# jaswon/osu-dreamer

Hardware: AMD Instinct MI355X
Metric: denoiser train-steps/sec + 50-step sample latents/sec, 1/2/4/8 MI355X (higher is better)
Workload: dtype bf16

## Files before the change

### include/osu_dreamer_hip.h

```cpp
#ifndef OSU_DREAMER_HIP_H
#define OSU_DREAMER_HIP_H

#ifdef __cplusplus
extern "C" {
#endif

enum { OD_F32 = 0, OD_BF16 = 1,
       OD_F32X3 = 2,
       OD_F32X3W = 3,
       OD_F16 = 4 };
enum { OD_EPI_NONE = 0, OD_EPI_SILU = 1 };
enum { OD_ACT_NONE = 0, OD_ACT_SILU = 1 };
enum { OD_ERR_ARG = -1, OD_ERR_ALIGN = -2, OD_ERR_UNSUPPORTED = -3, OD_ERR_COMM = -4 };

int od_version(void);
const char* od_build_source_sha(void);
const char* od_error_string(int code);

int od_gemm_nt(int dtype, const void* A, int lda, const void* W, int ldw, const float* bias, void* C, int ldc,
               int M, int N, int K, int epilogue, int accumulate, void* stream);
int od_gemm_nt_qkrope(int dtype, const void* A, int lda, const void* W, int ldw, const float* bias, void* C, int ldc, int M,
                      int N, int K, const float* wq, const float* wk, const float* table, int L, int H, int hd, float eps,
                      float q_scale, void* stream);
int od_gemm_nt_qkrope_split(int dtype, const void* A, int lda, const void* W, int ldw, const float* bias, void* C, int ldc,
                            void* qk_out, int ldqk, int qk_dtype, int M, int N, int K, const float* wq, const float* wk, const float* table,
                            int L, int H, int hd, float eps, float q_scale, void* stream);
int od_gemm_tn(int dtype, const void* G, int ldg, const void* A, int lda, float* dW, int lddw, float* dbias, int M, int N,
               int K, void* stream);
int od_gemm_tn_blocks(int dtype, const void* G, int ldg, const void* A, int lda, float* dW, int lddw, float* dbias, int M, int N,
                      int K, int n_block, int n_valid, void* stream);
int od_colsum(int dtype, const void* G, int ldg, float* out, int M, int N, void* stream);
int od_pack_weight(int dtype, const float* src, int N, int K, void* dst, int Np, int Kp, int transpose,
                   const int* row_map, void* stream);

int od_linear_small(const float* x, const float* W, const float* b, float* out, float* pre, int B, int N, int K, int act,
                    void* stream);
int od_linear_small_bwd(const float* x, const float* W, const float* pre, const float* dout, float* dpre, float* dW,
                        float* db, float* dx, int accumulate_dx, int B, int N, int K, int act, void* stream);

int od_cl_to_frames(int dtype, const float* src, void* dst, int ldd, int B, int C, int L, void* stream);
int od_proj_in(int dtype, const float* xt, const float* W, const float* bias, void* x, int ldx, int B, int E, int L,
               int D, void* stream);
int od_proj_in_bwd(int dtype, const float* xt, const void* dx, int ldx, float* dW, float* db, int B, int E, int L, int D,
                   void* stream);
int od_silu(int dtype, const void* x, void* y, long n, void* stream);
int od_silu_bwd(int dtype, const void* x, const void* dy, void* dx, long n, void* stream);

int od_rmsnorm_film(int dtype, const void* x, int ldx, const float* ssg, const void* cl, int ldcl, int cl_bcast,
                    void* h, int ldh, float* inv_rms, int B, int L, int C, float eps, void* stream);
int od_rmsnorm_film_bwd(int dtype, const void* x, int ldx, const float* inv_rms, const float* ssg, const void* dh,
                        int lddh, void* dres, int lddres, float* dssg, int B, int L, int C, void* stream);
int od_rmsnorm_gate_residual(int dtype, const void* x, int ldx, const void* h, int ldh, const float* ssg, void* xo,
                             int ldxo, float* inv_rms, int B, int L, int C, float eps, void* stream);
int od_rmsnorm_gate_residual_film(int dtype, const void* x, int ldx, const void* h, int ldh, const float* ssg_a, void* xo, int ldxo,
                                  float* inv_a, const float* ssg_b, const void* cl, int ldcl, int cl_bcast, void* h2, int ldh2,
                                  float* inv_b, int B, int L, int C, float eps, void* stream);
int od_rmsnorm_gate_residual_film_dwconv(int dtype, const void* x, int ldx, const void* h, int ldh, const float* ssg_a, void* xo, int ldxo,
                                         float* inv_a, const float* ssg_b, void* h2, int ldh2, float* inv_b, const float* conv_w,
                                         const float* conv_b, void* y, int ldy, int B, int L, int C, int ksize, float eps, void* stream);
int od_rmsnorm_gate_residual_bwd(int dtype, const void* h, int ldh, const float* inv_rms, const float* ssg,
                                 const void* dy, int lddy, void* dh, int lddh, float* dssg, int B, int L, int C,
                                 void* stream);

int od_rope_table(float* table, int L, int hd, void* stream);
int od_qk_norm_rope(int dtype, const void* qkv, int ldqkv, const float* wq, const float* wk, const float* table,
                    void* qk_out, int ldo, int B, int L, int H, int hd, float eps, float q_scale, void* stream);
int od_qk_norm_rope_bwd(int dtype, const void* qkv, int ldqkv, const float* wq, const float* wk, const float* table,
                        const void* dqk, int lddqk, void* dqkv, int lddqkv, float* dwq, float* dwk, int B, int L,
                        int H, int hd, float eps, float q_scale, void* stream);
int od_flash_attn_fwd(int dtype, const void* q, int ldq, const void* k, int ldk, const void* v, int ldv, void* o, int ldo,
                      float* lse, int B, int H, int L, int hd, float scale, int q_prescaled, void* stream);
int od_flash_attn_fwd_varlen(int dtype, const void* q, int ldq, const void* k, int ldk, const void* v, int ldv, void* o, int ldo,
                             float* lse, const int* lens, int B, int H, int L, int hd, float scale, int q_prescaled, void* stream);
int od_flash_attn_bwd(int dtype, const void* q, int ldq, const void* k, int ldk, const void* v, int ldv, const void* o,
                      int ldo, const void* dout, int lddo, const float* lse, float* delta, void* dq, int lddq, void* dk,
                      int lddk, void* dv, int lddv, int B, int H, int L, int hd, float scale, int q_prescaled, void* stream);
int od_attn_aux_create(void** aux_out);
int od_attn_aux_destroy(void* aux);
int od_flash_attn_bwd_aux(int dtype, const void* q, int ldq, const void* k, int ldk, const void* v, int ldv, const void* o,
                          int ldo, const void* dout, int lddo, const float* lse, float* delta, void* dq, int lddq, void* dk,
                          int lddk, void* dv, int lddv, int B, int H, int L, int hd, float scale, int q_prescaled, void* aux, void* stream);
int od_flash_attn_bwd_varlen(int dtype, const void* q, int ldq, const void* k, int ldk, const void* v, int ldv, const void* o,
                             int ldo, const void* dout, int lddo, const float* lse, float* delta, void* dq, int lddq, void* dk,
                             int lddk, void* dv, int lddv, const int* lens, int B, int H, int L, int hd, float scale, int q_prescaled,
                             void* aux, void* stream);
int od_flash_attn_bwd_fused_ws_bytes(int dtype, int B, int H, int L, long* total_out, long* zero_out);
int od_flash_attn_bwd_fused(int dtype, const void* q, int ldq, const void* k, int ldk, const void* v, int ldv, const void* o, int ldo,
                            const void* dout, int lddo, const float* lse, void* dq, int lddq, void* dk, int lddk, void* dv, int lddv,
                            int B, int H, int L, int hd, float scale, int q_prescaled, void* ws, long ws_bytes, void* stream);
int od_flash_attn_bwd_fused_status(const void* ws, int* err_out, void* stream);
int od_flash_attn_bwd_fused_err_offset(void);
int od_flash_attn_bwd_fused_passes(void);
int od_flash_attn_bwd_fused_prof(void* ws, long* out16);
int od_flash_attn_bwd_passes(void);

int od_dwconv(int dtype, const void* x, int ldx, const float* w, const float* bias, void* y, int ldy, int B, int L,
              int C, int ksize, void* stream);
int od_dwconv_varlen(int dtype, const void* x, int ldx, const float* w, const float* bias, void* y, int ldy, const int* lens,
                     int B, int L, int C, int ksize, void* stream);
int od_dwconv_bwd(int dtype, const void* x, int ldx, const float* w, const void* dy, int lddy, void* dx, int lddx,
                  float* dw, float* db, int B, int L, int C, int ksize, void* stream);
int od_dwconv_bwd_varlen(int dtype, const void* x, int ldx, const float* w, const void* dy, int lddy, void* dx, int lddx,
                         float* dw, float* db, const int* lens, int B, int L, int C, int ksize, void* stream);
int od_scale_channels(int dtype, void* x, int ldx, const float* scale, int B, int L, int C, void* stream);
int od_swiglu_rmsnorm(int dtype, const void* vg, int ldvg, void* hh, int ldhh, float* inv_rms, int M, int Hf, int Hp,
                      float eps, void* stream);
int od_swiglu_rmsnorm_bwd(int dtype, const void* vg, int ldvg, const float* inv_rms, const void* dhh, int lddhh,
                          void* dvg, int lddvg, int M, int Hf, int Hp, void* stream);

int od_final_norm_proj_out(int dtype, const void* x, int ldx, const float* W, const float* bias, float* v,
                           float* inv_rms, int B, int L, int C, int E, float eps, void* stream);
int od_final_norm_proj_out_bwd(int dtype, const void* x, int ldx, const float* inv_rms, const float* W, const float* dv,
                               void* dx, int lddx, float* dW, float* db, int B, int L, int C, int E, void* stream);
int od_uhead_fwd(const float* xt, const float* w0, const float* b0, const float* w1, const float* b1, const float* w3,
                 const float* b3, const float* w4, const float* b4, float* fsum, int B, int E, int L, int U,
                 void* stream);
int od_uhead_fwd_varlen(const float* xt, const float* w0, const float* b0, const float* w1, const float* b1, const float* w3,
                        const float* b3, const float* w4, const float* b4, float* fsum, const int* lens, int B, int E, int L,
                        int U, void* stream);
int od_uhead_bwd(const float* xt, const float* w0, const float* b0, const float* w1, const float* b1, const float* w3,
                 const float* b3, const float* w4, const float* b4, const float* dfm, float* dw0, float* db0, float* dw1,
                 float* db1, float* dw3, float* db3, float* dw4, float* db4, int B, int E, int L, int U, void* stream);
int od_uhead_bwd_varlen(const float* xt, const float* w0, const float* b0, const float* w1, const float* b1, const float* w3,
                        const float* b3, const float* w4, const float* b4, const float* dfm, float* dw0, float* db0, float* dw1,
                        float* db1, float* dw3, float* db3, float* dw4, float* db4, const int* lens, int B, int E, int L, int U,
                        void* stream);
int od_uhead_tail(const float* fsum, const float* mod, const float* w_out, const float* b_out, float* u, int B, int U,
                  int L, float u_scale, void* stream);
int od_uhead_tail_varlen(const float* fsum, const float* mod, const float* w_out, const float* b_out, float* u, const int* lens,
                         int B, int U, int L, float u_scale, void* stream);
int od_uhead_tail_bwd(const float* fsum, const float* mod, const float* w_out, const float* b_out, const float* du,
                      float* dfm, float* dmod, float* dw_out, float* db_out, int B, int U, int L, float u_scale,
                      void* stream);
int od_uhead_tail_bwd_varlen(const float* fsum, const float* mod, const float* w_out, const float* b_out, const float* du,
                             float* dfm, float* dmod, float* dw_out, float* db_out, const int* lens, int B, int U, int L,
                             float u_scale, void* stream);

int od_make_xt(const float* x0, const float* x1, const float* t, float* xt, float* dsq, int B, int E, int L, void* stream);
int od_make_xt_varlen(const float* x0, const float* x1, const float* t, float* xt, float* dsq, const int* lens, int B, int E, int L,
                      void* stream);
int od_loss_grad(const float* xt, const float* x1, const float* u, const float* v, const float* dsq, float* dv,
                 float* sums, int B, int E, int L, float c0, float osl_w, float del_w, void* stream);
int od_loss_grad_varlen(const float* xt, const float* x1, const float* u, const float* v, const float* dsq, float* dv,
                        float* sums, const int* lens, int B, int E, int L, float c0, float osl_w, float del_w, void* stream);
int od_loss_finalize(const float* sums, const float* dsq, const float* u, float* out, float* du, int B, float c0,
                     float osl_w, float del_w, void* stream);
int od_sampler_step(float* x, const float* u, const float* v, const float* eta, int B, int E, int L, void* stream);
int od_sampler_eta(const float* u, float* eta, int B, float c0, int num_steps, void* stream);
int od_sampler_eta_groups(const float* u, const int* offs, float* eta, int G, float c0, int num_steps, void* stream);
int od_sampler_step_varlen(float* x, const float* u, const float* v, const float* eta, const int* lens, const int* offs, int G,
                           int B, int E, int L, void* stream);

int od_det_clear(void);
int od_det_register(const float* base, long count, void* shadow_i64);
int od_det_enable(void* table_dev, void* stream);
int od_det_table_bytes(void);
int od_det_flush(float* dst, long count, void* stream);

int od_sqnorm(const float* g, long n, float* out, const int* status, void* stream);
int od_adamw_ema(float* p, const float* g, float* m, float* v, float* ema, long n, float lr, float beta1, float beta2,
                 float eps, float weight_decay, int step, float ema_decay, int ema_mode, const float* gnorm_sq,
                 float max_norm, const int* status, void* stream);

int od_ema_update(float* ema, const float* p, long n, float ema_decay, int ema_mode, void* stream);

int od_style_conditioning(const float* labels, const float* rff_w, const float* rff_b, const float* cond_w,
                          const float* cond_b, const float* null_labels, float* c, int B, int NL, int F, int H,
                          void* stream);
int od_rmsnorm_rows(const float* x, const float* gamma, float* y, int M, int C, float eps, void* stream);

int od_style_conditioning_bwd(const float* labels, const float* rff_w, const float* rff_b, const float* dc, float* dcond_w,
                              float* dcond_b, float* dnull_labels, int B, int NL, int F, int H, void* stream);
int od_rmsnorm_rows_bwd(const float* x, const float* gamma, const float* dy, float* dx, float* dgamma, int M, int C, float eps,
                        int accumulate_dx, void* stream);
int od_cast_rows(int src_dtype, const void* src, int dst_dtype, void* dst, long n, void* stream);

int od_spec_features_conv(int dtype, const float* audio, const float* w1, const float* b1, const float* g1, const float* w2,
                          const float* b2, const float* g2, void* out, int ldo, int B, int F, int L, float eps, void* stream);
int od_rmsnorm_affine_film(int dtype, const void* x, int ldx, const float* gamma, const float* ssg, void* y, int ldy, int B,
                           int L, int C, float eps, int act, void* stream);
int od_rmsnorm_affine_gate_residual(int dtype, const void* x, int ldx, const void* h, int ldh, const float* gamma,
                                    const float* ssg, void* xo, int ldxo, int B, int L, int C, float eps, void* stream);
int od_unet_mixer(int dtype, const void* x, int ldx, const void* p, int ldp, int p_bcast, const void* gx, int ldg,
                  const float* gamma, void* xo, int ldxo, int B, int L, int C, float eps, void* stream);
int od_unet_down(int dtype, const void* x, int ldx, const float* w, const float* bias, void* y, int ldy, int B, int Lo, int C,
                 int stride, void* stream);
int od_unet_up(int dtype, const void* x, int ldx, const float* w, const float* bias, void* y, int ldy, int B, int Li, int C,
               int stride, void* stream);
int od_chart_head(int dtype, const void* x, int ldx, const float* W, const float* bias, float* out, int B, int L, int C, int N,
// ... 83 lines not shown
```

### osu_dreamer_amd/csrc/heads.hip

```cpp
#include "od_common.h"
#include "od_api_internal.h"

namespace {

constexpr int UW = 32;
constexpr int UOWN = 30;
constexpr int UWPB = 4;
constexpr int MAXU = 64, MAXE = 8;

__device__ __forceinline__ float red32(float v) {
#pragma unroll
    for (int m = 16; m >= 1; m >>= 1) v += __shfl_xor(v, m);
    return v;
}

struct UHeadW {
    const float *w0, *b0, *w1, *b1, *w3, *b3, *w4, *b4;
};

struct UHeadSmem {
    float xts[MAXE][UW + 4];
    float z0s[MAXE][UW + 2];
    float z1s[MAXU][UW + 2];
    float a1s[MAXU][UW + 2];
    float z3s[MAXU][UW + 1];
    float g4s[MAXU][UW + 1];
    float w4s[MAXU][MAXU + 1];
};

__device__ __forceinline__ void uhead_window_fwd(UHeadSmem& S, const float* __restrict__ xt, const UHeadW& P, int b, int l0,
                                                 int E, int L, int U, int Lv) {
    const int t = threadIdx.x;
    for (int idx = t; idx < E * (UW + 4); idx += 256) {
        const int e = idx / (UW + 4), ix = idx % (UW + 4);
        const int f = l0 - 3 + ix;
        S.xts[e][ix] = (f >= 0 && f < Lv) ? xt[((size_t)b * E + e) * L + f] : 0.f;
    }
    __syncthreads();
    for (int idx = t; idx < E * (UW + 2); idx += 256) {
        const int e = idx / (UW + 2), i2 = idx % (UW + 2);
        S.z0s[e][i2] = P.b0[e] + P.w0[e * 3 + 0] * S.xts[e][i2] + P.w0[e * 3 + 1] * S.xts[e][i2 + 1] + P.w0[e * 3 + 2] * S.xts[e][i2 + 2];
    }
    __syncthreads();
    for (int idx = t; idx < U * (UW + 2); idx += 256) {
        const int c = idx / (UW + 2), i2 = idx % (UW + 2);
        const int f = l0 - 2 + i2;
        float z = P.b1[c];
        for (int e = 0; e < E; e++) z += P.w1[c * E + e] * S.z0s[e][i2];
        S.z1s[c][i2] = z;
        S.a1s[c][i2] = (f >= 0 && f < Lv) ? od_silu(z) : 0.f;
    }
    __syncthreads();
    for (int idx = t; idx < U * UW; idx += 256) {
        const int c = idx / UW, i = idx % UW;
        S.z3s[c][i] = P.b3[c] + P.w3[c * 3 + 0] * S.a1s[c][i] + P.w3[c * 3 + 1] * S.a1s[c][i + 1] + P.w3[c * 3 + 2] * S.a1s[c][i + 2];
    }
    __syncthreads();
}

__device__ __forceinline__ void uhead_load_w4(UHeadSmem& S, const UHeadW& P, int U) {
    for (int idx = threadIdx.x; idx < U * U; idx += 256) S.w4s[idx / U][idx % U] = P.w4[idx];
    __syncthreads();
}

template <bool VL = false>
__global__ __launch_bounds__(256) void uhead_fwd_kernel(const float* __restrict__ xt, UHeadW P, float* __restrict__ fsum,
                                                        int E, int L, int U, int nwin, int wpb, const OdDetTable* __restrict__ det,
                                                        const int* __restrict__ lens = nullptr) {
    __shared__ UHeadSmem S;
    const int b = blockIdx.y, t = threadIdx.x;
    const int Lb = VL ? od_uniform(lens[b]) : L;
    const int i = t & 31, grp = t >> 5, cpg = U / 8;
    uhead_load_w4(S, P, U);
    float acc[MAXU / 8];
#pragma unroll
    for (int q = 0; q < MAXU / 8; q++) acc[q] = 0.f;
    for (int wi = 0; wi < wpb; wi++) {
        const int win = blockIdx.x * wpb + wi;
        if (win >= nwin) break;
        const int l0 = win * UOWN;
        if (VL && l0 >= Lb) break;
        uhead_window_fwd(S, xt, P, b, l0, E, L, U, Lb);
        const int f = l0 - 1 + i;
        const bool own = (i >= 1 && i < UW - 1 && f < Lb);
#pragma unroll
        for (int q = 0; q < MAXU / 8; q++) {
            if (q < cpg) {
                const int c = grp * cpg + q;
                float z = P.b4[c];
                for (int cc = 0; cc < U; cc++) z += S.w4s[c][cc] * S.z3s[cc][i];
                if (own) acc[q] += od_silu(z);
            }
        }
        __syncthreads();
    }
#pragma unroll
    for (int q = 0; q < MAXU / 8; q++) {
        const float s = red32(acc[q]);
        if (q < cpg && i == 0) od_red_add(det, fsum + (size_t)b * U + grp * cpg + q, s);
    }
}

struct UHeadG {
    float *dw0, *db0, *dw1, *db1, *dw3, *db3, *dw4, *db4;
};

template <bool VL>
__device__ __forceinline__ void uhead_bwd_body(const float* __restrict__ xt, const UHeadW& P, const float* __restrict__ dfm,
                                               const UHeadG& G, int E, int L, int U, int nwin, const OdDetTable* __restrict__ det,
                                               const int* __restrict__ lens) {
    __shared__ UHeadSmem S;
    __shared__ float sdw3[MAXU][3], sdb3[MAXU], sdb4[MAXU], sdw1[MAXU][MAXE], sdb1[MAXU], sdw0[MAXE][3], sdb0[MAXE];
    const int b = blockIdx.y, t = threadIdx.x;
    const int i = t & 31, grp = t >> 5, cpg = U / 8;
    const int Lb = VL ? od_uniform(lens[b]) : L;
    for (int idx = t; idx < MAXU; idx += 256) {
        sdb3[idx] = 0.f; sdb4[idx] = 0.f; sdb1[idx] = 0.f;
        for (int j = 0; j < 3; j++) sdw3[idx][j] = 0.f;
        for (int e = 0; e < MAXE; e++) sdw1[idx][e] = 0.f;
    }
    if (t < MAXE) { sdb0[t] = 0.f; for (int j = 0; j < 3; j++) sdw0[t][j] = 0.f; }
    uhead_load_w4(S, P, U);
    float adw4[16];
#pragma unroll
    for (int q = 0; q < 16; q++) adw4[q] = 0.f;
    const float invL = 1.0f / (float)Lb;

    for (int wi = 0; wi < UWPB; wi++) {
        const int win = blockIdx.x * UWPB + wi;
        if (win >= nwin) break;
        const int l0 = win * UOWN;
        if (VL && l0 >= Lb) break;
        uhead_window_fwd(S, xt, P, b, l0, E, L, U, Lb);
        const int f = l0 - 1 + i;
        const bool inr = (f >= 0 && f < Lb);
        const bool own = (i >= 1 && i < UW - 1 && f < Lb);
#pragma unroll
        for (int q = 0; q < MAXU / 8; q++) {
            if (q < cpg) {
                const int c = grp * cpg + q;
                float z = P.b4[c];
                for (int cc = 0; cc < U; cc++) z += S.w4s[c][cc] * S.z3s[cc][i];
                const float g = inr ? dfm[(size_t)b * U + c] * invL * od_silu_grad(z) : 0.f;
                S.g4s[c][i] = g;
                const float s = red32(own ? g : 0.f);
                if (i == 0) atomicAdd(&sdb4[c], s);
            }
        }
        __syncthreads();
        {
            const int iend = (Lb - (l0 - 1)) < (UW - 1) ? (Lb - (l0 - 1)) : (UW - 1);
#pragma unroll
            for (int q = 0; q < 16; q++) {
                const int o = t + 256 * q;
                if (o < U * U) {
                    const int c = o / U, cc = o % U;
                    float s = 0.f;
                    for (int ii = 1; ii < iend; ii++) s += S.g4s[c][ii] * S.z3s[cc][ii];
                    adw4[q] += s;
                }
            }
        }
        __syncthreads();
        float dz3v[MAXU / 8];
#pragma unroll
        for (int q = 0; q < MAXU / 8; q++) {
            dz3v[q] = 0.f;
            if (q < cpg) {
                const int cc = grp * cpg + q;
                float s = 0.f;
                for (int c = 0; c < U; c++) s += S.w4s[c][cc] * S.g4s[c][i];
                dz3v[q] = s;
            }
        }
        __syncthreads();
#pragma unroll
        for (int q = 0; q < MAXU / 8; q++)
            if (q < cpg) S.z3s[grp * cpg + q][i] = dz3v[q];
        __syncthreads();
#pragma unroll
        for (int q = 0; q < MAXU / 8; q++) {
            if (q < cpg) {
                const int c = grp * cpg + q;
                const float g = own ? S.z3s[c][i] : 0.f;
                float s = red32(g);
                if (i == 0) atomicAdd(&sdb3[c], s);
                for (int j = 0; j < 3; j++) {
                    s = red32(g * S.a1s[c][i + j]);
                    if (i == 0) atomicAdd(&sdw3[c][j], s);
                }
                float dz1 = 0.f;
                if (own) {
                    float da1 = 0.f;
                    for (int j = 0; j < 3; j++) da1 += P.w3[c * 3 + j] * S.z3s[c][i - j + 1];
                    dz1 = da1 * od_silu_grad(S.z1s[c][i + 1]);
                }
                S.g4s[c][i] = dz1;
                s = red32(dz1);
                if (i == 0) atomicAdd(&sdb1[c], s);
                for (int e = 0; e < E; e++) {
                    s = red32(dz1 * S.z0s[e][i + 1]);
                    if (i == 0) atomicAdd(&sdw1[c][e], s);
                }
            }
        }
        __syncthreads();
        {
            const bool ev = grp < E;
            const int e = ev ? grp : 0;
            float dz0 = 0.f;
            if (ev)
                for (int c = 0; c < U; c++) dz0 += P.w1[c * E + e] * S.g4s[c][i];
            float s = red32(dz0);
            if (ev && i == 0) atomicAdd(&sdb0[e], s);
            for (int j = 0; j < 3; j++) {
                s = red32(dz0 * S.xts[e][i + 1 + j]);
                if (ev && i == 0) atomicAdd(&sdw0[e][j], s);
            }
        }
        __syncthreads();
    }
#pragma unroll
    for (int q = 0; q < 16; q++) {
        const int o = t + 256 * q;
        if (o < U * U) od_red_add(det, G.dw4 + o, adw4[q]);
    }
    __syncthreads();
    for (int c = t; c < U; c += 256) {
        od_red_add(det, G.db4 + c, sdb4[c]);
        od_red_add(det, G.db3 + c, sdb3[c]);
        od_red_add(det, G.db1 + c, sdb1[c]);
        for (int j = 0; j < 3; j++) od_red_add(det, G.dw3 + c * 3 + j, sdw3[c][j]);
        for (int e = 0; e < E; e++) od_red_add(det, G.dw1 + c * E + e, sdw1[c][e]);
    }
    if (t < E) {
        od_red_add(det, G.db0 + t, sdb0[t]);
        for (int j = 0; j < 3; j++) od_red_add(det, G.dw0 + t * 3 + j, sdw0[t][j]);
    }
}

__global__ __launch_bounds__(256) void uhead_bwd_kernel(const float* __restrict__ xt, UHeadW P, const float* __restrict__ dfm,
                                                        UHeadG G, int E, int L, int U, int nwin, const OdDetTable* __restrict__ det) {
    uhead_bwd_body<false>(xt, P, dfm, G, E, L, U, nwin, det, nullptr);
}
__global__ __launch_bounds__(256) void uhead_bwd_varlen_kernel(const float* __restrict__ xt, UHeadW P, const float* __restrict__ dfm,
                                                               UHeadG G, int E, int L, int U, int nwin, const OdDetTable* __restrict__ det,
                                                               const int* __restrict__ lens) {
    uhead_bwd_body<true>(xt, P, dfm, G, E, L, U, nwin, det, lens);
}

template <bool VL = false>
__global__ void uhead_tail_kernel(const float* __restrict__ fsum, const float* __restrict__ mod, const float* __restrict__ w,
                                  const float* __restrict__ bo, float* __restrict__ u, int B, int U, int L, float u_scale,
                                  const int* __restrict__ lens = nullptr) {
    const int b = blockIdx.x, lane = threadIdx.x;
    const float Lf = (float)(VL ? od_uniform(lens[b]) : L);
    float s = 0.f;
    for (int c = lane; c < U; c += 64) {
        const float f = fsum[(size_t)b * U + c] / Lf;
        s += w[c] * (f * (1.f + mod[(size_t)b * 2 * U + c]) + mod[(size_t)b * 2 * U + U + c]);
    }
    s = od_wave_sum(s);
    if (lane == 0) {
        const float y = s + bo[0];
        const float sp = y > 20.f ? y : log1pf(__expf(y));
        u[b] = u_scale * sp;
    }
}
template <bool VL = false>
__global__ void uhead_tail_bwd_kernel(const float* __restrict__ fsum, const float* __restrict__ mod, const float* __restrict__ w,
                                      const float* __restrict__ bo, const float* __restrict__ du, float* __restrict__ dfm,
                                      float* __restrict__ dmod, float* __restrict__ dw, float* __restrict__ dbo,
                                      int B, int U, int L, float u_scale, const OdDetTable* __restrict__ det,
                                      const int* __restrict__ lens = nullptr) {
    const int b = blockIdx.x, lane = threadIdx.x;
    const float Lf = (float)(VL ? od_uniform(lens[b]) : L);
    float s = 0.f;
    for (int c = lane; c < U; c += 64) {
        const float f = fsum[(size_t)b * U + c] / Lf;
        s += w[c] * (f * (1.f + mod[(size_t)b * 2 * U + c]) + mod[(size_t)b * 2 * U + U + c]);
    }
    s = od_wave_sum(s);
    const float y = s + bo[0];
    const float dy = du[b] * u_scale * od_sigmoid(y);
    for (int c = lane; c < U; c += 64) {
        const float f = fsum[(size_t)b * U + c] / Lf;
        const float sc = mod[(size_t)b * 2 * U + c], sh = mod[(size_t)b * 2 * U + U + c];
        const float fm = f * (1.f + sc) + sh;
        od_red_add(det, dw + c, dy * fm);
        const float dfmv = dy * w[c];
        dfm[(size_t)b * U + c] = dfmv * (1.f + sc);
        dmod[(size_t)b * 2 * U + c] = dfmv * f;
        dmod[(size_t)b * 2 * U + U + c] = dfmv;
    }
    if (lane == 0) od_red_add(det, dbo, dy);
}

__device__ __forceinline__ float block_sum_256(float v, float* sh) {
    v = od_wave_sum(v);
    __syncthreads();
    if ((threadIdx.x & 63) == 0) sh[threadIdx.x >> 6] = v;
    __syncthreads();
    return sh[0] + sh[1] + sh[2] + sh[3];
}

template <bool VL = false>
__global__ __launch_bounds__(256) void make_xt_kernel(const float* __restrict__ x0, const float* __restrict__ x1,
                                                      const float* __restrict__ t, float* __restrict__ xt,
                                                      float* __restrict__ dsq, int EL, int L, const OdDetTable* __restrict__ det,
                                                      const int* __restrict__ lens = nullptr) {
    __shared__ float sh[4];
    const int b = blockIdx.y;
    const int Lb = VL ? od_uniform(lens[b]) : L;
    const float w = t[b];
    float acc = 0.f;
    for (int i = blockIdx.x * 256 + threadIdx.x; i < EL; i += gridDim.x * 256) {
        const size_t o = (size_t)b * EL + i;
        if (VL && (i % L) >= Lb) { xt[o] = 0.f; continue; }
        const float a = x0[o], e = x1[o];
        const float v = w < 0.5f ? a + w * (e - a) : e - (e - a) * (1.f - w);
        xt[o] = v;
        const float d = v - e;
        acc += d * d;
    }
    acc = block_sum_256(acc, sh);
    if (threadIdx.x == 0) od_red_add(det, dsq + b, acc / (float)Lb);
}

template <bool VL = false>
__global__ __launch_bounds__(256) void loss_grad_kernel(const float* __restrict__ xt, const float* __restrict__ x1,
                                                        const float* __restrict__ u, const float* __restrict__ v,
                                                        const float* __restrict__ dsq, float* __restrict__ dv,
                                                        float* __restrict__ sums, int B, int EL, int L, float c0,
                                                        float osl_w, float del_w, const OdDetTable* __restrict__ det,
                                                        const int* __restrict__ lens = nullptr) {
    __shared__ float sh[4];
    const int b = blockIdx.y;
    const int Lb = VL ? od_uniform(lens[b]) : L;
    const float ub = u[b], den = dsq[b] + c0, ut = sqrtf(den);
    const float k1 = osl_w / ((float)B * den), k2 = del_w / (float)B, invL2 = 2.f / (float)Lb;
    float s1 = 0.f, s2 = 0.f, s3 = 0.f;
    for (int i = blockIdx.x * 256 + threadIdx.x; i < EL; i += gridDim.x * 256) {
        const size_t o = (size_t)b * EL + i;
        if (VL && (i % L) >= Lb) { dv[o] = 0.f; continue; }
        const float xv = xt[o], e = x1[o], vv = v[o];
        const float r1 = xv - ub * vv - e;
        const float r2 = vv - (xv - e) / ut;
        s1 += r1 * r1; s2 += r2 * r2; s3 += r1 * (-vv);
        dv[o] = k1 * invL2 * r1 * (-ub) + k2 * invL2 * r2;
    }
    s1 = block_sum_256(s1, sh); s2 = block_sum_256(s2, sh); s3 = block_sum_256(s3, sh);
    if (threadIdx.x == 0) {
        od_red_add(det, sums + b * 3 + 0, s1 / (float)Lb);
        od_red_add(det, sums + b * 3 + 1, s2 / (float)Lb);
        od_red_add(det, sums + b * 3 + 2, s3 * invL2);
    }
}

__global__ void loss_finalize_kernel(const float* __restrict__ sums, const float* __restrict__ dsq, const float* __restrict__ u,
                                     float* __restrict__ out, float* __restrict__ du, int B, float c0, float osl_w, float del_w) {
    const int lane = threadIdx.x;
    float osl = 0.f, del = 0.f, mape = 0.f;
    for (int b = lane; b < B; b += 64) {
        const float den = dsq[b] + c0, ut = sqrtf(den);
        osl += sums[b * 3 + 0] / den;
        del += sums[b * 3 + 1];
        mape += fabsf((u[b] - ut) / ut);
        du[b] = osl_w / ((float)B * den) * sums[b * 3 + 2];
    }
    osl = od_wave_sum(osl) / (float)B; del = od_wave_sum(del) / (float)B; mape = od_wave_sum(mape) / (float)B;
    if (lane == 0) { out[0] = osl_w * osl + del_w * del; out[1] = osl; out[2] = del; out[3] = mape; }
}

__global__ __launch_bounds__(256) void sampler_step_kernel(float* __restrict__ x, const float* __restrict__ u,
                                                           const float* __restrict__ v, const float* __restrict__ eta, int EL) {
    const int b = blockIdx.y;
    const float k = eta[0] * u[b];
    for (int i = blockIdx.x * 256 + threadIdx.x; i < EL; i += gridDim.x * 256) {
// ... 215 lines not shown
```

### osu_dreamer_amd/csrc/misc.hip

```cpp
#include "od_common.h"
#include "od_api_internal.h"
#include <type_traits>

namespace {

template <class T>
__global__ __launch_bounds__(256) void cl_to_frames_kernel(const float* __restrict__ src, T* __restrict__ dst, int ldd, int C, int L) {
    __shared__ float tile[64][65];
    const int b = blockIdx.z, l0 = blockIdx.x * 64, c0 = blockIdx.y * 64;
    const int tx = threadIdx.x & 63, ty = threadIdx.x >> 6;
    for (int i = ty; i < 64; i += 4) {
        const int c = c0 + i, l = l0 + tx;
        tile[i][tx] = (c < C && l < L) ? src[((size_t)b * C + c) * L + l] : 0.f;
    }
    __syncthreads();
    for (int i = ty; i < 64; i += 4) {
        const int l = l0 + i, c = c0 + tx;
        if (l < L && c < C) od_t<T>::st(dst + ((size_t)b * L + l) * ldd + c, tile[tx][i]);
    }
}

template <class T>
__global__ __launch_bounds__(256) void proj_in_kernel(const float* __restrict__ xt, const float* __restrict__ W,
                                                      const float* __restrict__ bias, T* __restrict__ x, int ldx,
                                                      int B, int E, int L, int D) {
    const int lane = threadIdx.x & 63;
    const long M = (long)B * L;
    const long nw = (long)gridDim.x * 4, w0 = (long)blockIdx.x * 4 + (threadIdx.x >> 6);
    for (int c = lane * 8; c < D; c += 512) {
        float wv[8][8], bv[8];
        od_ld8(bias + c, bv);
        if (E == 6) {
            float flat[48];
#pragma unroll
            for (int q = 0; q < 6; q++) od_ld8(W + (size_t)c * 6 + q * 8, *(float(*)[8])&flat[q * 8]);
#pragma unroll
            for (int k = 0; k < 8; k++)
#pragma unroll
                for (int e = 0; e < 8; e++) wv[k][e] = e < 6 ? flat[k * 6 + e] : 0.f;
        } else {
#pragma unroll
            for (int k = 0; k < 8; k++)
#pragma unroll
                for (int e = 0; e < 8; e++) wv[k][e] = e < E ? W[(size_t)(c + k) * E + e] : 0.f;
        }
        for (long m = w0; m < M; m += nw) {
            const int b = (int)(m / L), l = (int)(m % L);
            float xe[8];
#pragma unroll
            for (int e = 0; e < 8; e++) xe[e] = e < E ? xt[((size_t)b * E + e) * L + l] : 0.f;
            float o[8];
#pragma unroll
            for (int k = 0; k < 8; k++) {
                float s = bv[k];
#pragma unroll
                for (int e = 0; e < 8; e++) s += wv[k][e] * xe[e];
                o[k] = s;
            }
            od_st8(x + m * ldx + c, o);
        }
    }
}

template <class T>
__global__ __launch_bounds__(256) void proj_in_bwd_kernel(const float* __restrict__ xt, const T* __restrict__ dx, int ldx,
                                                          float* __restrict__ dW, float* __restrict__ db, int B, int E, int L, int D,
                                                          const OdDetTable* __restrict__ det) {
    __shared__ float red[64][73];
    const int lane = threadIdx.x & 63, wave = threadIdx.x >> 6;
    const int M = B * L;
    const int nw = gridDim.x * 4, w0 = blockIdx.x * 4 + wave;
    for (int c0 = 0; c0 < D; c0 += 512) {
        const int c = c0 + lane * 8;
        float aw[8][8], ab[8];
#pragma unroll
        for (int k = 0; k < 8; k++) {
            ab[k] = 0.f;
#pragma unroll
            for (int e = 0; e < 8; e++) aw[k][e] = 0.f;
        }
        if (c < D)
            for (int m = w0; m < M; m += nw) {
                const int b = m / L, l = m - b * L;
                float xe[8], g[8];
#pragma unroll
                for (int e = 0; e < 8; e++) xe[e] = e < E ? xt[((size_t)b * E + e) * L + l] : 0.f;
                od_ld8(dx + (size_t)m * ldx + c, g);
#pragma unroll
                for (int k = 0; k < 8; k++) {
                    ab[k] += g[k];
#pragma unroll
                    for (int e = 0; e < 8; e++) aw[k][e] += g[k] * xe[e];
                }
            }
        for (int w = 0; w < 4; w++) {
            if (wave == w) {
#pragma unroll
                for (int k = 0; k < 8; k++) {
                    red[lane][k * 9 + 8] = (w ? red[lane][k * 9 + 8] : 0.f) + ab[k];
#pragma unroll
                    for (int e = 0; e < 8; e++) red[lane][k * 9 + e] = (w ? red[lane][k * 9 + e] : 0.f) + aw[k][e];
                }
            }
            __syncthreads();
        }
        if (wave == 0 && c < D) {
#pragma unroll
            for (int k = 0; k < 8; k++) {
                od_red_add(det, db + c + k, red[lane][k * 9 + 8]);
#pragma unroll
                for (int e = 0; e < 8; e++)
                    if (e < E) od_red_add(det, dW + (size_t)(c + k) * E + e, red[lane][k * 9 + e]);
            }
        }
        __syncthreads();
    }
}

template <class T>
__global__ __launch_bounds__(256) void silu_kernel(const T* __restrict__ x, T* __restrict__ y, long n8) {
    for (long i = (long)blockIdx.x * 256 + threadIdx.x; i < n8; i += (long)gridDim.x * 256) {
        float v[8]; od_ld8(x + i * 8, v);
#pragma unroll
        for (int e = 0; e < 8; e++) v[e] = od_silu(v[e]);
        od_st8(y + i * 8, v);
    }
}
template <class T>
__global__ __launch_bounds__(256) void silu_bwd_kernel(const T* __restrict__ x, const T* __restrict__ dy, T* __restrict__ dx, long n8) {
    for (long i = (long)blockIdx.x * 256 + threadIdx.x; i < n8; i += (long)gridDim.x * 256) {
        float v[8], g[8]; od_ld8(x + i * 8, v); od_ld8(dy + i * 8, g);
#pragma unroll
        for (int e = 0; e < 8; e++) g[e] *= od_silu_grad(v[e]);
        od_st8(dx + i * 8, g);
    }
}

template <class T, int KS, int DW_RUN, bool VL = false>
__global__ __launch_bounds__(256) void dwconv_kernel(const T* __restrict__ x, int ldx, const float* __restrict__ w,
                                                     const float* __restrict__ bias, T* __restrict__ y, int ldy,
                                                     int L, int C, const int* __restrict__ lens = nullptr) {
    constexpr int R = KS / 2;
    const int cg = C / 8;
    const int b = blockIdx.y;
    const int Lb = VL ? od_uniform(lens[b]) : L;
    const long t = (long)blockIdx.x * 256 + threadIdx.x;
    const int cgi = (int)(t % cg);
    const long run = t / cg;
    const int l0 = (int)(run * DW_RUN);
    if (l0 >= L) return;
    const int c = cgi * 8;
    float wv[8][KS], bv[8];
#pragma unroll
    for (int k = 0; k < 8; k++) {
        bv[k] = bias[c + k];
#pragma unroll
        for (int j = 0; j < KS; j++) wv[k][j] = w[(size_t)(c + k) * KS + j];
    }
    float win[KS][8];
    const T* xb = x + (size_t)b * L * ldx + c;
#pragma unroll
    for (int j = 0; j < KS - 1; j++) {
        const int l = l0 - R + j;
        if (l >= 0 && l < Lb) od_ld8(xb + (size_t)l * ldx, win[j]);
        else {
#pragma unroll
            for (int k = 0; k < 8; k++) win[j][k] = 0.f;
        }
    }
    for (int i = 0; i < DW_RUN; i++) {
        const int l = l0 + i;
        if (l >= L) break;
        const int ln = l + R;
        if (ln < Lb) od_ld8(xb + (size_t)ln * ldx, win[KS - 1]);
        else {
#pragma unroll
            for (int k = 0; k < 8; k++) win[KS - 1][k] = 0.f;
        }
        float o[8];
#pragma unroll
        for (int k = 0; k < 8; k++) {
            float s = bv[k];
#pragma unroll
            for (int j = 0; j < KS; j++) s += wv[k][j] * win[j][k];
            o[k] = (VL && l >= Lb) ? 0.f : s;
        }
        od_st8(y + ((size_t)b * L + l) * ldy + c, o);
#pragma unroll
        for (int j = 0; j < KS - 1; j++)
#pragma unroll
            for (int k = 0; k < 8; k++) win[j][k] = win[j + 1][k];
    }
}

constexpr int DW_RUN_BWD = 64;
template <class T, int KS, bool VL = false>
__global__ __launch_bounds__(256) void dwconv_bwd_kernel(const T* __restrict__ x, int ldx, const float* __restrict__ w,
                                                         const T* __restrict__ dy, int lddy, T* __restrict__ dx, int lddx,
                                                         float* __restrict__ dw, float* __restrict__ db, int L, int C,
                                                         const OdDetTable* __restrict__ det, const int* __restrict__ lens = nullptr) {
    constexpr int R = KS / 2;
    __shared__ long long red[(KS <= 5 ? 1024 : 512) * (KS + 1)];
    __shared__ int s_bad;
    const int cg = C / 8;
    const int b = blockIdx.y;
    const int Lb = VL ? od_uniform(lens[b]) : L;
    const long t = (long)blockIdx.x * 256 + threadIdx.x;
    const int cgi = (int)(t % cg);
    const long run = t / cg;
    const int l0 = (int)(run * DW_RUN_BWD);
    const bool active = l0 < L;
    const int c = cgi * 8;
    for (int i = threadIdx.x; i < C * (KS + 1); i += 256) red[i] = 0;
    if (threadIdx.x == 0) s_bad = 0;
    __syncthreads();
    float wv[8][KS], adw[8][KS], adb[8];
#pragma unroll
    for (int k = 0; k < 8; k++) {
        adb[k] = 0.f;
#pragma unroll
        for (int j = 0; j < KS; j++) { wv[k][j] = w[(size_t)(c + k) * KS + j]; adw[k][j] = 0.f; }
    }
    if (active) {
        float wy[KS][8], wx[KS][8];
        const T* xb = x + (size_t)b * L * ldx + c;
        const T* yb = dy + (size_t)b * L * lddy + c;
#pragma unroll
        for (int j = 0; j < KS - 1; j++) {
            const int l = l0 - R + j;
            if (l >= 0 && l < Lb) { od_ld8(xb + (size_t)l * ldx, wx[j]); od_ld8(yb + (size_t)l * lddy, wy[j]); }
            else {
#pragma unroll
                for (int k = 0; k < 8; k++) { wx[j][k] = 0.f; wy[j][k] = 0.f; }
            }
        }
        constexpr int DW_PF = 2;
        typedef typename std::conditional<sizeof(T) == 2, u32x4, f32x4>::type row_t;
        row_t px[DW_PF][sizeof(T) == 2 ? 1 : 2], py[DW_PF][sizeof(T) == 2 ? 1 : 2];
        auto fetch = [&](int ln, int slot) {
            if (ln < Lb) {
#pragma unroll
                for (int h2 = 0; h2 < (sizeof(T) == 2 ? 1 : 2); h2++) {
                    px[slot][h2] = *(const row_t*)(xb + (size_t)ln * ldx + h2 * 4);
                    py[slot][h2] = *(const row_t*)(yb + (size_t)ln * lddy + h2 * 4);
                }
            } else {
#pragma unroll
                for (int h2 = 0; h2 < (sizeof(T) == 2 ? 1 : 2); h2++) { px[slot][h2] = (row_t)(0); py[slot][h2] = (row_t)(0); }
            }
        };
        auto unpack = [&](const row_t (&r)[sizeof(T) == 2 ? 1 : 2], float (&o8)[8]) {
            if constexpr (sizeof(T) == 2) {
#pragma unroll
                for (int i2 = 0; i2 < 4; i2++) {
                    union { uint32_t u; float f; } lo, hi;
                    lo.u = r[0][i2] << 16; hi.u = r[0][i2] & 0xffff0000u;
                    o8[2 * i2] = lo.f; o8[2 * i2 + 1] = hi.f;
                }
            } else {
#pragma unroll
                for (int i2 = 0; i2 < 4; i2++) { o8[i2] = r[0][i2]; o8[4 + i2] = r[1][i2]; }
            }
        };
#pragma unroll
        for (int pf = 0; pf < DW_PF; pf++) fetch(l0 + R + pf, pf);
        for (int i0 = 0; i0 < DW_RUN_BWD; i0 += DW_PF) {
          if (l0 + i0 >= L) break;
#pragma unroll
          for (int pf = 0; pf < DW_PF; pf++) {
            const int i = i0 + pf;
            const int l = l0 + i;
            if (l >= L) break;
            unpack(px[pf], wx[KS - 1]);
            unpack(py[pf], wy[KS - 1]);
            fetch(l + R + DW_PF, pf);
            float o[8];
#pragma unroll
            for (int k = 0; k < 8; k++) {
                float sacc = 0.f;
#pragma unroll
                for (int jj = 0; jj < KS; jj++) sacc += wv[k][jj] * wy[KS - 1 - jj][k];
                o[k] = (VL && l >= Lb) ? 0.f : sacc;
                const float gy = wy[R][k];
                adb[k] += gy;
#pragma unroll
                for (int jj = 0; jj < KS; jj++) adw[k][jj] += gy * wx[jj][k];
            }
            od_st8(dx + ((size_t)b * L + l) * lddx + c, o);
#pragma unroll
            for (int j = 0; j < KS - 1; j++)
#pragma unroll
                for (int k = 0; k < 8; k++) { wx[j][k] = wx[j + 1][k]; wy[j][k] = wy[j + 1][k]; }
          }
        }
#pragma unroll
        for (int k = 0; k < 8; k++) {
            od_lds_fix_add(&red[(c + k) * (KS + 1) + KS], adb[k], &s_bad);
#pragma unroll
            for (int j = 0; j < KS; j++) od_lds_fix_add(&red[(c + k) * (KS + 1) + j], adw[k][j], &s_bad);
        }
    }
    __syncthreads();
    for (int i = threadIdx.x; i < C * (KS + 1); i += 256) {
        const int ch = i / (KS + 1), j = i % (KS + 1);
        const float v = od_lds_unfix(red[i], s_bad);
        if (v != 0.f) {
            if (j == KS) od_red_add(det, db + ch, v); else od_red_add(det, dw + (size_t)ch * KS + j, v);
        }
    }
}

constexpr int LS_KC = 256, LS_NB = 8;
__global__ __launch_bounds__(256) void linear_small_kernel(const float* __restrict__ x, const float* __restrict__ W,
                                                           const float* __restrict__ bias, float* __restrict__ out,
                                                           float* __restrict__ pre, int B, int N, int K, int act) {
    __shared__ __attribute__((aligned(16))) float xs[32][LS_KC + 4];
    __shared__ __attribute__((aligned(16))) float ws[LS_NB][LS_KC + 4];
    const int b0 = blockIdx.y * 32, n0 = blockIdx.x * LS_NB;
    const int bl = threadIdx.x & 31, nl = threadIdx.x >> 5;
    float acc = 0.f;
    for (int k0 = 0; k0 < K; k0 += LS_KC) {
        const int kc = K - k0 < LS_KC ? K - k0 : LS_KC;
        for (int i = threadIdx.x; i < 32 * LS_KC; i += 256) {
            const int r = i / LS_KC, c = i % LS_KC;
            xs[r][c] = (b0 + r < B && c < kc) ? x[(size_t)(b0 + r) * K + k0 + c] : 0.f;
        }
        for (int i = threadIdx.x; i < LS_NB * LS_KC; i += 256) {
            const int r = i / LS_KC, c = i % LS_KC;
            ws[r][c] = (n0 + r < N && c < kc) ? W[(size_t)(n0 + r) * K + k0 + c] : 0.f;
        }
        __syncthreads();
#pragma unroll 8
        for (int c = 0; c < LS_KC; c += 4) {
            const f32x4 a = *(const f32x4*)&xs[bl][c], w = *(const f32x4*)&ws[nl][c];
            acc += a[0] * w[0]; acc += a[1] * w[1]; acc += a[2] * w[2]; acc += a[3] * w[3];
        }
        __syncthreads();
    }
    const int b = b0 + bl, n = n0 + nl;
    if (b < B && n < N) {
        const float s = acc + (bias ? bias[n] : 0.f);
        if (pre) pre[(size_t)b * N + n] = s;
        out[(size_t)b * N + n] = act == OD_ACT_SILU ? od_silu(s) : s;
    }
}
__global__ __launch_bounds__(256) void linear_small_dpre_kernel(const float* __restrict__ pre, const float* __restrict__ dout,
                                                                float* __restrict__ dpre, long n, int act) {
    const long i = (long)blockIdx.x * 256 + threadIdx.x;
    if (i >= n) return;
    dpre[i] = act == OD_ACT_SILU ? dout[i] * od_silu_grad(pre[i]) : dout[i];
}
__global__ __launch_bounds__(256) void linear_small_dw_kernel(const float* __restrict__ x, const float* __restrict__ dpre,
                                                              float* __restrict__ dW, float* __restrict__ db, int B, int N, int K) {
    const int n = blockIdx.y, k = blockIdx.x * 256 + threadIdx.x;
    if (dW && k < K) {
        float s0 = 0.f, s1 = 0.f, s2 = 0.f, s3 = 0.f;
        int b = 0;
        for (; b + 3 < B; b += 4) {
            s0 += dpre[(size_t)b * N + n] * x[(size_t)b * K + k];
            s1 += dpre[(size_t)(b + 1) * N + n] * x[(size_t)(b + 1) * K + k];
            s2 += dpre[(size_t)(b + 2) * N + n] * x[(size_t)(b + 2) * K + k];
            s3 += dpre[(size_t)(b + 3) * N + n] * x[(size_t)(b + 3) * K + k];
        }
        for (; b < B; b++) s0 += dpre[(size_t)b * N + n] * x[(size_t)b * K + k];
        dW[(size_t)n * K + k] += (s0 + s1) + (s2 + s3);
    }
    if (db && blockIdx.x == 0 && threadIdx.x == 0) {
        float s = 0.f;
        for (int b = 0; b < B; b++) s += dpre[(size_t)b * N + n];
        db[n] += s;
    }
}
constexpr int LS_NR = 32;
__global__ __launch_bounds__(256) void linear_small_dx_kernel(const float* __restrict__ W, const float* __restrict__ dpre,
                                                              float* __restrict__ dx, int B, int N, int K, const OdDetTable* __restrict__ det) {
    __shared__ __attribute__((aligned(16))) float ds[LS_NR][32];
    const int n0 = blockIdx.x * LS_NR, b0 = blockIdx.y * 32, k = blockIdx.z * 256 + threadIdx.x;
    for (int i = threadIdx.x; i < LS_NR * 32; i += 256) {
        const int bl = i / LS_NR, nl = i % LS_NR;
        ds[nl][bl] = (b0 + bl < B && n0 + nl < N) ? dpre[(size_t)(b0 + bl) * N + n0 + nl] : 0.f;
    }
    __syncthreads();
    if (k >= K) return;
    float acc[32];
#pragma unroll
    for (int i = 0; i < 32; i++) acc[i] = 0.f;
    const int nr = N - n0 < LS_NR ? N - n0 : LS_NR;
    for (int nl = 0; nl < nr; nl++) {
        const float w = W[(size_t)(n0 + nl) * K + k];
#pragma unroll
        for (int q4 = 0; q4 < 8; q4++) {
            const f32x4 d = *(const f32x4*)&ds[nl][4 * q4];
            acc[4 * q4] += d[0] * w; acc[4 * q4 + 1] += d[1] * w; acc[4 * q4 + 2] += d[2] * w; acc[4 * q4 + 3] += d[3] * w;
        }
    }
#pragma unroll
    for (int i = 0; i < 32; i++)
        if (b0 + i < B) od_red_add(det, dx + (size_t)(b0 + i) * K + k, acc[i]);
}

__global__ __launch_bounds__(256) void zero_f32_kernel(float* __restrict__ p, long n) {
    const long i = (long)blockIdx.x * 256 + threadIdx.x;
    if (i < n) p[i] = 0.f;
}

template <class T>
__global__ __launch_bounds__(256) void pack_weight_kernel(const float* __restrict__ src, int N, int K, T* __restrict__ dst,
                                                          int Np, int Kp, int transpose, const int* __restrict__ row_map) {
    const long i = (long)blockIdx.x * 256 + threadIdx.x;
    if (i >= (long)Np * Kp) return;
    int n, k;
    if (!transpose) { n = (int)(i / Kp); k = (int)(i % Kp); }
    else { k = (int)(i / Np); n = (int)(i % Np); }
    const int sn = row_map ? row_map[n] : (n < N ? n : -1);
    const float v = (sn >= 0 && k < K) ? src[(size_t)sn * K + k] : 0.f;
    od_t<T>::st(dst + i, v);
}

__global__ __launch_bounds__(256) void pack_weight_split_kernel(const float* __restrict__ src, int N, int K, bf16_t* __restrict__ dst,
                                                                int Np, int Kp, const int* __restrict__ row_map) {
    const long i = (long)blockIdx.x * 256 + threadIdx.x;
    if (i >= (long)Np * Kp) return;
    const int n = (int)(i / Kp), k = (int)(i % Kp);
    const int sn = row_map ? row_map[n] : (n < N ? n : -1);
    const float v = (sn >= 0 && k < K) ? src[(size_t)sn * K + k] : 0.f;
    const bf16_t hi = od_f2bf(v);
    const bf16_t lo = od_f2bf(v - od_bf2f(hi));
    bf16_t* slab = dst + ((size_t)n * Kp + (k & ~31)) * 2;
    slab[k & 31] = hi;
    slab[32 + (k & 31)] = lo;
}

}

#define DISPATCH_T(DT, CALL)                                       \
    do {                                                           \
        if ((DT) == OD_BF16) { typedef bf16_t T_; CALL; }          \
        else if ((DT) == OD_F32) { typedef float T_; CALL; }       \
        else return OD_ERR_ARG;                                    \
    } while (0)

extern "C" int od_cl_to_frames(int dtype, const float* src, void* dst, int ldd, int B, int C, int L, void* stream) {
    dim3 grid((L + 63) / 64, (C + 63) / 64, B);
    DISPATCH_T(dtype, OD_LAUNCH((cl_to_frames_kernel<T_>), grid, dim3(256), 0, (hipStream_t)stream, src, (T_*)dst, ldd, C, L));
    OD_CHECK_LAUNCH();
    return 0;
}

extern "C" int od_proj_in(int dtype, const float* xt, const float* W, const float* bias, void* x, int ldx, int B, int E, int L,
                          int D, void* stream) {
    if (E > 8) return OD_ERR_UNSUPPORTED;
    if (D % 8 || ldx % 8) return OD_ERR_ALIGN;
    const long M = (long)B * L;
    int blocks = (int)((M + 15) / 16); if (blocks > 4096) blocks = 4096;
    DISPATCH_T(dtype, OD_LAUNCH((proj_in_kernel<T_>), dim3(blocks), dim3(256), 0, (hipStream_t)stream, xt, W, bias, (T_*)x, ldx, B, E, L, D));
    OD_CHECK_LAUNCH();
    return 0;
}

extern "C" int od_proj_in_bwd(int dtype, const float* xt, const void* dx, int ldx, float* dW, float* db, int B, int E, int L, int D,
                              void* stream) {
    if (E > 8) return OD_ERR_UNSUPPORTED;
    if (D % 8 || ldx % 8) return OD_ERR_ALIGN;
    const long M = (long)B * L;
    if (M > 0x7fffffffL) return OD_ERR_UNSUPPORTED;
    int blocks = (int)((M + 63) / 64); if (blocks > 512) blocks = 512; if (blocks < 1) blocks = 1;
    DISPATCH_T(dtype, OD_LAUNCH((proj_in_bwd_kernel<T_>), dim3(blocks), dim3(256), 0, (hipStream_t)stream, xt, (const T_*)dx, ldx, dW, db, B, E, L, D, od_det_active()));
    OD_CHECK_LAUNCH();
    return 0;
}

extern "C" int od_silu(int dtype, const void* x, void* y, long n, void* stream) {
    if (n % 8) return OD_ERR_ALIGN;
    long n8 = n / 8; int blocks = (int)((n8 + 255) / 256); if (blocks > 4096) blocks = 4096; if (blocks < 1) blocks = 1;
    DISPATCH_T(dtype, OD_LAUNCH((silu_kernel<T_>), dim3(blocks), dim3(256), 0, (hipStream_t)stream, (const T_*)x, (T_*)y, n8));
    OD_CHECK_LAUNCH();
    return 0;
}
extern "C" int od_silu_bwd(int dtype, const void* x, const void* dy, void* dx, long n, void* stream) {
    if (n % 8) return OD_ERR_ALIGN;
    long n8 = n / 8; int blocks = (int)((n8 + 255) / 256); if (blocks > 4096) blocks = 4096; if (blocks < 1) blocks = 1;
    DISPATCH_T(dtype, OD_LAUNCH((silu_bwd_kernel<T_>), dim3(blocks), dim3(256), 0, (hipStream_t)stream, (const T_*)x, (const T_*)dy, (T_*)dx, n8));
    OD_CHECK_LAUNCH();
    return 0;
}

template <class T>
__global__ __launch_bounds__(256) void scale_channels_kernel(T* __restrict__ x, int ldx, const float* __restrict__ scale, long M, int L, int C) {
    const int cg = C / 8;
    const long i = (long)blockIdx.x * 256 + threadIdx.x;
    if (i >= M * cg) return;
    const long m = i / cg;
    const int c = (int)(i % cg) * 8;
    float v[8], f[8];
    od_ld8(x + m * ldx + c, v);
    od_ld8(scale + (m / L) * C + c, f);
#pragma unroll
    for (int e = 0; e < 8; e++) v[e] *= f[e];
    od_st8(x + m * ldx + c, v);
}

extern "C" int od_scale_channels(int dtype, void* x, int ldx, const float* scale, int B, int L, int C, void* stream) {
    if (C % 8 || ldx % 8) return OD_ERR_ALIGN;
    const long M = (long)B * L, n = M * (C / 8);
    if (n == 0) return 0;
    DISPATCH_T(dtype, OD_LAUNCH((scale_channels_kernel<T_>), dim3((unsigned)((n + 255) / 256)), dim3(256), 0, (hipStream_t)stream, (T_*)x, ldx, scale, M, L, C));
    OD_CHECK_LAUNCH();
    return 0;
}

extern "C" int od_dwconv(int dtype, const void* x, int ldx, const float* w, const float* bias, void* y, int ldy, int B, int L,
                         int C, int ksize, void* stream) {
    if (C % 8 || ldx % 8 || ldy % 8) return OD_ERR_ALIGN;
    if (ksize != 3 && ksize != 5 && ksize != 7 && ksize != 9) return OD_ERR_UNSUPPORTED;
#ifndef OD_DW_SMALL_THREADS
#define OD_DW_SMALL_THREADS 131072
#endif
    const bool small = (long)B * (C / 8) * ((L + 31) / 32) < OD_DW_SMALL_THREADS;
    const int run = small ? 4 : 32;
    const long threads = (long)(C / 8) * ((L + run - 1) / run);
    dim3 grid((unsigned)((threads + 255) / 256), B);
#define DW_GO(KS_, RUN_) DISPATCH_T(dtype, OD_LAUNCH((dwconv_kernel<T_, KS_, RUN_>), grid, dim3(256), 0, (hipStream_t)stream, (const T_*)x, ldx, w, bias, (T_*)y, ldy, L, C))
    if (ksize == 5) { if (small) DW_GO(5, 4); else DW_GO(5, 32); }
    else if (ksize == 3) { if (small) DW_GO(3, 4); else DW_GO(3, 32); }
    else if (ksize == 7) { if (small) DW_GO(7, 4); else DW_GO(7, 32); }
    else { if (small) DW_GO(9, 4); else DW_GO(9, 32); }
#undef DW_GO
    OD_CHECK_LAUNCH();
    return 0;
}

extern "C" int od_dwconv_varlen(int dtype, const void* x, int ldx, const float* w, const float* bias, void* y, int ldy, const int* lens,
                                int B, int L, int C, int ksize, void* stream) {
    if (C % 8 || ldx % 8 || ldy % 8) return OD_ERR_ALIGN;
    if (ksize != 3 && ksize != 5 && ksize != 7 && ksize != 9) return OD_ERR_UNSUPPORTED;
    if (!lens) return OD_ERR_ARG;
    const bool small = (long)B * (C / 8) * ((L + 31) / 32) < OD_DW_SMALL_THREADS;
    const int run = small ? 4 : 32;
    const long threads = (long)(C / 8) * ((L + run - 1) / run);
    dim3 grid((unsigned)((threads + 255) / 256), B);
#define DW_GO(KS_, RUN_) DISPATCH_T(dtype, OD_LAUNCH((dwconv_kernel<T_, KS_, RUN_, true>), grid, dim3(256), 0, (hipStream_t)stream, (const T_*)x, ldx, w, bias, (T_*)y, ldy, L, C, lens))
    if (ksize == 5) { if (small) DW_GO(5, 4); else DW_GO(5, 32); }
    else if (ksize == 3) { if (small) DW_GO(3, 4); else DW_GO(3, 32); }
    else if (ksize == 7) { if (small) DW_GO(7, 4); else DW_GO(7, 32); }
    else { if (small) DW_GO(9, 4); else DW_GO(9, 32); }
#undef DW_GO
    OD_CHECK_LAUNCH();
    return 0;
}

extern "C" int od_dwconv_bwd(int dtype, const void* x, int ldx, const float* w, const void* dy, int lddy, void* dx, int lddx,
                             float* dw, float* db, int B, int L, int C, int ksize, void* stream) {
    if (C % 8 || ldx % 8 || lddy % 8 || lddx % 8) return OD_ERR_ALIGN;
    if (C > 1024 || (ksize > 5 && C > 512)) return OD_ERR_UNSUPPORTED;
    const long threads = (long)(C / 8) * ((L + DW_RUN_BWD - 1) / DW_RUN_BWD);
    dim3 grid((unsigned)((threads + 255) / 256), B);
    if (ksize == 5) DISPATCH_T(dtype, OD_LAUNCH((dwconv_bwd_kernel<T_, 5>), grid, dim3(256), 0, (hipStream_t)stream, (const T_*)x, ldx, w, (const T_*)dy, lddy, (T_*)dx, lddx, dw, db, L, C, od_det_active()));
    else if (ksize == 3) DISPATCH_T(dtype, OD_LAUNCH((dwconv_bwd_kernel<T_, 3>), grid, dim3(256), 0, (hipStream_t)stream, (const T_*)x, ldx, w, (const T_*)dy, lddy, (T_*)dx, lddx, dw, db, L, C, od_det_active()));
    else if (ksize == 7 && C <= 512) DISPATCH_T(dtype, OD_LAUNCH((dwconv_bwd_kernel<T_, 7>), grid, dim3(256), 0, (hipStream_t)stream, (const T_*)x, ldx, w, (const T_*)dy, lddy, (T_*)dx, lddx, dw, db, L, C, od_det_active()));
    else if (ksize == 9 && C <= 512) DISPATCH_T(dtype, OD_LAUNCH((dwconv_bwd_kernel<T_, 9>), grid, dim3(256), 0, (hipStream_t)stream, (const T_*)x, ldx, w, (const T_*)dy, lddy, (T_*)dx, lddx, dw, db, L, C, od_det_active()));
    else return OD_ERR_UNSUPPORTED;
    OD_CHECK_LAUNCH();
    return 0;
}

extern "C" int od_dwconv_bwd_varlen(int dtype, const void* x, int ldx, const float* w, const void* dy, int lddy, void* dx, int lddx,
                                    float* dw, float* db, const int* lens, int B, int L, int C, int ksize, void* stream) {
    if (C % 8 || ldx % 8 || lddy % 8 || lddx % 8) return OD_ERR_ALIGN;
    if (C > 1024 || (ksize > 5 && C > 512)) return OD_ERR_UNSUPPORTED;
    if (!lens) return OD_ERR_ARG;
    const long threads = (long)(C / 8) * ((L + DW_RUN_BWD - 1) / DW_RUN_BWD);
    dim3 grid((unsigned)((threads + 255) / 256), B);
#define DWB_GO(KS_) DISPATCH_T(dtype, OD_LAUNCH((dwconv_bwd_kernel<T_, KS_, true>), grid, dim3(256), 0, (hipStream_t)stream, (const T_*)x, ldx, w, (const T_*)dy, lddy, (T_*)dx, lddx, dw, db, L, C, od_det_active(), lens))
    if (ksize == 5) DWB_GO(5);
    else if (ksize == 3) DWB_GO(3);
    else if (ksize == 7) DWB_GO(7);
    else if (ksize == 9) DWB_GO(9);
    else return OD_ERR_UNSUPPORTED;
#undef DWB_GO
    OD_CHECK_LAUNCH();
    return 0;
}

extern "C" int od_linear_small(const float* x, const float* W, const float* b, float* out, float* pre, int B, int N, int K, int act,
                               void* stream) {
    OD_LAUNCH(linear_small_kernel, dim3((N + LS_NB - 1) / LS_NB, (B + 31) / 32), dim3(256), 0, (hipStream_t)stream, x, W, b, out, pre, B, N, K, act);
    OD_CHECK_LAUNCH();
    return 0;
}

extern "C" int od_linear_small_bwd(const float* x, const float* W, const float* pre, const float* dout, float* dpre, float* dW,
                                   float* db, float* dx, int accumulate_dx, int B, int N, int K, int act, void* stream) {
    if (act != OD_ACT_NONE && !pre) return OD_ERR_ARG;
    const long n = (long)B * N;
    OD_LAUNCH(linear_small_dpre_kernel, dim3((unsigned)((n + 255) / 256)), dim3(256), 0, (hipStream_t)stream, pre, dout, dpre, n, act);
    if (dW || db)
        OD_LAUNCH(linear_small_dw_kernel, dim3((K + 255) / 256, N), dim3(256), 0, (hipStream_t)stream, x, (const float*)dpre, dW, db, B, N, K);
    if (dx) {
        if (!accumulate_dx)
            OD_LAUNCH(zero_f32_kernel, dim3((unsigned)(((long)B * K + 255) / 256)), dim3(256), 0, (hipStream_t)stream, dx, (long)B * K);
        OD_LAUNCH(linear_small_dx_kernel, dim3((N + LS_NR - 1) / LS_NR, (B + 31) / 32, (K + 255) / 256), dim3(256), 0, (hipStream_t)stream, W,
                  (const float*)dpre, dx, B, N, K, od_det_active());
    }
    OD_CHECK_LAUNCH();
    return 0;
}

extern "C" int od_pack_weight(int dtype, const float* src, int N, int K, void* dst, int Np, int Kp, int transpose,
                              const int* row_map, void* stream) {
    const long n = (long)Np * Kp;
    if (dtype == OD_F32X3W) {
        if (transpose || Kp % 32) return OD_ERR_UNSUPPORTED;
        OD_LAUNCH(pack_weight_split_kernel, dim3((unsigned)((n + 255) / 256)), dim3(256), 0, (hipStream_t)stream, src, N, K, (bf16_t*)dst, Np, Kp, row_map);
        OD_CHECK_LAUNCH();
        return 0;
    }
    DISPATCH_T(dtype, OD_LAUNCH((pack_weight_kernel<T_>), dim3((unsigned)((n + 255) / 256)), dim3(256), 0, (hipStream_t)stream, src, N, K, (T_*)dst, Np, Kp, transpose, row_map));
    OD_CHECK_LAUNCH();
    return 0;
}
```

### osu_dreamer_amd/csrc/od_common.h

```cpp
#pragma once
#if defined(OD_EMU)
#include "emu_hip.h"
#else
#include <hip/hip_runtime.h>
#define OD_LAUNCH(kern, grid, block, smem, stream, ...) \
    hipLaunchKernelGGL(kern, (grid), (block), (smem), (stream), __VA_ARGS__)
#define OD_LAUNCH_DYN(kern, grid, block, smem, stream, ...)                                                    \
    do {                                                                                                       \
         \
        static const hipError_t attr_rc__ =                                                                    \
            hipFuncSetAttribute((const void*)(kern), hipFuncAttributeMaxDynamicSharedMemorySize, 160 * 1024);  \
        if (attr_rc__ != hipSuccess) return -(int)attr_rc__ - 1000;                                            \
        hipLaunchKernelGGL(kern, (grid), (block), (smem), (stream), __VA_ARGS__);                              \
    } while (0)
#define OD_DYN_SMEM(name) extern __shared__ __attribute__((aligned(16))) unsigned char name[]
#endif
#include <stdint.h>

typedef unsigned short bf16_t;
typedef float f32x4 __attribute__((ext_vector_type(4)));
typedef float f32x16 __attribute__((ext_vector_type(16)));
typedef short s16x8 __attribute__((ext_vector_type(8)));
typedef short s16x4 __attribute__((ext_vector_type(4)));
typedef unsigned int u32x4 __attribute__((ext_vector_type(4)));
typedef unsigned int u32x2 __attribute__((ext_vector_type(2)));

#define OD_WAVE 64

__device__ __forceinline__ float od_bf2f(bf16_t h) {
    union { uint32_t u; float f; } c; c.u = ((uint32_t)h) << 16; return c.f;
}
#if defined(OD_EMU)
__device__ __forceinline__ bf16_t od_f2bf(float f) {
    union { uint32_t u; float f; } c; c.f = f;
    uint32_t u = c.u;
    if ((u & 0x7fffffffu) > 0x7f800000u) return (bf16_t)((u >> 16) | 0x40);
    u += 0x7fffu + ((u >> 16) & 1u);
    return (bf16_t)(u >> 16);
}
__device__ __forceinline__ uint32_t od_pack_bf2(float lo, float hi) { return (uint32_t)od_f2bf(lo) | ((uint32_t)od_f2bf(hi) << 16); }
__device__ __forceinline__ float od_exp2(float x) { return exp2f(x); }
#else
typedef __bf16 od_bf2_t __attribute__((ext_vector_type(2)));
typedef float od_f2_t __attribute__((ext_vector_type(2)));
__device__ __forceinline__ bf16_t od_f2bf(float f) { return __builtin_bit_cast(unsigned short, (__bf16)f); }
__device__ __forceinline__ uint32_t od_pack_bf2(float lo, float hi) {
    od_f2_t v; v[0] = lo; v[1] = hi;
    return __builtin_bit_cast(uint32_t, __builtin_convertvector(v, od_bf2_t));
}
__device__ __forceinline__ float od_exp2(float x) { return __builtin_amdgcn_exp2f(x); }
#endif

struct f16_t { unsigned short bits; };
#if defined(OD_EMU)
__device__ __forceinline__ float od_h2f(f16_t h) { return emu::f16_to_f32(h.bits); }
__device__ __forceinline__ f16_t od_f2h(float f) { return f16_t{emu::f32_to_f16(f)}; }
#else
__device__ __forceinline__ float od_h2f(f16_t h) { return (float)__builtin_bit_cast(_Float16, h.bits); }
__device__ __forceinline__ f16_t od_f2h(float f) { return f16_t{__builtin_bit_cast(unsigned short, (_Float16)f)}; }
#endif
#if defined(OD_EMU)
__device__ __forceinline__ uint32_t od_pack_h2(float lo, float hi) { return (uint32_t)od_f2h(lo).bits | ((uint32_t)od_f2h(hi).bits << 16); }
#else
typedef _Float16 od_h2_t __attribute__((ext_vector_type(2)));
__device__ __forceinline__ uint32_t od_pack_h2(float lo, float hi) {
    float __attribute__((ext_vector_type(2))) v; v[0] = lo; v[1] = hi;
    return __builtin_bit_cast(uint32_t, __builtin_convertvector(v, od_h2_t));
}
#endif
template <class T> __device__ __forceinline__ uint32_t od_pack2(float lo, float hi);
template <> __device__ __forceinline__ uint32_t od_pack2<bf16_t>(float lo, float hi) { return od_pack_bf2(lo, hi); }
template <> __device__ __forceinline__ uint32_t od_pack2<f16_t>(float lo, float hi) { return od_pack_h2(lo, hi); }

struct f32x3_t { float x; };
struct f32x3w_t : f32x3_t {};

template <class T> struct od_t;
template <> struct od_t<f32x3_t> {
    static __device__ __forceinline__ float ld(const f32x3_t* p) { return p->x; }
    static __device__ __forceinline__ void st(f32x3_t* p, float v) { p->x = v; }
};
template <> struct od_t<f32x3w_t> : od_t<f32x3_t> {};
template <> struct od_t<float> {
    static __device__ __forceinline__ float ld(const float* p) { return *p; }
    static __device__ __forceinline__ void st(float* p, float v) { *p = v; }
};
template <> struct od_t<bf16_t> {
    static __device__ __forceinline__ float ld(const bf16_t* p) { return od_bf2f(*p); }
    static __device__ __forceinline__ void st(bf16_t* p, float v) { *p = od_f2bf(v); }
};
template <> struct od_t<f16_t> {
    static __device__ __forceinline__ float ld(const f16_t* p) { return od_h2f(*p); }
    static __device__ __forceinline__ void st(f16_t* p, float v) { *p = od_f2h(v); }
};

template <class T> __device__ __forceinline__ float od_round_to(float x);
template <> __device__ __forceinline__ float od_round_to<float>(float x) { return x; }
template <> __device__ __forceinline__ float od_round_to<bf16_t>(float x) { return od_bf2f(od_f2bf(x)); }
template <> __device__ __forceinline__ float od_round_to<f16_t>(float x) { return od_h2f(od_f2h(x)); }
template <> __device__ __forceinline__ float od_round_to<f32x3_t>(float x) { return x; }
template <> __device__ __forceinline__ float od_round_to<f32x3w_t>(float x) { return x; }

__device__ __forceinline__ void od_ld8(const float* p, float (&v)[8]) {
    f32x4 a = *(const f32x4*)p, b = *(const f32x4*)(p + 4);
    v[0] = a[0]; v[1] = a[1]; v[2] = a[2]; v[3] = a[3];
    v[4] = b[0]; v[5] = b[1]; v[6] = b[2]; v[7] = b[3];
}
__device__ __forceinline__ void od_ld8(const bf16_t* p, float (&v)[8]) {
    u32x4 r = *(const u32x4*)p;
#pragma unroll
    for (int i = 0; i < 4; i++) {
        union { uint32_t u; float f; } lo, hi;
        lo.u = r[i] << 16; hi.u = r[i] & 0xffff0000u;
        v[2 * i] = lo.f; v[2 * i + 1] = hi.f;
    }
}
__device__ __forceinline__ void od_st8(float* p, const float (&v)[8]) {
    f32x4 a, b;
    a[0] = v[0]; a[1] = v[1]; a[2] = v[2]; a[3] = v[3];
    b[0] = v[4]; b[1] = v[5]; b[2] = v[6]; b[3] = v[7];
    *(f32x4*)p = a; *(f32x4*)(p + 4) = b;
}
__device__ __forceinline__ void od_ld8(const f32x3_t* p, float (&v)[8]) { od_ld8((const float*)p, v); }
__device__ __forceinline__ void od_st8(f32x3_t* p, const float (&v)[8]) { od_st8((float*)p, v); }
__device__ __forceinline__ void od_st8(bf16_t* p, const float (&v)[8]) {
    u32x4 r;
#pragma unroll
    for (int i = 0; i < 4; i++) r[i] = od_pack_bf2(v[2 * i], v[2 * i + 1]);
    *(u32x4*)p = r;
}

__device__ __forceinline__ void od_ld8(const f16_t* p, float (&v)[8]) {
    u32x4 r = *(const u32x4*)p;
#pragma unroll
    for (int i = 0; i < 4; i++) {
        v[2 * i] = od_h2f(f16_t{(unsigned short)(r[i] & 0xffffu)});
        v[2 * i + 1] = od_h2f(f16_t{(unsigned short)(r[i] >> 16)});
    }
}
__device__ __forceinline__ void od_st8(f16_t* p, const float (&v)[8]) {
    u32x4 r;
#pragma unroll
    for (int i = 0; i < 4; i++) r[i] = od_pack_h2(v[2 * i], v[2 * i + 1]);
    *(u32x4*)p = r;
}

template <class T> __device__ __forceinline__ void od_st8_nt(T* p, const float (&v)[8]) { od_st8(p, v); }
#if !defined(OD_EMU)
template <> __device__ __forceinline__ void od_st8_nt<bf16_t>(bf16_t* p, const float (&v)[8]) {
    u32x4 r;
#pragma unroll
    for (int i = 0; i < 4; i++) r[i] = od_pack_bf2(v[2 * i], v[2 * i + 1]);
    asm volatile("global_store_dwordx4 %0, %1, off nt\n\ts_nop 0" ::"v"(p), "v"(r) : "memory");
}
#endif

#if defined(OD_EMU)
__device__ __forceinline__ void od_st16_nt(void* p, u32x4 r) { *(u32x4*)p = r; }
#else
__device__ __forceinline__ void od_st16_nt(void* p, u32x4 r) {
    asm volatile("global_store_dwordx4 %0, %1, off nt\n\ts_nop 0" ::"v"(p), "v"(r) : "memory");
}
#endif

__device__ __forceinline__ float od_wave_sum(float v) {
#pragma unroll
    for (int m = 32; m >= 1; m >>= 1) v += __shfl_xor(v, m);
    return v;
}
__device__ __forceinline__ float od_silu(float x) { return x / (1.0f + __expf(-x)); }
__device__ __forceinline__ float od_sigmoid(float x) { return 1.0f / (1.0f + __expf(-x)); }
__device__ __forceinline__ float od_silu_grad(float x) {
    float s = od_sigmoid(x);
    return s * (1.0f + x * (1.0f - s));
}

#if defined(OD_EMU)
__device__ __forceinline__ f32x4 od_mul4(f32x4 a, f32x4 b) { return a * b; }
__device__ __forceinline__ f32x4 od_mul4s(f32x4 a, float b) { return a * b; }
#else
__device__ __forceinline__ float od_mul1(float a, float b) {
    float d = a * b;
    asm("" : "+v"(d));
    return d;
}
__device__ __forceinline__ f32x4 od_mul4(f32x4 a, f32x4 b) {
    f32x4 d;
#pragma unroll
    for (int r = 0; r < 4; r++) d[r] = od_mul1(a[r], b[r]);
    return d;
}
__device__ __forceinline__ f32x4 od_mul4s(f32x4 a, float b) {
    f32x4 d;
#pragma unroll
    for (int r = 0; r < 4; r++) d[r] = od_mul1(a[r], b);
    return d;
}
#endif

template <class T> struct od_frag;
template <> struct od_frag<bf16_t> { s16x8 v; };
template <> struct od_frag<f16_t> { s16x8 v; };
template <> struct od_frag<float> { float v[8]; };
template <> struct od_frag<f32x3_t> { s16x8 hi, lo; };
template <> struct od_frag<f32x3w_t> : od_frag<f32x3_t> {};
__device__ __forceinline__ void od_frag_pack(od_frag<float>& f, const float (&x)[8]) {
#pragma unroll
    for (int j = 0; j < 8; j++) f.v[j] = x[j];
}
__device__ __forceinline__ void od_split2(float a, float b, uint32_t& hi, uint32_t& lo) {
    hi = od_pack_bf2(a, b);
    union { uint32_t u; float f; } x, y;
    x.u = hi << 16; y.u = hi & 0xffff0000u;
    lo = od_pack_bf2(a - x.f, b - y.f);
}
__device__ __forceinline__ void od_frag_pack(od_frag<f32x3_t>& f, const float (&x)[8]) {
    u32x4 h, l;
#pragma unroll
    for (int i = 0; i < 4; i++) {
        uint32_t a, b;
        od_split2(x[2 * i], x[2 * i + 1], a, b);
        h[i] = a; l[i] = b;
    }
    f.hi = __builtin_bit_cast(s16x8, h); f.lo = __builtin_bit_cast(s16x8, l);
}

__device__ __forceinline__ void od_frag_load(od_frag<bf16_t>& f, const bf16_t* p) { f.v = *(const s16x8*)p; }
__device__ __forceinline__ void od_frag_load(od_frag<f16_t>& f, const f16_t* p) { f.v = *(const s16x8*)p; }
__device__ __forceinline__ void od_frag_load(od_frag<float>& f, const float* p) { od_ld8(p, f.v); }
__device__ __forceinline__ void od_frag_load(od_frag<f32x3_t>& f, const f32x3_t* p) { float x[8]; od_ld8(p, x); od_frag_pack(f, x); }
__device__ __forceinline__ void od_frag_zero(od_frag<bf16_t>& f) { f.v = (s16x8)(0); }
__device__ __forceinline__ void od_frag_zero(od_frag<float>& f) {
#pragma unroll
    for (int j = 0; j < 8; j++) f.v[j] = 0.f;
}
__device__ __forceinline__ void od_frag_zero(od_frag<f32x3_t>& f) { f.hi = (s16x8)(0); f.lo = (s16x8)(0); }
__device__ __forceinline__ void od_frag_set4(od_frag<bf16_t>& f, int half, float a, float b, float c, float d) {
    u32x4 w = __builtin_bit_cast(u32x4, f.v);
    w[2 * half] = od_pack_bf2(a, b);
    w[2 * half + 1] = od_pack_bf2(c, d);
    f.v = __builtin_bit_cast(s16x8, w);
}
__device__ __forceinline__ void od_frag_set4(od_frag<f16_t>& f, int half, float a, float b, float c, float d) {
    u32x4 w = __builtin_bit_cast(u32x4, f.v);
    w[2 * half] = od_pack_h2(a, b);
    w[2 * half + 1] = od_pack_h2(c, d);
    f.v = __builtin_bit_cast(s16x8, w);
}
__device__ __forceinline__ void od_frag_set4(od_frag<float>& f, int half, float a, float b, float c, float d) {
    f.v[4 * half] = a; f.v[4 * half + 1] = b; f.v[4 * half + 2] = c; f.v[4 * half + 3] = d;
}
__device__ __forceinline__ void od_frag_set4(od_frag<f32x3_t>& f, int half, float a, float b, float c, float d) {
    u32x4 h = __builtin_bit_cast(u32x4, f.hi), l = __builtin_bit_cast(u32x4, f.lo);
    uint32_t h0, l0, h1, l1;
    od_split2(a, b, h0, l0);
    od_split2(c, d, h1, l1);
    h[2 * half] = h0; l[2 * half] = l0; h[2 * half + 1] = h1; l[2 * half + 1] = l1;
    f.hi = __builtin_bit_cast(s16x8, h); f.lo = __builtin_bit_cast(s16x8, l);
}

#if defined(OD_EMU)
__device__ __forceinline__ s16x4 od_lds_tr_read(const bf16_t* p) { return emu::ds_read_tr16_b64(p); }
#else
__device__ __forceinline__ s16x4 od_lds_tr_read(const bf16_t* p) {
    return __builtin_amdgcn_ds_read_tr16_b64_v4i16((__attribute__((address_space(3))) s16x4*)p);
}
#endif
__device__ __forceinline__ s16x4 od_lds_tr_read_at(unsigned addr);

__device__ __forceinline__ f32x4 od_mma(const od_frag<bf16_t>& a, const od_frag<bf16_t>& b, f32x4 c) {
    return __builtin_amdgcn_mfma_f32_16x16x32_bf16(a.v, b.v, c, 0, 0, 0);
}
#if defined(OD_EMU)
__device__ __forceinline__ f32x4 od_mma(const od_frag<f16_t>& a, const od_frag<f16_t>& b, f32x4 c) { return emu::mfma_16x16x32_f16(a.v, b.v, c); }
#else
typedef _Float16 od_h8_t __attribute__((ext_vector_type(8)));
__device__ __forceinline__ f32x4 od_mma(const od_frag<f16_t>& a, const od_frag<f16_t>& b, f32x4 c) {
    return __builtin_amdgcn_mfma_f32_16x16x32_f16(__builtin_bit_cast(od_h8_t, a.v), __builtin_bit_cast(od_h8_t, b.v), c, 0, 0, 0);
}
#endif
__device__ __forceinline__ f32x4 od_mma(const od_frag<float>& a, const od_frag<float>& b, f32x4 c) {
#pragma unroll
    for (int j = 0; j < 8; j++) c = __builtin_amdgcn_mfma_f32_16x16x4f32(a.v[j], b.v[j], c, 0, 0, 0);
    return c;
}
__device__ __forceinline__ f32x4 od_mma(const od_frag<f32x3_t>& a, const od_frag<f32x3_t>& b, f32x4 c) {
    c = __builtin_amdgcn_mfma_f32_16x16x32_bf16(a.lo, b.hi, c, 0, 0, 0);
    c = __builtin_amdgcn_mfma_f32_16x16x32_bf16(a.hi, b.lo, c, 0, 0, 0);
    return __builtin_amdgcn_mfma_f32_16x16x32_bf16(a.hi, b.hi, c, 0, 0, 0);
}

static __device__ __attribute__((aligned(16))) unsigned char od_zero16[16];

#if defined(OD_EMU)
__device__ __forceinline__ void od_glds16(const void* g, void* lds) { emu::global_load_lds16(g, lds); }
#else
__device__ __forceinline__ void od_glds16(const void* g, void* lds) {
    __builtin_amdgcn_global_load_lds((const __attribute__((address_space(1))) void*)g,
                                     (__attribute__((address_space(3))) void*)lds, 16, 0, 0);
}
#endif
#if defined(OD_EMU)
__device__ __forceinline__ void od_glds16_async(const void* g, void* lds_base) { emu::global_load_lds16(g, (unsigned char*)lds_base + 16 * emu::lane_id()); }
#else
__device__ __forceinline__ void od_glds16_async(const void* g, void* lds_base) {
    const unsigned a = (unsigned)__builtin_amdgcn_readfirstlane((int)(unsigned)(size_t)(__attribute__((address_space(3))) unsigned char*)lds_base);
    asm volatile("s_mov_b32 m0, %1\n\ts_nop 0\n\tglobal_load_lds_dwordx4 %0, off" ::"v"(g), "s"(a) : "memory", "m0");
}
#endif

#if defined(OD_EMU)
struct od_srd_t { const unsigned char* base; unsigned bytes; };
__device__ __forceinline__ od_srd_t od_make_srd(const void* base, unsigned bytes) { return od_srd_t{(const unsigned char*)base, bytes}; }
__device__ __forceinline__ void od_srd_set_bytes(od_srd_t& r, unsigned bytes) { r.bytes = bytes; }
__device__ __forceinline__ void od_buffer_lds16(od_srd_t r, unsigned voff, unsigned soff, void* lds) {
    alignas(16) unsigned char tmp[16] = {0};
    const unsigned off = voff + soff;
    if (off < r.bytes) { const unsigned n = (r.bytes - off) & ~3u; memcpy(tmp, r.base + off, n < 16 ? n : 16); }
    emu::global_load_lds16(tmp, (unsigned char*)lds + 16 * emu::lane_id());
}
// ... 137 lines not shown
```

### osu_dreamer_amd/csrc/rowops.hip

```cpp
#include "od_common.h"
#include "od_api_internal.h"

namespace {

#ifndef OD_QK_BPW
#define OD_QK_BPW 8
#endif
constexpr int ROWS_PER_WAVE_BWD = 16;

template <class T, int NCH>
__device__ __forceinline__ void load_row(const T* row, int C, int lane, float (&v)[NCH][8]) {
#pragma unroll
    for (int i = 0; i < NCH; i++) {
        const int c = (lane + 64 * i) * 8;
        if (c < C) od_ld8(row + c, v[i]);
        else {
#pragma unroll
            for (int e = 0; e < 8; e++) v[i][e] = 0.f;
        }
    }
}
template <int NCH>
__device__ __forceinline__ float row_sumsq(const float (&v)[NCH][8]) {
    float s = 0.f;
// ... 250 lines not shown
                for (int e = 0; e < 8; e++) hv[e] = v[0][e] * inv2 * (1.f + sc[e]) + sh[e];
                if (own && h2) od_st8(h2 + m * ldh2 + c, hv);
#pragma unroll
                for (int e = 0; e < 8; e++) win[KS - 1][e] = od_round_to<T>(hv[e]);
            }
        }
        const int lc = l - R;
        if (lc >= l0 && lc < lend && act) {
            float o[8];
#pragma unroll
            for (int k = 0; k < 8; k++) {
                float s = bv[k];
#pragma unroll
                for (int j = 0; j < KS; j++) s += wv[k][j] * win[j][k];
                o[k] = s;
            }
            od_st8(y + ((size_t)b * L + lc) * ldy + c, o);
        }
#pragma unroll
        for (int j = 0; j < KS - 1; j++)
#pragma unroll
            for (int e = 0; e < 8; e++) win[j][e] = win[j + 1][e];
    }
}

template <class T, int NCH>
__global__ __launch_bounds__(256) void rmsnorm_gate_res_bwd_kernel(const T* __restrict__ h, int ldh, const float* __restrict__ inv_rms,
                                                                   const float* __restrict__ ssg, const T* __restrict__ dy, int lddy,
                                                                   T* __restrict__ dh, int lddh, float* __restrict__ dssg,
                                                                   int B, int L, int C, const OdDetTable* __restrict__ det) {
    __shared__ float red[NCH * 512];
    const int lane = threadIdx.x & 63, wave = threadIdx.x >> 6;
    const int b = blockIdx.y;
    const int l0 = (blockIdx.x * 4 + wave) * ROWS_PER_WAVE_BWD;
    float dg[NCH][8], gate[NCH][8];
#pragma unroll
    for (int i = 0; i < NCH; i++) {
        const int c = (lane + 64 * i) * 8;
#pragma unroll
        for (int e = 0; e < 8; e++) { dg[i][e] = 0.f; gate[i][e] = 0.f; }
        if (c < C) od_ld8(ssg + (size_t)b * 3 * C + 2 * C + c, gate[i]);
    }
    for (int r = 0; r < ROWS_PER_WAVE_BWD; r++) {
        const int l = l0 + r;
        if (l >= L) break;
        const long m = (long)b * L + l;
        float hv[NCH][8], gv[NCH][8];
        load_row<T, NCH>(h + m * ldh, C, lane, hv);
        load_row<T, NCH>(dy + m * lddy, C, lane, gv);
        const float inv = inv_rms[m];
        float dot = 0.f;
#pragma unroll
        for (int i = 0; i < NCH; i++)
#pragma unroll
            for (int e = 0; e < 8; e++) {
                const float hh = hv[i][e] * inv;
                dg[i][e] += gv[i][e] * hh;
                gv[i][e] *= gate[i][e];
                dot += gv[i][e] * hh;
                hv[i][e] = hh;
            }
        dot = od_wave_sum(dot) / (float)C;
#pragma unroll
        for (int i = 0; i < NCH; i++) {
            const int c = (lane + 64 * i) * 8;
            if (c >= C) continue;
            float o[8];
#pragma unroll
            for (int e = 0; e < 8; e++) o[e] = inv * (gv[i][e] - hv[i][e] * dot);
            od_st8(dh + m * lddh + c, o);
        }
    }
    for (int w = 0; w < 4; w++) {
        if (wave == w) {
#pragma unroll
            for (int i = 0; i < NCH; i++)
#pragma unroll
                for (int e = 0; e < 8; e++) {
                    const int idx = (lane + 64 * i) * 8 + e;
                    if (w == 0) red[idx] = dg[i][e]; else red[idx] += dg[i][e];
                }
        }
        __syncthreads();
    }
    for (int c = threadIdx.x; c < C; c += 256) od_red_add(det, dssg + (size_t)b * 3 * C + 2 * C + c, red[c]);
}

template <class T, int NCH>
__global__ __launch_bounds__(256) void swiglu_rmsnorm_kernel(const T* __restrict__ vg, int ldvg, T* __restrict__ hh, int ldhh,
                                                             float* __restrict__ inv_rms, long M, int Hf, int Hp, float eps) {
    const int lane = threadIdx.x & 63;
    const long m = (long)blockIdx.x * 4 + (threadIdx.x >> 6);
    if (m >= M) return;
    float v[NCH][8], g[NCH][8];
    load_row<T, NCH>(vg + m * ldvg, Hp, lane, v);
    load_row<T, NCH>(vg + m * ldvg + Hp, Hp, lane, g);
#pragma unroll
    for (int i = 0; i < NCH; i++)
#pragma unroll
        for (int e = 0; e < 8; e++) v[i][e] *= od_silu(g[i][e]);
    const float inv = rsqrtf(row_sumsq<NCH>(v) / (float)Hf + eps);
    if (lane == 0 && inv_rms) inv_rms[m] = inv;
#pragma unroll
    for (int i = 0; i < NCH; i++) {
        const int c = (lane + 64 * i) * 8;
        if (c >= Hp) continue;
        float o[8];
#pragma unroll
        for (int e = 0; e < 8; e++) o[e] = v[i][e] * inv;
        od_st8(hh + m * ldhh + c, o);
    }
}

template <class T, int NCH>
__global__ __launch_bounds__(256) void swiglu_rmsnorm_bwd_kernel(const T* __restrict__ vg, int ldvg, const float* __restrict__ inv_rms,
                                                                 const T* __restrict__ dhh, int lddhh, T* __restrict__ dvg, int lddvg,
                                                                 long M, int Hf, int Hp) {
    const int lane = threadIdx.x & 63;
    const long m = (long)blockIdx.x * 4 + (threadIdx.x >> 6);
    if (m >= M) return;
    float v[NCH][8], g[NCH][8], d[NCH][8];
    load_row<T, NCH>(vg + m * ldvg, Hp, lane, v);
    load_row<T, NCH>(vg + m * ldvg + Hp, Hp, lane, g);
    load_row<T, NCH>(dhh + m * lddhh, Hp, lane, d);
    const float inv = inv_rms[m];
    float dot = 0.f;
    float sg[NCH][8], gs[NCH][8];
#pragma unroll
    for (int i = 0; i < NCH; i++)
#pragma unroll
        for (int e = 0; e < 8; e++) {
            gs[i][e] = od_sigmoid(g[i][e]);
            sg[i][e] = g[i][e] * gs[i][e];
            dot += d[i][e] * (v[i][e] * sg[i][e] * inv);
        }
    dot = od_wave_sum(dot) / (float)Hf;
#pragma unroll
    for (int i = 0; i < NCH; i++) {
        const int c = (lane + 64 * i) * 8;
        if (c >= Hp) continue;
        float ov[8], og[8];
#pragma unroll
        for (int e = 0; e < 8; e++) {
            const float sh = v[i][e] * sg[i][e] * inv;
            const float ds = inv * (d[i][e] - sh * dot);
            ov[e] = ds * sg[i][e];
            og[e] = ds * v[i][e] * (gs[i][e] * (1.0f + g[i][e] * (1.0f - gs[i][e])));
        }
        od_st8(dvg + m * lddvg + c, ov);
        od_st8(dvg + m * lddvg + Hp + c, og);
    }
}

template <class T, int NCH>
__global__ __launch_bounds__(256) void final_proj_kernel(const T* __restrict__ x, int ldx, const float* __restrict__ W,
                                                         const float* __restrict__ bias, float* __restrict__ vout,
                                                         float* __restrict__ inv_rms, int B, int L, int C, int E, float eps) {
    const int lane = threadIdx.x & 63;
    const long m = (long)blockIdx.x * 4 + (threadIdx.x >> 6);
    if (m >= (long)B * L) return;
    const int b = (int)(m / L), l = (int)(m % L);
    float v[NCH][8];
    load_row<T, NCH>(x + m * ldx, C, lane, v);
    const float inv = rsqrtf(row_sumsq<NCH>(v) / (float)C + eps);
    if (lane == 0 && inv_rms) inv_rms[m] = inv;
    for (int e = 0; e < E; e++) {
        float s = 0.f;
#pragma unroll
        for (int i = 0; i < NCH; i++) {
            const int c = (lane + 64 * i) * 8;
            if (c >= C) continue;
            float w[8]; od_ld8(W + (size_t)e * C + c, w);
#pragma unroll
            for (int k = 0; k < 8; k++) s += w[k] * v[i][k];
        }
        s = od_wave_sum(s) * inv;
        if (lane == 0) vout[((size_t)b * E + e) * L + l] = s + bias[e];
    }
}

template <class T, int NCH>
__global__ __launch_bounds__(256) void final_proj_bwd_kernel(const T* __restrict__ x, int ldx, const float* __restrict__ inv_rms,
                                                             const float* __restrict__ W, const float* __restrict__ dv,
                                                             T* __restrict__ dx, int lddx, float* __restrict__ dW,
                                                             float* __restrict__ db, int B, int L, int C, int E,
                                                             const OdDetTable* __restrict__ det) {
    constexpr int MAXE = 8;
    __shared__ float red[MAXE * NCH * 512];
    __shared__ float redb[4][MAXE];
    const int lane = threadIdx.x & 63, wave = threadIdx.x >> 6;
    const int b = blockIdx.y;
    const int l0 = (blockIdx.x * 4 + wave) * ROWS_PER_WAVE_BWD;
    float wv[MAXE][NCH][8], dw[MAXE][NCH][8], dbv[MAXE];
#pragma unroll
    for (int e = 0; e < MAXE; e++) {
        dbv[e] = 0.f;
#pragma unroll
        for (int i = 0; i < NCH; i++) {
            const int c = (lane + 64 * i) * 8;
#pragma unroll
            for (int k = 0; k < 8; k++) { wv[e][i][k] = 0.f; dw[e][i][k] = 0.f; }
            if (e < E && c < C) od_ld8(W + (size_t)e * C + c, wv[e][i]);
        }
    }
    for (int r = 0; r < ROWS_PER_WAVE_BWD; r++) {
        const int l = l0 + r;
        if (l >= L) break;
        const long m = (long)b * L + l;
        float xv[NCH][8], dn[NCH][8], dve[MAXE];
        load_row<T, NCH>(x + m * ldx, C, lane, xv);
        const float inv = inv_rms[m];
#pragma unroll
        for (int e = 0; e < MAXE; e++) { dve[e] = e < E ? dv[((size_t)b * E + e) * L + l] : 0.f; dbv[e] += dve[e]; }
        float dot = 0.f;
#pragma unroll
        for (int i = 0; i < NCH; i++)
#pragma unroll
            for (int k = 0; k < 8; k++) {
                const float xh = xv[i][k] * inv;
                float s = 0.f;
#pragma unroll
                for (int e = 0; e < MAXE; e++) { s += dve[e] * wv[e][i][k]; dw[e][i][k] += dve[e] * xh; }
                dn[i][k] = s;
                dot += s * xh;
                xv[i][k] = xh;
            }
        dot = od_wave_sum(dot) / (float)C;
#pragma unroll
        for (int i = 0; i < NCH; i++) {
            const int c = (lane + 64 * i) * 8;
            if (c >= C) continue;
            float o[8];
#pragma unroll
            for (int k = 0; k < 8; k++) o[k] = inv * (dn[i][k] - xv[i][k] * dot);
            od_st8(dx + m * lddx + c, o);
        }
    }
    if (lane == 0)
        for (int e = 0; e < MAXE; e++) redb[wave][e] = dbv[e];
    for (int w = 0; w < 4; w++) {
        if (wave == w) {
#pragma unroll
            for (int e = 0; e < MAXE; e++)
#pragma unroll
                for (int i = 0; i < NCH; i++)
#pragma unroll
                    for (int k = 0; k < 8; k++) {
                        const int idx = e * NCH * 512 + (lane + 64 * i) * 8 + k;
                        if (w == 0) red[idx] = dw[e][i][k]; else red[idx] += dw[e][i][k];
                    }
        }
        __syncthreads();
    }
    for (int e = 0; e < E; e++)
        for (int c = threadIdx.x; c < C; c += 256) od_red_add(det, dW + (size_t)e * C + c, red[e * NCH * 512 + c]);
    if (threadIdx.x < E) od_red_add(det, db + threadIdx.x, redb[0][threadIdx.x] + redb[1][threadIdx.x] + redb[2][threadIdx.x] + redb[3][threadIdx.x]);
}

template <class T, class TO = T>
__global__ __launch_bounds__(256) void qk_norm_rope_kernel(const T* __restrict__ qkv, int ldqkv, const float* __restrict__ wq,
                                                           const float* __restrict__ wk, const float* __restrict__ table,
                                                           TO* __restrict__ out, int ldo, int B, int L, int H, int hd, float eps,
                                                           float q_scale) {
    const int lane = threadIdx.x & 63;
    const long m = (long)blockIdx.x * 4 + (threadIdx.x >> 6);
    if (m >= (long)B * L) return;
    const int l = (int)(m % L);
    const int lph = hd / 8, half = lph / 2;
    const int nchunks = 2 * H * lph;
    const int niter = (nchunks + 63) / 64;
    for (int it = 0; it < niter; it++) {
        const int q = it * 64 + lane;
        const bool act = q < nchunks;
        const int slot = q / lph, c8 = q % lph;
        float v[8];
        if (act) od_ld8(qkv + m * ldqkv + (size_t)slot * hd + c8 * 8, v);
        else {
#pragma unroll
            for (int e = 0; e < 8; e++) v[e] = 0.f;
        }
        float ss = 0.f;
#pragma unroll
        for (int e = 0; e < 8; e++) ss += v[e] * v[e];
        for (int msk = 1; msk < lph; msk <<= 1) ss += __shfl_xor(ss, msk);
        const float inv = rsqrtf(ss / (float)hd + eps);
        const float* w = (slot < H ? wq : wk) + c8 * 8;
        float y[8], p[8];
#pragma unroll
        for (int e = 0; e < 8; e++) y[e] = act ? v[e] * inv * w[e] : 0.f;
#pragma unroll
        for (int e = 0; e < 8; e++) p[e] = __shfl_xor(y[e], half);
        if (act) {
            const bool first = c8 < half;
            const int j0 = (c8 % half) * 8;
            const float* tb = table + ((size_t)l * (hd / 2) + j0) * 2;
            float o[8];
#pragma unroll
            for (int e = 0; e < 8; e++) {
                const float cs = tb[2 * e], sn = tb[2 * e + 1];
                o[e] = (first ? (y[e] * cs - p[e] * sn) : (p[e] * sn + y[e] * cs)) * (slot < H ? q_scale : 1.f);
            }
            od_st8(out + m * ldo + (size_t)slot * hd + c8 * 8, o);
        }
    }
}

template <class T>
__global__ __launch_bounds__(256) void qk_norm_rope_bwd_kernel(const T* __restrict__ qkv, int ldqkv, const float* __restrict__ wq,
                                                               const float* __restrict__ wk, const float* __restrict__ table,
                                                               const T* __restrict__ dqk, int lddqk, T* __restrict__ dqkv, int lddqkv,
                                                               float* __restrict__ dwq, float* __restrict__ dwk,
                                                               int B, int L, int H, int hd, float eps, float q_scale,
                                                               const OdDetTable* __restrict__ det) {
    __shared__ long long sdw[2][256];
    __shared__ int s_bad;
    const int lane = threadIdx.x & 63, wave = threadIdx.x >> 6;
    for (int i = threadIdx.x; i < 512; i += 256) sdw[i >> 8][i & 255] = 0;
    if (threadIdx.x == 0) s_bad = 0;
    __syncthreads();
    const int lph = hd / 8, half = lph / 2;
    const int nchunks = 2 * H * lph;
    const int niter = (nchunks + 63) / 64;
    float aq[8], ak[8];
#pragma unroll
    for (int e = 0; e < 8; e++) { aq[e] = 0.f; ak[e] = 0.f; }
    const long M = (long)B * L;
    const long mbase = ((long)blockIdx.x * 4 + wave) * ROWS_PER_WAVE_BWD;
    for (int r = 0; r < ROWS_PER_WAVE_BWD; r++) {
        const long m = mbase + r;
        if (m >= M) break;
        const int l = (int)(m % L);
        for (int it = 0; it < niter; it++) {
            const int q = it * 64 + lane;
            const bool act = q < nchunks;
            const int slot = q / lph, c8 = q % lph;
            float v[8], d[8];
            if (act) {
                od_ld8(qkv + m * ldqkv + (size_t)slot * hd + c8 * 8, v); od_ld8(dqk + m * lddqk + (size_t)slot * hd + c8 * 8, d);
                if (slot < H) {
#pragma unroll
                    for (int e = 0; e < 8; e++) d[e] *= q_scale;
                }
            } else {
#pragma unroll
                for (int e = 0; e < 8; e++) { v[e] = 0.f; d[e] = 0.f; }
            }
            float ss = 0.f;
#pragma unroll
            for (int e = 0; e < 8; e++) ss += v[e] * v[e];
            for (int msk = 1; msk < lph; msk <<= 1) ss += __shfl_xor(ss, msk);
            const float inv = rsqrtf(ss / (float)hd + eps);
            float p[8], dy[8];
#pragma unroll
            for (int e = 0; e < 8; e++) p[e] = __shfl_xor(d[e], half);
            const bool first = c8 < half;
            const int j0 = (c8 % (half > 0 ? half : 1)) * 8;
            const float* tb = table + ((size_t)l * (hd / 2) + j0) * 2;
            const float* w = (slot < H ? wq : wk) + c8 * 8;
            float dot = 0.f;
#pragma unroll
            for (int e = 0; e < 8; e++) {
                const float cs = act ? tb[2 * e] : 0.f, sn = act ? tb[2 * e + 1] : 0.f;
                dy[e] = first ? (d[e] * cs + p[e] * sn) : (-p[e] * sn + d[e] * cs);
                const float xh = v[e] * inv;
                const float wv = act ? w[e] : 0.f;
                if (act) { if (slot < H) aq[e] += dy[e] * xh; else ak[e] += dy[e] * xh; }
                dy[e] *= wv;
                dot += dy[e] * xh;
                v[e] = xh;
            }
            for (int msk = 1; msk < lph; msk <<= 1) dot += __shfl_xor(dot, msk);
            dot /= (float)hd;
            if (act) {
                float o[8];
#pragma unroll
                for (int e = 0; e < 8; e++) o[e] = inv * (dy[e] - v[e] * dot);
                od_st8(dqkv + m * lddqkv + (size_t)slot * hd + c8 * 8, o);
            }
        }
    }
    const int c8 = lane % lph;
#pragma unroll
    for (int e = 0; e < 8; e++) {
        od_lds_fix_add(&sdw[0][c8 * 8 + e], aq[e], &s_bad);
        od_lds_fix_add(&sdw[1][c8 * 8 + e], ak[e], &s_bad);
    }
    __syncthreads();
    if (threadIdx.x < hd) {
        od_red_add(det, dwq + threadIdx.x, od_lds_unfix(sdw[0][threadIdx.x], s_bad));
        od_red_add(det, dwk + threadIdx.x, od_lds_unfix(sdw[1][threadIdx.x], s_bad));
    }
}

template <class T, int LPH, int NIT>
__global__ __launch_bounds__(256) void qk_norm_rope_pos_kernel(const T* __restrict__ qkv, int ldqkv, const float* __restrict__ wq,
                                                               const float* __restrict__ wk, const float* __restrict__ table,
// ... 129 lines not shown

__global__ void rope_table_kernel(float* __restrict__ table, int L, int hd) {
    const long i = (long)blockIdx.x * blockDim.x + threadIdx.x;
    const int half = hd / 2;
    if (i >= (long)L * half) return;
    const int l = (int)(i / half), j = (int)(i % half);
    const float e = (float)(2 * j) / (float)(-hd);
    const float inv_freq = (float)pow(10000.0, (double)e);
    const float ang = (float)l * inv_freq;
    table[2 * i] = cosf(ang);
    table[2 * i + 1] = sinf(ang);
}

inline int nch_for(int C) { return (C + 511) / 512; }

inline void qk_pos_split(int B, int L, int& bpw, int& lpw) {
    bpw = B < OD_QK_BPW ? B : OD_QK_BPW;
    lpw = OD_QK_BPW / bpw;
    if (lpw < 1) lpw = 1;
    (void)L;
}

}

#define DISPATCH_T_NCH(DT, NCHV, CALL)                                          \
    do {                                                                        \
        if ((DT) == OD_BF16) {                                                  \
            typedef bf16_t T_;                                                  \
            if ((NCHV) == 1) { constexpr int N_ = 1; CALL; }                    \
            else if ((NCHV) == 2) { constexpr int N_ = 2; CALL; }               \
            else if ((NCHV) == 3) { constexpr int N_ = 3; CALL; }               \
            else return OD_ERR_UNSUPPORTED;                                     \
        } else if ((DT) == OD_F32) {                                            \
            typedef float T_;                                                   \
            if ((NCHV) == 1) { constexpr int N_ = 1; CALL; }                    \
            else if ((NCHV) == 2) { constexpr int N_ = 2; CALL; }               \
            else if ((NCHV) == 3) { constexpr int N_ = 3; CALL; }               \
            else return OD_ERR_UNSUPPORTED;                                     \
        } else return OD_ERR_ARG;                                               \
    } while (0)

extern "C" int od_rmsnorm_film(int dtype, const void* x, int ldx, const float* ssg, const void* cl, int ldcl, int cl_bcast,
                               void* h, int ldh, float* inv_rms, int B, int L, int C, float eps, void* stream) {
    if (C % 8 || ldx % 8 || ldh % 8 || (cl && ldcl % 8)) return OD_ERR_ALIGN;
    const long M = (long)B * L;
    dim3 grid((unsigned)((M + 3) / 4));
    DISPATCH_T_NCH(dtype, nch_for(C),
        OD_LAUNCH((rmsnorm_film_kernel<T_, N_>), grid, dim3(256), 0, (hipStream_t)stream, (const T_*)x, ldx, ssg, (const T_*)cl, ldcl,
                  cl_bcast, (T_*)h, ldh, inv_rms, B, L, C, eps));
    OD_CHECK_LAUNCH();
    return 0;
}

extern "C" int od_rmsnorm_film_bwd(int dtype, const void* x, int ldx, const float* inv_rms, const float* ssg, const void* dh,
                                   int lddh, void* dres, int lddres, float* dssg, int B, int L, int C, void* stream) {
    if (C % 8 || ldx % 8 || lddh % 8 || lddres % 8) return OD_ERR_ALIGN;
    dim3 grid((L + 4 * ROWS_PER_WAVE_BWD - 1) / (4 * ROWS_PER_WAVE_BWD), B);
    DISPATCH_T_NCH(dtype, nch_for(C),
        OD_LAUNCH((rmsnorm_film_bwd_kernel<T_, N_>), grid, dim3(256), 0, (hipStream_t)stream, (const T_*)x, ldx, inv_rms, ssg,
                  (const T_*)dh, lddh, (T_*)dres, lddres, dssg, B, L, C, od_det_active()));
    OD_CHECK_LAUNCH();
    return 0;
}

extern "C" int od_rmsnorm_gate_residual(int dtype, const void* x, int ldx, const void* h, int ldh, const float* ssg, void* xo,
                                        int ldxo, float* inv_rms, int B, int L, int C, float eps, void* stream) {
    if (C % 8 || ldx % 8 || ldh % 8 || ldxo % 8) return OD_ERR_ALIGN;
    const long M = (long)B * L;
    dim3 grid((unsigned)((M + 3) / 4));
    DISPATCH_T_NCH(dtype, nch_for(C),
        OD_LAUNCH((rmsnorm_gate_res_kernel<T_, N_>), grid, dim3(256), 0, (hipStream_t)stream, (const T_*)x, ldx, (const T_*)h, ldh, ssg,
                  (T_*)xo, ldxo, inv_rms, B, L, C, eps));
    OD_CHECK_LAUNCH();
    return 0;
}

extern "C" int od_rmsnorm_gate_residual_film(int dtype, const void* x, int ldx, const void* h, int ldh, const float* ssg_a, void* xo,
                                             int ldxo, float* inv_a, const float* ssg_b, const void* cl, int ldcl, int cl_bcast,
                                             void* h2, int ldh2, float* inv_b, int B, int L, int C, float eps, void* stream) {
    if (C % 8 || ldx % 8 || ldh % 8 || ldxo % 8 || ldh2 % 8 || (cl && ldcl % 8)) return OD_ERR_ALIGN;
    const long M = (long)B * L;
    dim3 grid((unsigned)((M + 3) / 4));
    DISPATCH_T_NCH(dtype, nch_for(C),
        OD_LAUNCH((rmsnorm_gate_res_film_kernel<T_, N_>), grid, dim3(256), 0, (hipStream_t)stream, (const T_*)x, ldx, (const T_*)h, ldh,
                  ssg_a, (T_*)xo, ldxo, inv_a, ssg_b, (const T_*)cl, ldcl, cl_bcast, (T_*)h2, ldh2, inv_b, B, L, C, eps));
    OD_CHECK_LAUNCH();
    return 0;
}

extern "C" int od_rmsnorm_gate_residual_film_dwconv(int dtype, const void* x, int ldx, const void* h, int ldh, const float* ssg_a, void* xo,
                                                    int ldxo, float* inv_a, const float* ssg_b, void* h2, int ldh2, float* inv_b,
                                                    const float* conv_w, const float* conv_b, void* y, int ldy, int B, int L, int C,
                                                    int ksize, float eps, void* stream) {
    if (C % 8 || ldx % 8 || ldh % 8 || ldxo % 8 || (h2 && ldh2 % 8) || ldy % 8) return OD_ERR_ALIGN;
    if (C > 512 || (ksize != 3 && ksize != 5 && ksize != 7 && ksize != 9)) return OD_ERR_UNSUPPORTED;
    if (!x || !h || !xo || !y || !conv_w || !conv_b || xo == x || xo == h) return OD_ERR_ARG;
#ifndef OD_FD_SMALL_RUNS
#define OD_FD_SMALL_RUNS 2048
#endif
    const bool small = (long)B * ((L + 31) / 32) < OD_FD_SMALL_RUNS;
    const int run = small ? 8 : 32;
    dim3 grid((unsigned)((L + 4 * run - 1) / (4 * run)), (unsigned)B);
#define FD_GO2(T_, KS_, RUN_) OD_LAUNCH((rmsnorm_gate_res_film_dwconv_kernel<T_, KS_, RUN_>), grid, dim3(256), 0, (hipStream_t)stream, (const T_*)x, ldx, \
                   (const T_*)h, ldh, ssg_a, (T_*)xo, ldxo, inv_a, ssg_b, (T_*)h2, ldh2, inv_b, conv_w, conv_b, (T_*)y, ldy, B, L, C, eps)
#define FD_GO1(T_, KS_) do { if (small) FD_GO2(T_, KS_, 8); else FD_GO2(T_, KS_, 32); } while (0)
#define FD_GO(KS_) do { if (dtype == OD_BF16) FD_GO1(bf16_t, KS_); else if (dtype == OD_F32) FD_GO1(float, KS_); else return OD_ERR_UNSUPPORTED; } while (0)
    if (ksize == 5) FD_GO(5); else if (ksize == 3) FD_GO(3); else if (ksize == 7) FD_GO(7); else FD_GO(9);
#undef FD_GO
#undef FD_GO1
#undef FD_GO2
    OD_CHECK_LAUNCH();
    return 0;
}

extern "C" int od_rmsnorm_gate_residual_bwd(int dtype, const void* h, int ldh, const float* inv_rms, const float* ssg,
                                            const void* dy, int lddy, void* dh, int lddh, float* dssg, int B, int L, int C,
                                            void* stream) {
    if (C % 8 || ldh % 8 || lddy % 8 || lddh % 8) return OD_ERR_ALIGN;
    dim3 grid((L + 4 * ROWS_PER_WAVE_BWD - 1) / (4 * ROWS_PER_WAVE_BWD), B);
    DISPATCH_T_NCH(dtype, nch_for(C),
        OD_LAUNCH((rmsnorm_gate_res_bwd_kernel<T_, N_>), grid, dim3(256), 0, (hipStream_t)stream, (const T_*)h, ldh, inv_rms, ssg,
                  (const T_*)dy, lddy, (T_*)dh, lddh, dssg, B, L, C, od_det_active()));
    OD_CHECK_LAUNCH();
    return 0;
}

extern "C" int od_swiglu_rmsnorm(int dtype, const void* vg, int ldvg, void* hh, int ldhh, float* inv_rms, int M, int Hf, int Hp,
                                 float eps, void* stream) {
    if (Hp % 8 || ldvg % 8 || ldhh % 8 || Hf > Hp) return OD_ERR_ALIGN;
    dim3 grid((unsigned)((M + 3) / 4));
    DISPATCH_T_NCH(dtype, nch_for(Hp),
        OD_LAUNCH((swiglu_rmsnorm_kernel<T_, N_>), grid, dim3(256), 0, (hipStream_t)stream, (const T_*)vg, ldvg, (T_*)hh, ldhh, inv_rms,
                  (long)M, Hf, Hp, eps));
    OD_CHECK_LAUNCH();
    return 0;
}

extern "C" int od_swiglu_rmsnorm_bwd(int dtype, const void* vg, int ldvg, const float* inv_rms, const void* dhh, int lddhh,
                                     void* dvg, int lddvg, int M, int Hf, int Hp, void* stream) {
    if (Hp % 8 || ldvg % 8 || lddhh % 8 || lddvg % 8 || Hf > Hp) return OD_ERR_ALIGN;
    dim3 grid((unsigned)((M + 3) / 4));
    DISPATCH_T_NCH(dtype, nch_for(Hp),
        OD_LAUNCH((swiglu_rmsnorm_bwd_kernel<T_, N_>), grid, dim3(256), 0, (hipStream_t)stream, (const T_*)vg, ldvg, inv_rms,
                  (const T_*)dhh, lddhh, (T_*)dvg, lddvg, (long)M, Hf, Hp));
    OD_CHECK_LAUNCH();
    return 0;
}

extern "C" int od_final_norm_proj_out(int dtype, const void* x, int ldx, const float* W, const float* bias, float* v,
                                      float* inv_rms, int B, int L, int C, int E, float eps, void* stream) {
    if (C % 8 || ldx % 8) return OD_ERR_ALIGN;
    if (E > 8 || C > 1024) return OD_ERR_UNSUPPORTED;
    const long M = (long)B * L;
    dim3 grid((unsigned)((M + 3) / 4));
    DISPATCH_T_NCH(dtype, nch_for(C),
        OD_LAUNCH((final_proj_kernel<T_, N_>), grid, dim3(256), 0, (hipStream_t)stream, (const T_*)x, ldx, W, bias, v, inv_rms, B, L, C, E, eps));
    OD_CHECK_LAUNCH();
    return 0;
}

extern "C" int od_final_norm_proj_out_bwd(int dtype, const void* x, int ldx, const float* inv_rms, const float* W,
                                          const float* dv, void* dx, int lddx, float* dW, float* db, int B, int L, int C, int E,
                                          void* stream) {
    if (C % 8 || ldx % 8 || lddx % 8) return OD_ERR_ALIGN;
    if (E > 8 || C > 512) return OD_ERR_UNSUPPORTED;
    dim3 grid((L + 4 * ROWS_PER_WAVE_BWD - 1) / (4 * ROWS_PER_WAVE_BWD), B);
    if (dtype == OD_BF16)
        OD_LAUNCH((final_proj_bwd_kernel<bf16_t, 1>), grid, dim3(256), 0, (hipStream_t)stream, (const bf16_t*)x, ldx, inv_rms, W, dv,
                  (bf16_t*)dx, lddx, dW, db, B, L, C, E, od_det_active());
    else
        OD_LAUNCH((final_proj_bwd_kernel<float, 1>), grid, dim3(256), 0, (hipStream_t)stream, (const float*)x, ldx, inv_rms, W, dv,
                  (float*)dx, lddx, dW, db, B, L, C, E, od_det_active());
    OD_CHECK_LAUNCH();
    return 0;
}

extern "C" int od_rope_table(float* table, int L, int hd, void* stream) {
    if (hd % 2 || L <= 0) return OD_ERR_ARG;
    const long n = (long)L * (hd / 2);
    OD_LAUNCH(rope_table_kernel, dim3((unsigned)((n + 255) / 256)), dim3(256), 0, (hipStream_t)stream, table, L, hd);
    OD_CHECK_LAUNCH();
    return 0;
}

extern "C" int od_qk_norm_rope(int dtype, const void* qkv, int ldqkv, const float* wq, const float* wk, const float* table,
                               void* qk_out, int ldo, int B, int L, int H, int hd, float eps, float q_scale, void* stream) {
    if (hd % 16 || hd > 256 || 64 % (hd / 8)) return OD_ERR_UNSUPPORTED;
    if (ldqkv % 8 || ldo % 8) return OD_ERR_ALIGN;
    const long M = (long)B * L;
    const int lph = hd / 8;
    if (dtype != OD_F16 && (lph == 4 || lph == 8) && (H * lph) % 64 == 0 && ldqkv >= 2 * H * hd) {
        const int nit = 2 * H * lph / 64;
        if (nit == 2 || nit == 4 || nit == 8) {
            int bpw, lpw; qk_pos_split(B, L, bpw, lpw);
            const long waves = (long)((L + lpw - 1) / lpw) * ((B + bpw - 1) / bpw);
            dim3 g2((unsigned)((waves + 3) / 4));
#define QKP(TT, LPHV, NITV) OD_LAUNCH((qk_norm_rope_pos_kernel<TT, LPHV, NITV>), g2, dim3(256), 0, (hipStream_t)stream, (const TT*)qkv, ldqkv, wq, wk, table, (TT*)qk_out, ldo, B, L, eps, q_scale, bpw, lpw)
#define QKP_T(TT) do { if (lph == 8) { if (nit == 2) QKP(TT, 8, 2); else if (nit == 4) QKP(TT, 8, 4); else QKP(TT, 8, 8); } \
                       else { if (nit == 2) QKP(TT, 4, 2); else if (nit == 4) QKP(TT, 4, 4); else QKP(TT, 4, 8); } } while (0)
            if (dtype == OD_BF16) QKP_T(bf16_t); else QKP_T(float);
#undef QKP_T
#undef QKP
            OD_CHECK_LAUNCH();
            return 0;
        }
    }
    dim3 grid((unsigned)((M + 3) / 4));
    if (dtype == OD_F16)
        OD_LAUNCH((qk_norm_rope_kernel<bf16_t, f16_t>), grid, dim3(256), 0, (hipStream_t)stream, (const bf16_t*)qkv, ldqkv, wq, wk, table,
                  (f16_t*)qk_out, ldo, B, L, H, hd, eps, q_scale);
    else if (dtype == OD_BF16)
        OD_LAUNCH((qk_norm_rope_kernel<bf16_t>), grid, dim3(256), 0, (hipStream_t)stream, (const bf16_t*)qkv, ldqkv, wq, wk, table,
                  (bf16_t*)qk_out, ldo, B, L, H, hd, eps, q_scale);
    else
        OD_LAUNCH((qk_norm_rope_kernel<float>), grid, dim3(256), 0, (hipStream_t)stream, (const float*)qkv, ldqkv, wq, wk, table,
                  (float*)qk_out, ldo, B, L, H, hd, eps, q_scale);
    OD_CHECK_LAUNCH();
    return 0;
}

extern "C" int od_qk_norm_rope_bwd(int dtype, const void* qkv, int ldqkv, const float* wq, const float* wk, const float* table,
                                   const void* dqk, int lddqk, void* dqkv, int lddqkv, float* dwq, float* dwk, int B, int L,
                                   int H, int hd, float eps, float q_scale, void* stream) {
    if (hd % 16 || hd > 256 || 64 % (hd / 8)) return OD_ERR_UNSUPPORTED;
    if (ldqkv % 8 || lddqk % 8 || lddqkv % 8) return OD_ERR_ALIGN;
    const long M = (long)B * L;
    const int lph = hd / 8;
    if ((lph == 4 || lph == 8) && (H * lph) % 64 == 0) {
        const int nit = 2 * H * lph / 64;
        if (nit == 2 || nit == 4 || nit == 8) {
            int bpw, lpw; qk_pos_split(B, L, bpw, lpw);
            lpw *= 4;
            const long waves = (long)((L + lpw - 1) / lpw) * ((B + bpw - 1) / bpw);
            dim3 g2((unsigned)((waves + 3) / 4));
#define QKPB(TT, LPHV, NITV) OD_LAUNCH((qk_norm_rope_pos_bwd_kernel<TT, LPHV, NITV>), g2, dim3(256), 0, (hipStream_t)stream, (const TT*)qkv, ldqkv, wq, wk, table, (const TT*)dqk, lddqk, (TT*)dqkv, lddqkv, dwq, dwk, B, L, eps, q_scale, bpw, lpw, od_det_active())
#define QKPB_T(TT) do { if (lph == 8) { if (nit == 2) QKPB(TT, 8, 2); else if (nit == 4) QKPB(TT, 8, 4); else QKPB(TT, 8, 8); } \
                        else { if (nit == 2) QKPB(TT, 4, 2); else if (nit == 4) QKPB(TT, 4, 4); else QKPB(TT, 4, 8); } } while (0)
            if (dtype == OD_BF16) QKPB_T(bf16_t); else QKPB_T(float);
#undef QKPB_T
#undef QKPB
            OD_CHECK_LAUNCH();
            return 0;
        }
    }
    dim3 grid((unsigned)((M + 4 * ROWS_PER_WAVE_BWD - 1) / (4 * ROWS_PER_WAVE_BWD)));
    if (dtype == OD_BF16)
        OD_LAUNCH((qk_norm_rope_bwd_kernel<bf16_t>), grid, dim3(256), 0, (hipStream_t)stream, (const bf16_t*)qkv, ldqkv, wq, wk, table,
                  (const bf16_t*)dqk, lddqk, (bf16_t*)dqkv, lddqkv, dwq, dwk, B, L, H, hd, eps, q_scale, od_det_active());
    else
        OD_LAUNCH((qk_norm_rope_bwd_kernel<float>), grid, dim3(256), 0, (hipStream_t)stream, (const float*)qkv, ldqkv, wq, wk, table,
                  (const float*)dqk, lddqk, (float*)dqkv, lddqkv, dwq, dwk, B, L, H, hd, eps, q_scale, od_det_active());
    OD_CHECK_LAUNCH();
    return 0;
}
```

### osu_dreamer_amd/engine.py

```python
from __future__ import annotations


import math
import os
from typing import Dict, List, Optional

import torch

from . import det, ops
from ._lib import OD_ACT_NONE, OD_ACT_SILU

OD_FUSE_FILM_DWCONV_DEFAULT = "0"

FP32_EPS = float(torch.finfo(torch.float32).eps)


def _ceil(x: int, m: int) -> int:
    return (x + m - 1) // m * m


class Workspace:

    def __init__(self, device):
        self.device = device
        self.t: Dict[str, torch.Tensor] = {}
        self.bytes = 0

    def get(self, name: str, shape, dtype) -> torch.Tensor:
        t = self.t.get(name)
        if t is None:
            t = torch.zeros(shape, dtype=dtype, device=self.device)
            self.t[name] = t
            self.bytes += t.numel() * t.element_size()
            if name in det.WS_NAMES:
                ctx = det.context(self.device)
                if ctx is not None:
                    ctx.register(t)
        return t


class DenoiserEngine:
    def __init__(self, model):
        self.model = model
        a = model.args
        ba = a.backbone_args
        self.E, self.A, self.S = model.emb_dim, model.a_dim, model.style_dim
        self.Cg, self.D, self.U = a.global_cond_dim, a.backbone_dim, a.u_head_dim
        self.H, self.hd, self.depth = ba.n_heads, ba.head_dim, ba.depth
        self.dh = self.H * self.hd
        self.q_scale = math.log2(math.e) / math.sqrt(self.hd)
        self.radius = ba.radius
        self.ksize = 1 + 2 * ba.radius
        self.Hf = int(self.D * ba.expand * 2 / 3)
        self.Hp = _ceil(self.Hf, 64)
        if ba.radius not in (0, 1, 2, 3, 4):
            raise NotImplementedError("depthwise kernel sizes 3, 5, 7, 9 (radius 1-4) are compiled; radius 0 is the identity")
        if not (0.0 <= ba.dropout < 1.0):
            raise ValueError(f"dropout probability has to be in [0, 1), got {ba.dropout}")
        self.dropout = float(ba.dropout)
        self._packed: Dict[str, torch.Tensor] = {}
        self._packed_key = None
        self._plan_key = None
        self.ws: Optional[Workspace] = None
        self._rowmap = None
        self.generation = 0
        self._attn_aux = None
        self._attn_ws_cache: Dict[tuple, "ops.FusedAttnBwdWorkspace"] = {}
        self._attn_ws = None
        self.varlen = False
        self.attn_f16 = False

    def _det_flush(self, *tensors):
        ctx = det.context(self.model.arena.data.device)
        if ctx is not None:
            for t in tensors:
                ctx.flush(t)

    def _det_flush_segment(self, name: str):
        ctx = det.context(self.model.arena.data.device)
        if ctx is not None:
            s, e = self.model.arena.segments(self.depth)[name]
            ctx.flush(self.model.arena.ensure_grad()[s:e])

    def P(self, name: str) -> torch.Tensor:
        return self.model.arena.view(name)

    def G(self, name: str) -> torch.Tensor:
        return self.model.arena.grad_view(name)

    def _gemm_weights(self) -> List[str]:
        names = ["proj_audio.0"]
        for i in range(self.depth):
            p = f"net.layers.{i}."
            names += [p + "proj_cl", p + "attn.qkv_proj", p + "attn.out_proj", p + "ffn.proj_vg.1", p + "ffn.proj_o"]
        return names

    def pack_weights(self, dtype: torch.dtype, train: bool, x3: bool = False):
        dev = self.model.arena.data.device
        x3 = bool(x3 and dtype == torch.float32 and not train)
        key = (dtype, train, dev, x3)
        if self._packed_key != key:
            self._packed = {}
            self._packed_key = key
            self.generation += 1
            Hf, Hp = self.Hf, self.Hp
            rm = [-1] * (2 * Hp)
            for j in range(Hf):
                rm[j] = j
                rm[Hp + j] = Hf + j
            self._rowmap = torch.tensor(rm, dtype=torch.int32, device=dev)
        pk = self._packed
        for n in self._gemm_weights():
            w = self.P(n + ".weight")
            N, K = w.shape[0], w.shape[1]
            Np, Kp, rmap = N, K, None
            if n.endswith("ffn.proj_vg.1"):
                Np, rmap = 2 * self.Hp, self._rowmap
            if n.endswith("ffn.proj_o"):
                Kp = self.Hp
            if n not in pk:
                pk[n] = torch.empty(Np, Kp, dtype=dtype, device=dev)
                if x3 and Kp % 32 == 0:
                    pk[n] = ops.SplitWeight(pk[n])
                if train:
                    pk[n + ".T"] = torch.empty(Kp, Np, dtype=dtype, device=dev)
                if rmap is not None:
                    pk[n + ".b"] = torch.empty(Np, dtype=torch.float32, device=dev)
            ops.pack_weight(w, pk[n], row_map=rmap)
            if train:
                ops.pack_weight(w, pk[n + ".T"], transpose=True, row_map=rmap)
            if rmap is not None:
                ops.pack_weight(self.P(n + ".bias"), pk[n + ".b"].view(Np, 1), row_map=rmap)

    def W(self, name: str, T: bool = False) -> torch.Tensor:
        return self._packed[name + (".T" if T else "")]

    def plain_gemm(self, A: torch.Tensor, W: torch.Tensor, bias, C: torch.Tensor):
        ops.gemm_nt(A, W, bias, C, x3=self.x3)

    def plan(self, B: int, L: int, Ba: int, dtype: torch.dtype, train: bool, x3: bool = False, lens=None, offs=None):
        dev = self.model.arena.data.device
        assert not (x3 and train), "the f32x3 product exists for the forward kernels only"
        varlen = lens is not None
        x3 = bool(x3 and dtype == torch.float32)
        ngroups = len(offs) - 1 if offs is not None else 0
        key = (B, L, Ba, dtype, train, dev, x3, getattr(self.model, "attn_dtype", None), varlen, ngroups)
        if key != self._plan_key:
            self.ws = Workspace(dev)
            self._plan_key = key
            self.generation += 1
            tab = self.ws.get("rope", (L, self.hd // 2, 2), torch.float32)
            ops.rope_table(tab, L, self.hd)
        self.varlen = varlen
        if varlen:
            lens_t = torch.as_tensor(lens).to("cpu", torch.int32)
            if lens_t.shape != (B,) or int(lens_t.min()) < 1 or int(lens_t.max()) > L:
                raise ValueError(f"lens must hold B = {B} lengths in [1, {L}]")
            self.ws.get("vl.lens", (B,), torch.int32).copy_(lens_t)
            if offs is not None:
                offs_t = torch.as_tensor(offs).to("cpu", torch.int32)
                if int(offs_t[0]) != 0 or int(offs_t[-1]) != B or bool((offs_t[1:] <= offs_t[:-1]).any()):
                    raise ValueError("offs must rise strictly from 0 to B")
                self.ws.get("vl.offs", (ngroups + 1,), torch.int32).copy_(offs_t)
        self.B, self.L, self.Ba, self.dtype, self.train, self.x3 = B, L, Ba, dtype, train, x3
        self.M, self.Ma = B * L, Ba * L
        self.attn_f16 = getattr(self.model, "attn_dtype", None) == torch.float16
        if self.attn_f16 and (dtype != torch.bfloat16 or self.hd != 64):
            if not getattr(self, "_warned_f16_fallback", False):
                import warnings
                warnings.warn(f"attn_dtype = float16 applies to compute_dtype bfloat16 with head_dim 64; this plan (dtype {dtype}, head_dim "
                              f"{self.hd}) runs its attention in {dtype}")
                self._warned_f16_fallback = True
            self.attn_f16 = False
        if varlen and train and self.attn_f16:
            raise NotImplementedError("ragged training has no half-operand attention (attn_dtype = float16 runs the fused backward, which has no "
                                      "varlen form): train ragged batches with attn_dtype = None")
        return self.ws

    def buf(self, name, shape, dtype=None):
        return self.ws.get(name, shape, self.dtype if dtype is None else dtype)

    def lbuf(self, name, i, shape, dtype=None):
        return self.buf(f"{name}.{i}" if self.train else name, shape, dtype)

    def conditioning(self, audio: torch.Tensor, style: torch.Tensor):
        B, Ba, L = self.B, self.Ba, self.L
        D, A, Cg, U = self.D, self.A, self.Cg, self.U
        f32 = torch.float32
        a_t = self.buf("a_t", (self.Ma, A))
        a_pre = self.buf("a_pre", (self.Ma, A))
        a = self.buf("a", (self.Ma, A))
        ops.cl_to_frames(audio, a_t)
        ops.gemm_nt(a_t, self.W("proj_audio.0"), self.P("proj_audio.0.bias"), a_pre, x3=self.x3)
        ops.silu(a_pre, a)
        cg, cg_pre = self.buf("cg", (B, Cg), f32), self.buf("cg_pre", (B, Cg), f32)
        ops.linear_small(style, self.P("proj_style.0.weight"), self.P("proj_style.0.bias"), cg, cg_pre, OD_ACT_SILU)
        for i in range(self.depth):
            p = f"net.layers.{i}."
            for s in ("ssg1", "ssg2"):
                ops.linear_small(cg, self.P(p + s + ".weight"), self.P(p + s + ".bias"),
                                 self.buf(f"{s}.{i}", (B, 3 * D), f32))
            if not self.train:
                ops.gemm_nt(a, self.W(p + "proj_cl"), self.P(p + "proj_cl.bias"), self.buf(f"cl.{i}", (self.Ma, D)), x3=self.x3)
        ops.linear_small(cg, self.P("u_mod.weight"), self.P("u_mod.bias"), self.buf("umod", (B, 2 * U), f32))

    def pred(self, xt: torch.Tensor, u: torch.Tensor, v: torch.Tensor):
        B, L, M, D, dh, Hp = self.B, self.L, self.M, self.D, self.dh, self.Hp
        f32 = torch.float32
        tab = self.ws.t["rope"]
        bcast = self.Ba == 1 and B > 1
        x = self.lbuf("x_in", 0, (M, D))
        ops.proj_in(xt, self.P("proj_in.weight"), self.P("proj_in.bias"), x)

        def cl_of(i):
            if not self.train:
                return self.ws.t[f"cl.{i}"]
            cl = self.buf("cl", (self.Ma, D))
            ops.gemm_nt(self.ws.t["a"], self.W(f"net.layers.{i}.proj_cl"), self.P(f"net.layers.{i}.proj_cl.bias"), cl)
            return cl

        h1 = self.lbuf("h1", 0, (M, D))
        ops.rmsnorm_film(x, self.ws.t["ssg1.0"], cl_of(0), bcast, h1, self.lbuf("inv1", 0, (M,), f32), B, L)
        for i in range(self.depth):
            p = f"net.layers.{i}."
            ssg1, ssg2 = self.ws.t[f"ssg1.{i}"], self.ws.t[f"ssg2.{i}"]
            qkv = self.lbuf("qkv", i, (M, 3 * dh))
            if self.train or self.attn_f16 or self.hd not in (32, 64) or (2 * dh) % 128:
                qk = self.lbuf("qk16" if self.attn_f16 else "qk", i, (M, 2 * dh), torch.float16 if self.attn_f16 else None)
                ops.gemm_nt_qkrope_split(h1, self.W(p + "attn.qkv_proj"), self.P(p + "attn.qkv_proj.bias"), qkv, qk,
                                         self.P(p + "attn.q_norm.weight"), self.P(p + "attn.k_norm.weight"), tab, L, self.H,
                                         self.hd, FP32_EPS, x3=self.x3, q_scale=self.q_scale)
            else:
                ops.gemm_nt_qkrope(h1, self.W(p + "attn.qkv_proj"), self.P(p + "attn.qkv_proj.bias"), qkv,
                                   self.P(p + "attn.q_norm.weight"), self.P(p + "attn.k_norm.weight"), tab, L,
                                   self.H, self.hd, FP32_EPS, x3=self.x3, q_scale=self.q_scale)
                qk = qkv
            y = self.lbuf("y", i, (M, dh))
            lse = self.lbuf("lse", i, (B, self.H, L), f32)
            if self.varlen:
                ops.flash_attn_fwd_varlen(qk[:, :dh], qk[:, dh:], self._v_of(qkv), y, lse, self.ws.t["vl.lens"], B, self.H, L, self.hd,
                                          1.0 / math.sqrt(self.hd), x3=self.x3, q_prescaled=True)
            else:
                ops.flash_attn_fwd(qk[:, :dh], qk[:, dh:], self._v_of(qkv), y, lse, B, self.H, L, self.hd,
                                   1.0 / math.sqrt(self.hd), x3=self.x3, q_prescaled=True)
            ao = self.lbuf("ao", i, (M, D))
            self.plain_gemm(y, self.W(p + "attn.out_proj"), self.P(p + "attn.out_proj.bias"), ao)
            x_mid = self.lbuf("x_mid", i, (M, D))
            h2 = self.lbuf("h2", i, (M, D))
            fuse_dw = (self.radius > 0 and not self.varlen and D <= 512 and x.data_ptr() != x_mid.data_ptr() and x.dtype in (torch.bfloat16, torch.float32)
                       and os.environ.get("OD_FUSE_FILM_DWCONV", OD_FUSE_FILM_DWCONV_DEFAULT) == "1")
            if fuse_dw:
                hdw = self.lbuf("hdw", i, (M, D))
                ops.rmsnorm_gate_residual_film_dwconv(x, ao, ssg1, x_mid, self.lbuf("inv2", i, (M,), f32), ssg2, h2 if self.train else None,
                                                      self.lbuf("inv3", i, (M,), f32),
                                                      self.P(p + "ffn.proj_vg.0.weight"), self.P(p + "ffn.proj_vg.0.bias"), hdw, B, L, self.ksize)
            else:
                ops.rmsnorm_gate_residual_film(x, ao, ssg1, x_mid, self.lbuf("inv2", i, (M,), f32), ssg2, None, False, h2,
                                               self.lbuf("inv3", i, (M,), f32), B, L)
            if fuse_dw:
                pass
            elif self.radius > 0:
                hdw = self.lbuf("hdw", i, (M, D))
                if self.varlen:
                    ops.dwconv_varlen(h2, self.P(p + "ffn.proj_vg.0.weight"), self.P(p + "ffn.proj_vg.0.bias"), hdw, self.ws.t["vl.lens"], B, L,
                                      self.ksize)
                else:
                    ops.dwconv(h2, self.P(p + "ffn.proj_vg.0.weight"), self.P(p + "ffn.proj_vg.0.bias"), hdw, B, L, self.ksize)
            else:
                hdw = h2
            vg = self.lbuf("vg", i, (M, 2 * Hp))
            ops.gemm_nt(hdw, self.W(p + "ffn.proj_vg.1"), self._packed[p + "ffn.proj_vg.1.b"], vg, x3=self.x3)
            hh = self.lbuf("hh", i, (M, Hp))
            ops.swiglu_rmsnorm(vg, hh, self.lbuf("inv4", i, (M,), f32), self.Hf, Hp)
            if self._drop_active():
                ops.scale_channels(hh, self.draw_dropout_mask(i), B, L)
            fo = self.lbuf("fo", i, (M, D))
            self.plain_gemm(hh, self.W(p + "ffn.proj_o"), self.P(p + "ffn.proj_o.bias"), fo)
            x = self.buf(f"x_in.{i + 1}", (M, D)) if self.train else self.buf(f"x_in.{(i + 1) & 1}", (M, D))
            if i + 1 < self.depth:
                h1 = self.lbuf("h1", i + 1, (M, D))
                ops.rmsnorm_gate_residual_film(x_mid, fo, ssg2, x, self.lbuf("inv5", i, (M,), f32),
                                               self.ws.t[f"ssg1.{i + 1}"], cl_of(i + 1), bcast, h1,
                                               self.lbuf("inv1", i + 1, (M,), f32), B, L)
            else:
                ops.rmsnorm_gate_residual(x_mid, fo, ssg2, x, self.lbuf("inv5", i, (M,), f32), B, L)
        self._x_last = x
        ops.final_norm_proj_out(x, self.P("proj_out.weight"), self.P("proj_out.bias"), v,
                                self.buf("invf", (M,), f32), B, L)
        fsum = self.buf("fsum", (B, self.U), f32)
        fsum.zero_()
        if self.varlen:
            ops.uhead_fwd_varlen(xt, self._uhead_w(), fsum, self.ws.t["vl.lens"], self.U)
            self._det_flush(fsum)
            ops.uhead_tail_varlen(fsum, self.ws.t["umod"], self.P("u_out.weight"), self.P("u_out.bias"), u, self.ws.t["vl.lens"], L,
                                  self.model.u_scale)
        else:
            ops.uhead_fwd(xt, self._uhead_w(), fsum, self.U)
            self._det_flush(fsum)
            ops.uhead_tail(fsum, self.ws.t["umod"], self.P("u_out.weight"), self.P("u_out.bias"), u, L, self.model.u_scale)

    def _v_of(self, qkv: torch.Tensor) -> torch.Tensor:
        v = qkv[:, 2 * self.dh:]
        return v.view(torch.float16) if self.attn_f16 else v

    def attn_bwd_passes(self) -> int:
        from . import _lib
        return int(_lib.lib().cdll.od_flash_attn_bwd_fused_passes() if self.fused_attn_bwd() else _lib.lib().cdll.od_flash_attn_bwd_passes())

    def fused_attn_bwd(self) -> bool:
        import os
        if self.dtype != torch.bfloat16 or self.hd != 64 or self.varlen:
            return False
        if self.attn_f16:
            return True
        env = os.environ.get("OD_ATTN_BWD_FUSED", "")
        if env in ("0", "1"):
            return env == "1"
        return self.L >= 2048

    def attn_bwd_launch(self, i: int, dy: torch.Tensor, delta: torch.Tensor, dqkv: torch.Tensor, core_only: bool = False):
        t, dh, p = self.ws.t, self.dh, f"net.layers.{i}."
        qk, qkv, y, lse = t[f"qk16.{i}" if self.attn_f16 else f"qk.{i}"], t[f"qkv.{i}"], t[f"y.{i}"], t[f"lse.{i}"]
        wq, wk = self.P(p + "attn.q_norm.weight"), self.P(p + "attn.k_norm.weight")
        gq, gk = self.G(p + "attn.q_norm.weight"), self.G(p + "attn.k_norm.weight")
        scale = 1.0 / math.sqrt(self.hd)
        dqk = self.buf("d.qk", (self.M, 2 * dh))
        if self.fused_attn_bwd():
            key = (self.B, self.H, self.L, qk.device, qk.dtype)
            ws = self._attn_ws_cache.get(key)
            if ws is None:
                if len(self._attn_ws_cache) >= 4:
                    self._attn_ws_cache.pop(next(iter(self._attn_ws_cache)))
                ws = self._attn_ws_cache[key] = ops.FusedAttnBwdWorkspace(self.B, self.H, self.L, qk.device, qk.dtype)
                ws.checked = False
            self._attn_ws = ws
            ops.flash_attn_bwd_fused(qk[:, :dh], qk[:, dh:], self._v_of(qkv), y, dy, lse, dqk[:, :dh], dqk[:, dh:], dqkv[:, 2 * dh:],
                                     self.B, self.H, self.L, self.hd, scale, self._attn_ws, q_prescaled=True)
        else:
            if (self._attn_aux is None or self._attn_aux.device != qk.device) and qk.is_cuda:
                if self._attn_aux is not None:
                    self._attn_aux.close()
                with torch.cuda.device(qk.device):
                    self._attn_aux = ops.AttnAux()
                self._attn_aux.device = qk.device
            if self.varlen:
                ops.flash_attn_bwd_varlen(qk[:, :dh], qk[:, dh:], qkv[:, 2 * dh:], y, dy, lse, delta, dqk[:, :dh], dqk[:, dh:],
                                          dqkv[:, 2 * dh:], self.ws.t["vl.lens"], self.B, self.H, self.L, self.hd, scale, q_prescaled=True,
                                          aux=self._attn_aux)
            else:
                ops.flash_attn_bwd(qk[:, :dh], qk[:, dh:], qkv[:, 2 * dh:], y, dy, lse, delta, dqk[:, :dh], dqk[:, dh:],
                                   dqkv[:, 2 * dh:], self.B, self.H, self.L, self.hd, scale, q_prescaled=True, aux=self._attn_aux)
        if not core_only:
            ops.qk_norm_rope_bwd(qkv, wq, wk, t["rope"], dqk, dqkv, gq, gk, self.B, self.L, self.H, self.hd, FP32_EPS, q_scale=self.q_scale)

    def _drop_active(self) -> bool:
        return self.dropout > 0.0 and self.model.training

# ... 134 lines not shown
```

### osu_dreamer_amd/ops.py

```python
from __future__ import annotations

import os
from typing import Optional

import torch

from . import _lib
from ._lib import OD_ACT_NONE, OD_ACT_SILU, OD_BF16, OD_EPI_NONE, OD_EPI_SILU, OD_F32, OD_F32X3, OD_F32X3W


def dt_code(dtype: torch.dtype) -> int:
    if dtype == torch.float32:
        return OD_F32
    if dtype == torch.bfloat16:
        return OD_BF16
    if dtype == torch.float16:
        return _lib.OD_F16
    raise TypeError(f"unsupported compute dtype {dtype}")


class SplitWeight:

    def __init__(self, storage: torch.Tensor):
        self.t = storage


def mm_code(dtype: torch.dtype, x3: bool, w=None) -> int:
    if isinstance(w, SplitWeight):
        if not (x3 and dtype == torch.float32):
            raise ValueError("a pre-split weight can only feed the fp32-as-3-x-bf16 product")
        return OD_F32X3W
    return OD_F32X3 if (x3 and dtype == torch.float32) else dt_code(dtype)


def _w(W):
    return W.t if isinstance(W, SplitWeight) else W


def _stream(t: torch.Tensor) -> int:
    return torch.cuda.current_stream(t.device).cuda_stream if t.is_cuda else 0


def _p(t: Optional[torch.Tensor]) -> Optional[int]:
    return None if t is None else t.data_ptr()


def _ld(t: torch.Tensor) -> int:
    assert t.dim() == 2 and t.stride(1) == 1, "need a row-major 2-D view"
    return t.stride(0)


def _f32(*ts):
    for t in ts:
        assert t is None or (t.dtype == torch.float32 and t.is_contiguous()), "expected contiguous fp32"


def _i32(*ts):
    for t in ts:
        assert t.dtype == torch.int32 and t.is_contiguous(), "expected contiguous int32"


def gemm_nt(A, W, bias, C, epilogue=OD_EPI_NONE, accumulate=False, x3=False):
    code, W = mm_code(A.dtype, x3, W), _w(W)
    M, K = A.shape
    N = W.shape[0]
    assert W.shape[1] == K and tuple(C.shape) == (M, N)
    assert A.dtype == W.dtype == C.dtype
    _f32(bias)
    _lib.lib().od_gemm_nt(code, _p(A), _ld(A), _p(W), _ld(W), _p(bias), _p(C), _ld(C), M, N, K,
                          epilogue, int(accumulate), _stream(A))


def gemm_nt_qkrope(A, W, bias, C, wq, wk, table, L, H, hd, eps, x3=False, q_scale=1.0):
    code, W = mm_code(A.dtype, x3, W), _w(W)
    M, K = A.shape
    N = W.shape[0]
    assert W.shape[1] == K and tuple(C.shape) == (M, N) and A.dtype == W.dtype == C.dtype
    _f32(bias, wq, wk, table)
    _lib.lib().od_gemm_nt_qkrope(code, _p(A), _ld(A), _p(W), _ld(W), _p(bias), _p(C), _ld(C), M, N, K,
                                 _p(wq), _p(wk), _p(table), L, H, hd, eps, q_scale, _stream(A))


def gemm_nt_qkrope_split(A, W, bias, C, qk_out, wq, wk, table, L, H, hd, eps, x3=False, q_scale=1.0):
    code, W = mm_code(A.dtype, x3, W), _w(W)
    M, K = A.shape
    N = W.shape[0]
    assert W.shape[1] == K and tuple(C.shape) == (M, N) and tuple(qk_out.shape) == (M, 2 * H * hd)
    assert A.dtype == W.dtype == C.dtype
    assert qk_out.dtype == A.dtype or (qk_out.dtype == torch.float16 and A.dtype == torch.bfloat16)
    _f32(bias, wq, wk, table)
    qk_code = _lib.OD_F16 if qk_out.dtype == torch.float16 else (OD_F32 if A.dtype == torch.float32 else code)
    _lib.lib().od_gemm_nt_qkrope_split(code, _p(A), _ld(A), _p(W), _ld(W), _p(bias), _p(C), _ld(C), _p(qk_out),
                                       _ld(qk_out), qk_code, M, N, K, _p(wq), _p(wk), _p(table), L, H, hd, eps, q_scale, _stream(A))


def gemm_tn(G, A, dW, n_cols=None, k_cols=None, dbias=None, n_block=0, n_valid=0):
    M = G.shape[0]
    N = n_cols if n_cols is not None else G.shape[1]
    K = k_cols if k_cols is not None else A.shape[1]
    rows = N if not n_block else (N // n_block) * n_valid
    assert not n_block or N % n_block == 0
    assert dW.dtype == torch.float32 and dW.is_contiguous() and dW.numel() == rows * K
    _f32(dbias)
    _lib.lib().od_gemm_tn_blocks(dt_code(G.dtype), _p(G), _ld(G), _p(A), _ld(A), _p(dW), K, _p(dbias), M, N, K, n_block, n_valid, _stream(G))


def colsum(G, out, n_cols=None):
    M = G.shape[0]
    N = n_cols if n_cols is not None else G.shape[1]
    _f32(out)
    _lib.lib().od_colsum(dt_code(G.dtype), _p(G), _ld(G), _p(out), M, N, _stream(G))


def pack_weight(src, dst, transpose=False, row_map=None):
    N = src.shape[0]
    K = src.numel() // N
    _f32(src)
    code = OD_F32X3W if isinstance(dst, SplitWeight) else dt_code(_w(dst).dtype)
    dst = _w(dst)
    if transpose:
        Kp, Np = dst.shape
    else:
        Np, Kp = dst.shape
    assert dst.is_contiguous()
    _lib.lib().od_pack_weight(code, _p(src), N, K, _p(dst), Np, Kp, int(transpose), _p(row_map), _stream(src))


def linear_small(x, W, b, out, pre=None, act=OD_ACT_NONE):
    B, K = x.shape
    N = W.shape[0]
    _f32(x, W, b, out, pre)
    _lib.lib().od_linear_small(_p(x), _p(W), _p(b), _p(out), _p(pre), B, N, K, act, _stream(x))


def linear_small_bwd(x, W, pre, dout, dpre, dW, db, dx, accumulate_dx, act=OD_ACT_NONE):
    B, K = x.shape
    N = W.shape[0]
    _f32(x, W, pre, dout, dpre, dW, db, dx)
    _lib.lib().od_linear_small_bwd(_p(x), _p(W), _p(pre), _p(dout), _p(dpre), _p(dW), _p(db), _p(dx),
                                   int(accumulate_dx), B, N, K, act, _stream(x))


def cl_to_frames(src, dst):
    B, C, L = src.shape
    _f32(src)
    _lib.lib().od_cl_to_frames(dt_code(dst.dtype), _p(src), _p(dst), _ld(dst), B, C, L, _stream(src))


def proj_in(xt, W, bias, x):
    B, E, L = xt.shape
    D = x.shape[1]
    _f32(xt, W, bias)
    _lib.lib().od_proj_in(dt_code(x.dtype), _p(xt), _p(W), _p(bias), _p(x), _ld(x), B, E, L, D, _stream(xt))


def proj_in_bwd(xt, dx, dW, db):
    B, E, L = xt.shape
    D = dx.shape[1]
    _f32(xt, dW, db)
    _lib.lib().od_proj_in_bwd(dt_code(dx.dtype), _p(xt), _p(dx), _ld(dx), _p(dW), _p(db), B, E, L, D, _stream(xt))


def silu(x, y):
    assert x.is_contiguous() and y.is_contiguous()
    _lib.lib().od_silu(dt_code(x.dtype), _p(x), _p(y), x.numel(), _stream(x))


def silu_bwd(x, dy, dx):
    assert x.is_contiguous() and dy.is_contiguous() and dx.is_contiguous()
    _lib.lib().od_silu_bwd(dt_code(x.dtype), _p(x), _p(dy), _p(dx), x.numel(), _stream(x))


def rmsnorm_film(x, ssg, cl, cl_bcast, h, inv_rms, B, L, eps=1e-6):
    C = x.shape[1]
    _f32(ssg, inv_rms)
    _lib.lib().od_rmsnorm_film(dt_code(x.dtype), _p(x), _ld(x), _p(ssg), _p(cl), _ld(cl) if cl is not None else 0,
                               int(cl_bcast), _p(h), _ld(h), _p(inv_rms), B, L, C, eps, _stream(x))


def rmsnorm_film_bwd(x, inv_rms, ssg, dh, dres, dssg, B, L):
    C = x.shape[1]
    _f32(ssg, inv_rms, dssg)
    _lib.lib().od_rmsnorm_film_bwd(dt_code(x.dtype), _p(x), _ld(x), _p(inv_rms), _p(ssg), _p(dh), _ld(dh), _p(dres),
                                   _ld(dres), _p(dssg), B, L, C, _stream(x))


def rmsnorm_gate_residual(x, h, ssg, xo, inv_rms, B, L, eps=1e-6):
    C = x.shape[1]
    _f32(ssg, inv_rms)
    _lib.lib().od_rmsnorm_gate_residual(dt_code(x.dtype), _p(x), _ld(x), _p(h), _ld(h), _p(ssg), _p(xo), _ld(xo),
                                        _p(inv_rms), B, L, C, eps, _stream(x))


def rmsnorm_gate_residual_film(x, h, ssg_a, xo, inv_a, ssg_b, cl, cl_bcast, h2, inv_b, B, L, eps=1e-6):
    _f32(ssg_a, ssg_b, inv_a, inv_b)
    _lib.lib().od_rmsnorm_gate_residual_film(dt_code(x.dtype), _p(x), _ld(x), _p(h), _ld(h), _p(ssg_a), _p(xo), _ld(xo),
                                             _p(inv_a), _p(ssg_b), _p(cl), _ld(cl) if cl is not None else 0, int(cl_bcast),
                                             _p(h2), _ld(h2), _p(inv_b), B, L, x.shape[1], eps, _stream(x))


def rmsnorm_gate_residual_film_dwconv(x, h, ssg_a, xo, inv_a, ssg_b, h2, inv_b, conv_w, conv_b, y, B, L, ksize, eps=1e-6):
    _f32(ssg_a, ssg_b, inv_a, inv_b, conv_w, conv_b)
    assert xo.data_ptr() != x.data_ptr() and xo.data_ptr() != h.data_ptr()
    _lib.lib().od_rmsnorm_gate_residual_film_dwconv(dt_code(x.dtype), _p(x), _ld(x), _p(h), _ld(h), _p(ssg_a), _p(xo), _ld(xo), _p(inv_a),
                                                    _p(ssg_b), _p(h2), _ld(h2) if h2 is not None else 0, _p(inv_b), _p(conv_w), _p(conv_b),
                                                    _p(y), _ld(y), B, L, x.shape[1], ksize, eps, _stream(x))


def rmsnorm_gate_residual_bwd(h, inv_rms, ssg, dy, dh, dssg, B, L):
    C = h.shape[1]
    _f32(ssg, inv_rms, dssg)
    _lib.lib().od_rmsnorm_gate_residual_bwd(dt_code(h.dtype), _p(h), _ld(h), _p(inv_rms), _p(ssg), _p(dy), _ld(dy),
                                            _p(dh), _ld(dh), _p(dssg), B, L, C, _stream(h))


def rope_table(table, L, hd):
    _f32(table)
    _lib.lib().od_rope_table(_p(table), L, hd, _stream(table))


def qk_norm_rope(qkv, wq, wk, table, qk_out, B, L, H, hd, eps, q_scale=1.0):
    _f32(wq, wk, table)
    _lib.lib().od_qk_norm_rope(dt_code(qkv.dtype), _p(qkv), _ld(qkv), _p(wq), _p(wk), _p(table), _p(qk_out),
                               _ld(qk_out), B, L, H, hd, eps, q_scale, _stream(qkv))


def qk_norm_rope_bwd(qkv, wq, wk, table, dqk, dqkv, dwq, dwk, B, L, H, hd, eps, q_scale=1.0):
    _f32(wq, wk, table, dwq, dwk)
    _lib.lib().od_qk_norm_rope_bwd(dt_code(qkv.dtype), _p(qkv), _ld(qkv), _p(wq), _p(wk), _p(table), _p(dqk), _ld(dqk),
                                   _p(dqkv), _ld(dqkv), _p(dwq), _p(dwk), B, L, H, hd, eps, q_scale, _stream(qkv))


def flash_attn_fwd(q, k, v, o, lse, B, H, L, hd, scale, x3=False, q_prescaled=False):
    _f32(lse)
    assert q.dtype == k.dtype == v.dtype and (o.dtype == q.dtype or (q.dtype == torch.float16 and o.dtype == torch.bfloat16))
    _lib.lib().od_flash_attn_fwd(mm_code(q.dtype, x3), _p(q), _ld(q), _p(k), _ld(k), _p(v), _ld(v), _p(o), _ld(o), _p(lse),
                                 B, H, L, hd, scale, int(q_prescaled), _stream(q))


class AttnAux:

    def __init__(self):
        import ctypes
        self.handle = ctypes.c_void_p()
        _lib.lib().od_attn_aux_create(ctypes.byref(self.handle))

    def close(self):
        if self.handle:
            _lib.lib().od_attn_aux_destroy(self.handle)
            self.handle = None

    def __del__(self):
        try:
            self.close()
        except Exception:
            pass


def flash_attn_fwd_varlen(q, k, v, o, lse, lens, B, H, L, hd, scale, x3=False, q_prescaled=False):
    _f32(lse)
    _i32(lens)
    assert q.dtype == k.dtype == v.dtype and (o.dtype == q.dtype or (q.dtype == torch.float16 and o.dtype == torch.bfloat16))
    _lib.lib().od_flash_attn_fwd_varlen(mm_code(q.dtype, x3), _p(q), _ld(q), _p(k), _ld(k), _p(v), _ld(v), _p(o), _ld(o), _p(lse),
                                        _p(lens), B, H, L, hd, scale, int(q_prescaled), _stream(q))


def flash_attn_bwd(q, k, v, o, do, lse, delta, dq, dk, dv, B, H, L, hd, scale, q_prescaled=False, aux=None):
    _f32(lse, delta)
    _lib.lib().od_flash_attn_bwd_aux(dt_code(q.dtype), _p(q), _ld(q), _p(k), _ld(k), _p(v), _ld(v), _p(o), _ld(o), _p(do),
                                     _ld(do), _p(lse), _p(delta), _p(dq), _ld(dq), _p(dk), _ld(dk), _p(dv), _ld(dv),
                                     B, H, L, hd, scale, int(q_prescaled), aux.handle if aux is not None else None, _stream(q))


def flash_attn_bwd_varlen(q, k, v, o, do, lse, delta, dq, dk, dv, lens, B, H, L, hd, scale, q_prescaled=False, aux=None):
    _f32(lse, delta)
    _i32(lens)
    _lib.lib().od_flash_attn_bwd_varlen(dt_code(q.dtype), _p(q), _ld(q), _p(k), _ld(k), _p(v), _ld(v), _p(o), _ld(o), _p(do),
                                        _ld(do), _p(lse), _p(delta), _p(dq), _ld(dq), _p(dk), _ld(dk), _p(dv), _ld(dv), _p(lens),
                                        B, H, L, hd, scale, int(q_prescaled), aux.handle if aux is not None else None, _stream(q))


class FusedAttnBwdWorkspace:

    def __init__(self, B, H, L, device, dtype=torch.bfloat16):
        import ctypes
# ... 525 lines not shown
```

Baseline: 3.238.

## Batch small linears and weight packing, restructure u-head and projection backward kernels

Several independent changes land together. The per-layer FiLM modulation linears are batched into one multi-job launch, and weight packing becomes a single multi-job kernel. The u-head forward and backward kernels now use transposed, padded w4 in shared memory with vectorized loads, register accumulation in place of shared atomics, and a 4x4 register tile for dw4. The proj_in and final_proj backward kernels are templated on the embedding count and software-pipelined over frame chunks. The goal is to cut launch overhead, shared-memory atomics and redundant loads, at the cost of more template instantiations and higher register pressure.

```diff
diff --git a/include/osu_dreamer_hip.h b/include/osu_dreamer_hip.h
--- a/include/osu_dreamer_hip.h
+++ b/include/osu_dreamer_hip.h
@@ -32,9 +32,13 @@
 int od_colsum(int dtype, const void* G, int ldg, float* out, int M, int N, void* stream);
 int od_pack_weight(int dtype, const float* src, int N, int K, void* dst, int Np, int Kp, int transpose,
                    const int* row_map, void* stream);
+int od_pack_weights_multi(int njobs, const void* src, const void* dst, const void* dst_T, const int* dims, const int* row_map,
+                          void* stream);
 
 int od_linear_small(const float* x, const float* W, const float* b, float* out, float* pre, int B, int N, int K, int act,
                     void* stream);
+int od_linear_small_multi(const float* x, int njobs, const void* W, const void* bias, const void* out, const int* N, int B, int K,
+                          void* stream);
 int od_linear_small_bwd(const float* x, const float* W, const float* pre, const float* dout, float* dpre, float* dW,
                         float* db, float* dx, int accumulate_dx, int B, int N, int K, int act, void* stream);
 
diff --git a/osu_dreamer_amd/csrc/heads.hip b/osu_dreamer_amd/csrc/heads.hip
--- a/osu_dreamer_amd/csrc/heads.hip
+++ b/osu_dreamer_amd/csrc/heads.hip
@@ -18,15 +18,18 @@
     const float *w0, *b0, *w1, *b1, *w3, *b3, *w4, *b4;
 };
 
+constexpr int UZS = UW + 4;
+constexpr int UWS = MAXU + 4;
 struct UHeadSmem {
     float xts[MAXE][UW + 4];
     float z0s[MAXE][UW + 2];
     float z1s[MAXU][UW + 2];
     float a1s[MAXU][UW + 2];
-    float z3s[MAXU][UW + 1];
-    float g4s[MAXU][UW + 1];
-    float w4s[MAXU][MAXU + 1];
+    __attribute__((aligned(16))) float z3s[MAXU][UZS];
+    __attribute__((aligned(16))) float g4s[MAXU][UZS];
+    __attribute__((aligned(16))) float w4t[MAXU][UWS];
 };
+__device__ __forceinline__ int uhead_pad(int c, int cpg) { return 8 * (c / cpg) + c % cpg; }
 
 __device__ __forceinline__ void uhead_window_fwd(UHeadSmem& S, const float* __restrict__ xt, const UHeadW& P, int b, int l0,
                                                  int E, int L, int U, int Lv) {
@@ -59,8 +62,21 @@
 }
 
 __device__ __forceinline__ void uhead_load_w4(UHeadSmem& S, const UHeadW& P, int U) {
-    for (int idx = threadIdx.x; idx < U * U; idx += 256) S.w4s[idx / U][idx % U] = P.w4[idx];
-    __syncthreads();
+    const int cpg = U / 8;
+    for (int idx = threadIdx.x; idx < MAXU * UWS; idx += 256) (&S.w4t[0][0])[idx] = 0.f;
+    __syncthreads();
+    for (int idx = threadIdx.x; idx < U * U; idx += 256) S.w4t[idx % U][uhead_pad(idx / U, cpg)] = P.w4[idx];
+    __syncthreads();
+}
+__device__ __forceinline__ void uhead_z4(const UHeadSmem& S, int U, int grp, int i, const float (&b4v)[8], float (&z)[8]) {
+#pragma unroll
+    for (int q = 0; q < 8; q++) z[q] = b4v[q];
+    for (int cc = 0; cc < U; cc++) {
+        const float zv = S.z3s[cc][i];
+        const f32x4 wa = *(const f32x4*)&S.w4t[cc][grp * 8], wb = *(const f32x4*)&S.w4t[cc][grp * 8 + 4];
+#pragma unroll
+        for (int q = 0; q < 4; q++) { z[q] += wa[q] * zv; z[4 + q] += wb[q] * zv; }
+    }
 }
 
 template <bool VL = false>
@@ -72,9 +88,9 @@
     const int Lb = VL ? od_uniform(lens[b]) : L;
     const int i = t & 31, grp = t >> 5, cpg = U / 8;
     uhead_load_w4(S, P, U);
-    float acc[MAXU / 8];
-#pragma unroll
-    for (int q = 0; q < MAXU / 8; q++) acc[q] = 0.f;
+    float acc[MAXU / 8], b4v[MAXU / 8];
+#pragma unroll
+    for (int q = 0; q < MAXU / 8; q++) { acc[q] = 0.f; b4v[q] = q < cpg ? P.b4[grp * cpg + q] : 0.f; }
     for (int wi = 0; wi < wpb; wi++) {
         const int win = blockIdx.x * wpb + wi;
         if (win >= nwin) break;
@@ -83,15 +99,11 @@
         uhead_window_fwd(S, xt, P, b, l0, E, L, U, Lb);
         const int f = l0 - 1 + i;
         const bool own = (i >= 1 && i < UW - 1 && f < Lb);
-#pragma unroll
-        for (int q = 0; q < MAXU / 8; q++) {
-            if (q < cpg) {
-                const int c = grp * cpg + q;
-                float z = P.b4[c];
-                for (int cc = 0; cc < U; cc++) z += S.w4s[c][cc] * S.z3s[cc][i];
-                if (own) acc[q] += od_silu(z);
-            }
-        }
+        float z[MAXU / 8];
+        uhead_z4(S, U, grp, i, b4v, z);
+#pragma unroll
+        for (int q = 0; q < MAXU / 8; q++)
+            if (q < cpg && own) acc[q] += od_silu(z[q]);
         __syncthreads();
     }
 #pragma unroll
@@ -114,17 +126,32 @@
     const int b = blockIdx.y, t = threadIdx.x;
     const int i = t & 31, grp = t >> 5, cpg = U / 8;
     const int Lb = VL ? od_uniform(lens[b]) : L;
-    for (int idx = t; idx < MAXU; idx += 256) {
-        sdb3[idx] = 0.f; sdb4[idx] = 0.f; sdb1[idx] = 0.f;
-        for (int j = 0; j < 3; j++) sdw3[idx][j] = 0.f;
-        for (int e = 0; e < MAXE; e++) sdw1[idx][e] = 0.f;
-    }
-    if (t < MAXE) { sdb0[t] = 0.f; for (int j = 0; j < 3; j++) sdw0[t][j] = 0.f; }
+    for (int idx = t; idx < MAXU * UZS; idx += 256) (&S.g4s[0][0])[idx] = 0.f;
     uhead_load_w4(S, P, U);
-    float adw4[16];
-#pragma unroll
-    for (int q = 0; q < 16; q++) adw4[q] = 0.f;
     const float invL = 1.0f / (float)Lb;
+    float rdb4[8], rdb3[8], rdw3[8][3], rdb1[8], rdw1[8][MAXE], rdb0 = 0.f, rdw0[3] = {0.f, 0.f, 0.f};
+    float b4v[8], dfv[8], w3v[8][3];
+#pragma unroll
+    for (int q = 0; q < 8; q++) {
+        const int c = grp * cpg + q;
+        rdb4[q] = 0.f; rdb3[q] = 0.f; rdb1[q] = 0.f;
+        b4v[q] = q < cpg ? P.b4[c] : 0.f;
+        dfv[q] = q < cpg ? dfm[(size_t)b * U + c] * invL : 0.f;
+#pragma unroll
+        for (int j = 0; j < 3; j++) { rdw3[q][j] = 0.f; w3v[q][j] = q < cpg ? P.w3[c * 3 + j] : 0.f; }
+#pragma unroll
+        for (int e = 0; e < MAXE; e++) rdw1[q][e] = 0.f;
+    }
+    const int tc = (t >> 4) * 4, tcc = (t & 15) * 4;
+    const bool tile = tc < U && tcc < U;
+    float adw4[4][4];
+#pragma unroll
+    for (int a = 0; a < 4; a++)
+#pragma unroll
+        for (int a2 = 0; a2 < 4; a2++) adw4[a][a2] = 0.f;
+    int prow[4];
+#pragma unroll
+    for (int a = 0; a < 4; a++) prow[a] = tile ? uhead_pad(tc + a, cpg) : 0;
 
     for (int wi = 0; wi < UWPB; wi++) {
         const int win = blockIdx.x * UWPB + wi;
@@ -135,95 +162,131 @@
         const int f = l0 - 1 + i;
         const bool inr = (f >= 0 && f < Lb);
         const bool own = (i >= 1 && i < UW - 1 && f < Lb);
-#pragma unroll
-        for (int q = 0; q < MAXU / 8; q++) {
-            if (q < cpg) {
-                const int c = grp * cpg + q;
-                float z = P.b4[c];
-                for (int cc = 0; cc < U; cc++) z += S.w4s[c][cc] * S.z3s[cc][i];
-                const float g = inr ? dfm[(size_t)b * U + c] * invL * od_silu_grad(z) : 0.f;
-                S.g4s[c][i] = g;
-                const float s = red32(own ? g : 0.f);
-                if (i == 0) atomicAdd(&sdb4[c], s);
-            }
-        }
-        __syncthreads();
         {
-            const int iend = (Lb - (l0 - 1)) < (UW - 1) ? (Lb - (l0 - 1)) : (UW - 1);
-#pragma unroll
-            for (int q = 0; q < 16; q++) {
-                const int o = t + 256 * q;
-                if (o < U * U) {
-                    const int c = o / U, cc = o % U;
-                    float s = 0.f;
-                    for (int ii = 1; ii < iend; ii++) s += S.g4s[c][ii] * S.z3s[cc][ii];
-                    adw4[q] += s;
+            float z[8];
+            uhead_z4(S, U, grp, i, b4v, z);
+#pragma unroll
+            for (int q = 0; q < 8; q++) {
+                if (q < cpg) {
+                    const float g = inr ? dfv[q] * od_silu_grad(z[q]) : 0.f;
+                    S.g4s[grp * 8 + q][i] = g;
+                    rdb4[q] += own ? g : 0.f;
                 }
             }
         }
         __syncthreads();
-        float dz3v[MAXU / 8];
-#pragma unroll
-        for (int q = 0; q < MAXU / 8; q++) {
-            dz3v[q] = 0.f;
-            if (q < cpg) {
-                const int cc = grp * cpg + q;
-                float s = 0.f;
-                for (int c = 0; c < U; c++) s += S.w4s[c][cc] * S.g4s[c][i];
-                dz3v[q] = s;
+        if (tile) {
+            const int iend = (Lb - (l0 - 1)) < (UW - 1) ? (Lb - (l0 - 1)) : (UW - 1);
+            for (int i4 = 0; i4 < UW; i4 += 4) {
+                if (i4 >= iend) break;
+                f32x4 gv[4], zv[4];
+#pragma unroll
+                for (int a = 0; a < 4; a++) {
+                    gv[a] = *(const f32x4*)&S.g4s[prow[a]][i4];
+                    zv[a] = *(const f32x4*)&S.z3s[tcc + a][i4];
+#pragma unroll
+                    for (int k = 0; k < 4; k++)
+                        if (i4 + k < 1 || i4 + k >= iend) zv[a][k] = 0.f;
+                }
+#pragma unroll
+                for (int a = 0; a < 4; a++)
+#pragma unroll
+                    for (int a2 = 0; a2 < 4; a2++)
+#pragma unroll
+                        for (int k = 0; k < 4; k++) adw4[a][a2] += gv[a][k] * zv[a2][k];
             }
         }
         __syncthreads();
-#pragma unroll
-        for (int q = 0; q < MAXU / 8; q++)
-            if (q < cpg) S.z3s[grp * cpg + q][i] = dz3v[q];
-        __syncthreads();
-#pragma unroll
-        for (int q = 0; q < MAXU / 8; q++) {
-            if (q < cpg) {
-                const int c = grp * cpg + q;
-                const float g = own ? S.z3s[c][i] : 0.f;
-                float s = red32(g);
-                if (i == 0) atomicAdd(&sdb3[c], s);
-                for (int j = 0; j < 3; j++) {
-                    s = red32(g * S.a1s[c][i + j]);
-                    if (i == 0) atomicAdd(&sdw3[c][j], s);
-                }
-                float dz1 = 0.f;
-                if (own) {
-                    float da1 = 0.f;
-                    for (int j = 0; j < 3; j++) da1 += P.w3[c * 3 + j] * S.z3s[c][i - j + 1];
-                    dz1 = da1 * od_silu_grad(S.z1s[c][i + 1]);
-                }
-                S.g4s[c][i] = dz1;
-                s = red32(dz1);
-                if (i == 0) atomicAdd(&sdb1[c], s);
-                for (int e = 0; e < E; e++) {
-                    s = red32(dz1 * S.z0s[e][i + 1]);
-                    if (i == 0) atomicAdd(&sdw1[c][e], s);
+        float dz3v[8];
+#pragma unroll
+        for (int q = 0; q < 8; q++) dz3v[q] = 0.f;
+        for (int p = 0; p < MAXU; p += 4) {
+            const float g0 = S.g4s[p][i], g1 = S.g4s[p + 1][i], g2 = S.g4s[p + 2][i], g3 = S.g4s[p + 3][i];
+#pragma unroll
+            for (int q = 0; q < 8; q++) {
+                if (q < cpg) {
+                    const f32x4 w = *(const f32x4*)&S.w4t[grp * cpg + q][p];
+                    dz3v[q] += w[0] * g0; dz3v[q] += w[1] * g1; dz3v[q] += w[2] * g2; dz3v[q] += w[3] * g3;
                 }
             }
         }
         __syncthreads();
-        {
-            const bool ev = grp < E;
-            const int e = ev ? grp : 0;
-            float dz0 = 0.f;
-            if (ev)
-                for (int c = 0; c < U; c++) dz0 += P.w1[c * E + e] * S.g4s[c][i];
-            float s = red32(dz0);
-            if (ev && i == 0) atomicAdd(&sdb0[e], s);
-            for (int j = 0; j < 3; j++) {
-                s = red32(dz0 * S.xts[e][i + 1 + j]);
-                if (ev && i == 0) atomicAdd(&sdw0[e][j], s);
+#pragma unroll
+        for (int q = 0; q < 8; q++)
+            if (q < cpg) S.z3s[grp * cpg + q][i] = dz3v[q];
+        __syncthreads();
+#pragma unroll
+        for (int q = 0; q < 8; q++) {
+            if (q < cpg) {
+                const int c = grp * cpg + q;
+                const float g = own ? S.z3s[c][i] : 0.f;
+                rdb3[q] += g;
+#pragma unroll
+                for (int j = 0; j < 3; j++) rdw3[q][j] += g * S.a1s[c][i + j];
+                float dz1 = 0.f;
+                if (own) {
+                    float da1 = 0.f;
+#pragma unroll
+                    for (int j = 0; j < 3; j++) da1 += w3v[q][j] * S.z3s[c][i - j + 1];
+                    dz1 = da1 * od_silu_grad(S.z1s[c][i + 1]);
+                }
+                S.g4s[grp * 8 + q][i] = dz1;
+                rdb1[q] += dz1;
+#pragma unroll
+                for (int e = 0; e < MAXE; e++)
+                    if (e < E) rdw1[q][e] += dz1 * S.z0s[e][i + 1];
             }
         }
         __syncthreads();
-    }
-#pragma unroll
-    for (int q = 0; q < 16; q++) {
-        const int o = t + 256 * q;
-        if (o < U * U) od_red_add(det, G.dw4 + o, adw4[q]);
+        if (grp < E) {
+            const int e = grp;
+            float dz0 = 0.f;
+            for (int c = 0; c < U; c++) dz0 += P.w1[c * E + e] * S.g4s[uhead_pad(c, cpg)][i];
+            rdb0 += dz0;
+#pragma unroll
+            for (int j = 0; j < 3; j++) rdw0[j] += dz0 * S.xts[e][i + 1 + j];
+        }
+        __syncthreads();
+    }
+#pragma unroll
+    for (int q = 0; q < 8; q++) {
+        if (q < cpg) {
+            const int c = grp * cpg + q;
+            float s = red32(rdb4[q]);
+            if (i == 0) sdb4[c] = s;
+            s = red32(rdb3[q]);
+            if (i == 0) sdb3[c] = s;
+            s = red32(rdb1[q]);
+            if (i == 0) sdb1[c] = s;
+#pragma unroll
+            for (int j = 0; j < 3; j++) {
+                s = red32(rdw3[q][j]);
+                if (i == 0) sdw3[c][j] = s;
+            }
+#pragma unroll
+            for (int e = 0; e < MAXE; e++) {
+                if (e < E) {
+                    s = red32(rdw1[q][e]);
+                    if (i == 0) sdw1[c][e] = s;
+                }
+            }
+        }
+    }
+    {
+        const bool ev = grp < E;
+        float s = red32(rdb0);
+        if (ev && i == 0) sdb0[grp] = s;
+#pragma unroll
+        for (int j = 0; j < 3; j++) {
+            s = red32(rdw0[j]);
+            if (ev && i == 0) sdw0[grp][j] = s;
+        }
+    }
+    if (tile) {
+#pragma unroll
+        for (int a = 0; a < 4; a++)
+#pragma unroll
+            for (int a2 = 0; a2 < 4; a2++) od_red_add(det, G.dw4 + (size_t)(tc + a) * U + tcc + a2, adw4[a][a2]);
     }
     __syncthreads();
     for (int c = t; c < U; c += 256) {
diff --git a/osu_dreamer_amd/csrc/misc.hip b/osu_dreamer_amd/csrc/misc.hip
--- a/osu_dreamer_amd/csrc/misc.hip
+++ b/osu_dreamer_amd/csrc/misc.hip
@@ -62,56 +62,88 @@
     }
 }
 
-template <class T>
+constexpr int PIB_CH = 8;
+template <class T, int NE>
 __global__ __launch_bounds__(256) void proj_in_bwd_kernel(const float* __restrict__ xt, const T* __restrict__ dx, int ldx,
                                                           float* __restrict__ dW, float* __restrict__ db, int B, int E, int L, int D,
                                                           const OdDetTable* __restrict__ det) {
+    static_assert(NE * PIB_CH <= 64, "one lane per (channel, frame) of a chunk");
     __shared__ float red[64][73];
     const int lane = threadIdx.x & 63, wave = threadIdx.x >> 6;
-    const int M = B * L;
-    const int nw = gridDim.x * 4, w0 = blockIdx.x * 4 + wave;
+    const long M = (long)B * L;
+    const long nw = (long)gridDim.x * 4, w0 = (long)blockIdx.x * 4 + wave;
+    const long per = (M + nw - 1) / nw;
+    const long mbeg = w0 * per < M ? w0 * per : M, mend = mbeg + per < M ? mbeg + per : M;
+    const int xe_e = lane / PIB_CH, xe_j = lane % PIB_CH;
     for (int c0 = 0; c0 < D; c0 += 512) {
         const int c = c0 + lane * 8;
-        float aw[8][8], ab[8];
+        const bool act = c < D;
+        float aw[8][NE], ab[8];
 #pragma unroll
         for (int k = 0; k < 8; k++) {
             ab[k] = 0.f;
 #pragma unroll
-            for (int e = 0; e < 8; e++) aw[k][e] = 0.f;
-        }
-        if (c < D)
-            for (int m = w0; m < M; m += nw) {
-                const int b = m / L, l = m - b * L;
-                float xe[8], g[8];
-#pragma unroll
-                for (int e = 0; e < 8; e++) xe[e] = e < E ? xt[((size_t)b * E + e) * L + l] : 0.f;
-                od_ld8(dx + (size_t)m * ldx + c, g);
+            for (int e = 0; e < NE; e++) aw[k][e] = 0.f;
+        }
+        auto chunk = [&](long m) {
+            if (m >= mend) return 0;
+            long n = mend - m;
+            const long left = L - m % L;
+            if (n > left) n = left;
+            return (int)(n < PIB_CH ? n : PIB_CH);
+        };
+        auto fetch = [&](long m, int n, od_raw8<T> (&g)[PIB_CH], float& xv) {
+            const long b = m / L, l = m - b * L;
+            xv = (xe_e < E && xe_j < n) ? xt[((size_t)b * E + xe_e) * L + l + xe_j] : 0.f;
+#pragma unroll
+            for (int j = 0; j < PIB_CH; j++) {
+                if (act && j < n) g[j].ld(dx + (size_t)(m + j) * ldx + c);
+                else g[j].zero();
+            }
+        };
+        od_raw8<T> g[PIB_CH], gn[PIB_CH];
+        float xv = 0.f, xvn = 0.f;
+        long m = mbeg;
+        int n = chunk(m);
+        if (n) fetch(m, n, g, xv);
+        while (n) {
+            const long m2 = m + n;
+            const int n2 = chunk(m2);
+            if (n2) fetch(m2, n2, gn, xvn);
+#pragma unroll
+            for (int j = 0; j < PIB_CH; j++) {
+                float gv[8], xe[NE];
+                g[j].get(gv);
+#pragma unroll
+                for (int e = 0; e < NE; e++) xe[e] = od_readlane(xv, e * PIB_CH + j);
 #pragma unroll
                 for (int k = 0; k < 8; k++) {
-                    ab[k] += g[k];
-#pragma unroll
-                    for (int e = 0; e < 8; e++) aw[k][e] += g[k] * xe[e];
+                    ab[k] += gv[k];
+#pragma unroll
+                    for (int e = 0; e < NE; e++) aw[k][e] += gv[k] * xe[e];
                 }
             }
+#pragma unroll
+            for (int j = 0; j < PIB_CH; j++) g[j] = gn[j];
+            xv = xvn; m = m2; n = n2;
+        }
         for (int w = 0; w < 4; w++) {
             if (wave == w) {
 #pragma unroll
                 for (int k = 0; k < 8; k++) {
                     red[lane][k * 9 + 8] = (w ? red[lane][k * 9 + 8] : 0.f) + ab[k];
 #pragma unroll
-                    for (int e = 0; e < 8; e++) red[lane][k * 9 + e] = (w ? red[lane][k * 9 + e] : 0.f) + aw[k][e];
+                    for (int e = 0; e < NE; e++) red[lane][k * 9 + e] = (w ? red[lane][k * 9 + e] : 0.f) + aw[k][e];
                 }
             }
             __syncthreads();
         }
-        if (wave == 0 && c < D) {
-#pragma unroll
-            for (int k = 0; k < 8; k++) {
-                od_red_add(det, db + c + k, red[lane][k * 9 + 8]);
-#pragma unroll
-                for (int e = 0; e < 8; e++)
-                    if (e < E) od_red_add(det, dW + (size_t)(c + k) * E + e, red[lane][k * 9 + e]);
-            }
+#pragma unroll 1
+        for (int i = threadIdx.x; i < 64 * 72; i += 256) {
+            const int q = i % 72, k = q / 9, e = q % 9, cc = c0 + (i / 72) * 8 + k;
+            if (cc >= D) continue;
+            if (e == 8) od_red_add(det, db + cc, red[i / 72][q]);
+            else if (e < E) od_red_add(det, dW + (size_t)cc * E + e, red[i / 72][q]);
         }
         __syncthreads();
     }
@@ -311,12 +343,11 @@
 }
 
 constexpr int LS_KC = 256, LS_NB = 8;
-__global__ __launch_bounds__(256) void linear_small_kernel(const float* __restrict__ x, const float* __restrict__ W,
-                                                           const float* __restrict__ bias, float* __restrict__ out,
-                                                           float* __restrict__ pre, int B, int N, int K, int act) {
+__device__ __forceinline__ void linear_small_tile(const float* __restrict__ x, const float* __restrict__ W,
+                                                  const float* __restrict__ bias, float* __restrict__ out,
+                                                  float* __restrict__ pre, int B, int N, int K, int act, int b0, int n0) {
     __shared__ __attribute__((aligned(16))) float xs[32][LS_KC + 4];
     __shared__ __attribute__((aligned(16))) float ws[LS_NB][LS_KC + 4];
-    const int b0 = blockIdx.y * 32, n0 = blockIdx.x * LS_NB;
     const int bl = threadIdx.x & 31, nl = threadIdx.x >> 5;
     float acc = 0.f;
     for (int k0 = 0; k0 < K; k0 += LS_KC) {
@@ -343,6 +374,21 @@
         if (pre) pre[(size_t)b * N + n] = s;
         out[(size_t)b * N + n] = act == OD_ACT_SILU ? od_silu(s) : s;
     }
+}
+__global__ __launch_bounds__(256) void linear_small_kernel(const float* __restrict__ x, const float* __restrict__ W,
+                                                           const float* __restrict__ bias, float* __restrict__ out,
+                                                           float* __restrict__ pre, int B, int N, int K, int act) {
+    linear_small_tile(x, W, bias, out, pre, B, N, K, act, blockIdx.y * 32, blockIdx.x * LS_NB);
+}
+constexpr int LSM_MAXJ = 32;
+struct LsJob { const float* W; const float* bias; float* out; int N, blk0; };
+struct LsTable { int n, pad; LsJob j[LSM_MAXJ]; };
+__global__ __launch_bounds__(256) void linear_small_multi_kernel(const float* __restrict__ x, const LsTable tab, int B, int K) {
+    int j = 0;
+    for (int i = 1; i < tab.n; i++)
+        if ((int)blockIdx.x >= tab.j[i].blk0) j = i;
+    linear_small_tile(x, tab.j[j].W, tab.j[j].bias, tab.j[j].out, nullptr, B, tab.j[j].N, K, OD_ACT_NONE, blockIdx.y * 32,
+                      ((int)blockIdx.x - tab.j[j].blk0) * LS_NB);
 }
 __global__ __launch_bounds__(256) void linear_small_dpre_kernel(const float* __restrict__ pre, const float* __restrict__ dout,
                                                                 float* __restrict__ dpre, long n, int act) {
@@ -431,6 +477,77 @@
     slab[32 + (k & 31)] = lo;
 }
 
+constexpr int PWM_TILE = 64;
+constexpr int PWM_MAXJ = 64;
+constexpr int PWM_ROWMAP = 1, PWM_F32 = 2;
+struct PackJob { const float* src; void* dst; void* dst_T; int N, K, Np, Kp, flags, blk0; };
+struct PackTable { int n, pad; const int* row_map; PackJob j[PWM_MAXJ]; };
+
+__device__ __forceinline__ void pwm_store(bf16_t* p, const float (&v)[8]) { od_st8(p, v); }
+__device__ __forceinline__ void pwm_store(float* p, const float (&v)[4]) {
+    f32x4 a; a[0] = v[0]; a[1] = v[1]; a[2] = v[2]; a[3] = v[3];
+    *(f32x4*)p = a;
+}
+template <class T, bool TR>
+__device__ __forceinline__ void pwm_write(T* __restrict__ dst, const float (*tile)[PWM_TILE + 1], int r0, int c0, int R, int C) {
+    constexpr int V = 16 / (int)sizeof(T), CPR = PWM_TILE / V;
+    const bool vec = C % V == 0 && ((size_t)dst & 15) == 0;
+#pragma unroll
+    for (int q = threadIdx.x; q < PWM_TILE * CPR; q += 256) {
+        const int rl = q / CPR, cl = (q % CPR) * V;
+        const int r = r0 + rl, c = c0 + cl;
+        if (r >= R || c >= C) continue;
+        float v[V];
+#pragma unroll
+        for (int i = 0; i < V; i++) v[i] = TR ? tile[cl + i][rl] : tile[rl][cl + i];
+        T* o = dst + (size_t)r * C + c;
+        if (vec) pwm_store(o, v);
+        else {
+            for (int i = 0; i < V; i++)
+                if (c + i < C) od_t<T>::st(o + i, v[i]);
+        }
+    }
+}
+__global__ __launch_bounds__(256) void pack_weights_multi_kernel(const PackTable tab) {
+    __shared__ float tile[PWM_TILE][PWM_TILE + 1];
+    int j = 0;
+    for (int i = 1; i < tab.n; i++)
+        if ((int)blockIdx.x >= tab.j[i].blk0) j = i;
+    const float* __restrict__ src = tab.j[j].src;
+    const int N = tab.j[j].N, K = tab.j[j].K, Np = tab.j[j].Np, Kp = tab.j[j].Kp, flags = tab.j[j].flags;
+    const int tk = (Kp + PWM_TILE - 1) / PWM_TILE, t = (int)blockIdx.x - tab.j[j].blk0;
+    const int n0 = (t / tk) * PWM_TILE, k0 = (t % tk) * PWM_TILE;
+    const bool vsrc = K % 4 == 0 && ((size_t)src & 15) == 0;
+#pragma unroll
+    for (int p = 0; p < PWM_TILE / 16; p++) {
+        const int r = (threadIdx.x >> 4) + 16 * p, c = 4 * (threadIdx.x & 15);
+        const int n = n0 + r, k = k0 + c;
+        int sn = -1;
+        if (n < Np) sn = (flags & PWM_ROWMAP) ? tab.row_map[n] : (n < N ? n : -1);
+        float v[4] = {0.f, 0.f, 0.f, 0.f};
+        if (sn >= 0 && k < K) {
+            const float* s = src + (size_t)sn * K + k;
+            if (vsrc) {
+                const f32x4 a = *(const f32x4*)s;
+                v[0] = a[0]; v[1] = a[1]; v[2] = a[2]; v[3] = a[3];
+            } else {
+                for (int i = 0; i < 4; i++)
+                    if (k + i < K) v[i] = s[i];
+            }
+        }
+#pragma unroll
+        for (int i = 0; i < 4; i++) tile[r][c + i] = v[i];
+    }
+    __syncthreads();
+    if (flags & PWM_F32) {
+        pwm_write<float, false>((float*)tab.j[j].dst, tile, n0, k0, Np, Kp);
+        if (tab.j[j].dst_T) pwm_write<float, true>((float*)tab.j[j].dst_T, tile, k0, n0, Kp, Np);
+    } else {
+        pwm_write<bf16_t, false>((bf16_t*)tab.j[j].dst, tile, n0, k0, Np, Kp);
+        if (tab.j[j].dst_T) pwm_write<bf16_t, true>((bf16_t*)tab.j[j].dst_T, tile, k0, n0, Kp, Np);
+    }
+}
+
 }
 
 #define DISPATCH_T(DT, CALL)                                       \
@@ -465,7 +582,8 @@
     const long M = (long)B * L;
     if (M > 0x7fffffffL) return OD_ERR_UNSUPPORTED;
     int blocks = (int)((M + 63) / 64); if (blocks > 512) blocks = 512; if (blocks < 1) blocks = 1;
-    DISPATCH_T(dtype, OD_LAUNCH((proj_in_bwd_kernel<T_>), dim3(blocks), dim3(256), 0, (hipStream_t)stream, xt, (const T_*)dx, ldx, dW, db, B, E, L, D, od_det_active()));
+    if (E <= 6) DISPATCH_T(dtype, OD_LAUNCH((proj_in_bwd_kernel<T_, 6>), dim3(blocks), dim3(256), 0, (hipStream_t)stream, xt, (const T_*)dx, ldx, dW, db, B, E, L, D, od_det_active()));
+    else DISPATCH_T(dtype, OD_LAUNCH((proj_in_bwd_kernel<T_, 8>), dim3(blocks), dim3(256), 0, (hipStream_t)stream, xt, (const T_*)dx, ldx, dW, db, B, E, L, D, od_det_active()));
     OD_CHECK_LAUNCH();
     return 0;
 }
@@ -589,6 +707,28 @@
     return 0;
 }
 
+extern "C" int od_linear_small_multi(const float* x, int njobs, const void* W, const void* bias, const void* out, const int* N, int B,
+                                     int K, void* stream) {
+    if (njobs < 0 || (njobs && (!W || !bias || !out || !N))) return OD_ERR_ARG;
+    const float* const* Wp = (const float* const*)W;
+    const float* const* bp = (const float* const*)bias;
+    float* const* op = (float* const*)out;
+    for (int j0 = 0; j0 < njobs; j0 += LSM_MAXJ) {
+        LsTable tab;
+        tab.n = njobs - j0 < LSM_MAXJ ? njobs - j0 : LSM_MAXJ;
+        tab.pad = 0;
+        int blocks = 0;
+        for (int i = 0; i < tab.n; i++) {
+            if (N[j0 + i] < 1 || !Wp[j0 + i] || !op[j0 + i]) return OD_ERR_ARG;
+            tab.j[i] = LsJob{Wp[j0 + i], bp[j0 + i], op[j0 + i], N[j0 + i], blocks};
+            blocks += (N[j0 + i] + LS_NB - 1) / LS_NB;
+        }
+        OD_LAUNCH(linear_small_multi_kernel, dim3(blocks, (B + 31) / 32), dim3(256), 0, (hipStream_t)stream, x, tab, B, K);
+    }
+    OD_CHECK_LAUNCH();
+    return 0;
+}
+
 extern "C" int od_linear_small_bwd(const float* x, const float* W, const float* pre, const float* dout, float* dpre, float* dW,
                                    float* db, float* dx, int accumulate_dx, int B, int N, int K, int act, void* stream) {
     if (act != OD_ACT_NONE && !pre) return OD_ERR_ARG;
@@ -619,3 +759,33 @@
     OD_CHECK_LAUNCH();
     return 0;
 }
+
+extern "C" int od_pack_weights_multi(int njobs, const void* src, const void* dst, const void* dst_T, const int* dims, const int* row_map,
+                                     void* stream) {
+    if (njobs < 0 || (njobs && (!src || !dst || !dst_T || !dims))) return OD_ERR_ARG;
+    const float* const* sp = (const float* const*)src;
+    void* const* dp = (void* const*)dst;
+    void* const* tp = (void* const*)dst_T;
+    for (int i = 0; i < njobs; i++) {
+        const int* d = dims + 6 * i;
+        if (d[4] != OD_BF16 && d[4] != OD_F32) return OD_ERR_UNSUPPORTED;
+        if (d[0] < 1 || d[1] < 1 || d[2] < 1 || d[3] < 1 || !sp[i] || !dp[i] || (d[5] && !row_map)) return OD_ERR_ARG;
+    }
+    for (int j0 = 0; j0 < njobs; j0 += PWM_MAXJ) {
+        PackTable tab;
+        tab.n = njobs - j0 < PWM_MAXJ ? njobs - j0 : PWM_MAXJ;
+        tab.pad = 0;
+        tab.row_map = row_map;
+        long blocks = 0;
+        for (int i = 0; i < tab.n; i++) {
+            const int* d = dims + 6 * (j0 + i);
+            tab.j[i] = PackJob{sp[j0 + i], dp[j0 + i], tp[j0 + i], d[0], d[1], d[2], d[3],
+                               (d[5] ? PWM_ROWMAP : 0) | (d[4] == OD_F32 ? PWM_F32 : 0), (int)blocks};
+            blocks += (long)((d[2] + PWM_TILE - 1) / PWM_TILE) * ((d[3] + PWM_TILE - 1) / PWM_TILE);
+            if (blocks > 0x7fffffffL) return OD_ERR_UNSUPPORTED;
+        }
+        OD_LAUNCH(pack_weights_multi_kernel, dim3((unsigned)blocks), dim3(256), 0, (hipStream_t)stream, tab);
+    }
+    OD_CHECK_LAUNCH();
+    return 0;
+}
diff --git a/osu_dreamer_amd/csrc/od_common.h b/osu_dreamer_amd/csrc/od_common.h
--- a/osu_dreamer_amd/csrc/od_common.h
+++ b/osu_dreamer_amd/csrc/od_common.h
@@ -145,6 +145,30 @@
     *(u32x4*)p = r;
 }
 
+template <class T> struct od_raw8;
+template <> struct od_raw8<bf16_t> {
+    u32x4 r;
+    __device__ __forceinline__ void ld(const bf16_t* p) { r = *(const u32x4*)p; }
+    __device__ __forceinline__ void zero() { r = (u32x4)(0u); }
+    __device__ __forceinline__ void get(float (&v)[8]) const {
+#pragma unroll
+        for (int i = 0; i < 4; i++) {
+            union { uint32_t u; float f; } lo, hi;
+            lo.u = r[i] << 16; hi.u = r[i] & 0xffff0000u;
+            v[2 * i] = lo.f; v[2 * i + 1] = hi.f;
+        }
+    }
+};
+template <> struct od_raw8<float> {
+    f32x4 a, b;
+    __device__ __forceinline__ void ld(const float* p) { a = *(const f32x4*)p; b = *(const f32x4*)(p + 4); }
+    __device__ __forceinline__ void zero() { a = (f32x4)(0.f); b = (f32x4)(0.f); }
+    __device__ __forceinline__ void get(float (&v)[8]) const {
+        v[0] = a[0]; v[1] = a[1]; v[2] = a[2]; v[3] = a[3];
+        v[4] = b[0]; v[5] = b[1]; v[6] = b[2]; v[7] = b[3];
+    }
+};
+
 template <class T> __device__ __forceinline__ void od_st8_nt(T* p, const float (&v)[8]) { od_st8(p, v); }
 #if !defined(OD_EMU)
 template <> __device__ __forceinline__ void od_st8_nt<bf16_t>(bf16_t* p, const float (&v)[8]) {
@@ -166,6 +190,30 @@
 __device__ __forceinline__ float od_wave_sum(float v) {
 #pragma unroll
     for (int m = 32; m >= 1; m >>= 1) v += __shfl_xor(v, m);
+    return v;
+}
+#if defined(OD_EMU)
+__device__ __forceinline__ float od_readlane(float v, int src) { return emu::shfl(v, src); }
+#else
+__device__ __forceinline__ float od_readlane(float v, int src) {
+    return __builtin_bit_cast(float, __builtin_amdgcn_readlane(__builtin_bit_cast(int, v), src));
+}
+#endif
+template <int SLOTS>
+__device__ __forceinline__ float od_slot_sum(float (&p)[SLOTS], int lane) {
+    int m = 32;
+#pragma unroll
+    for (int h = SLOTS / 2; h >= 1; h >>= 1, m >>= 1) {
+        const bool up = (lane & m) != 0;
+#pragma unroll
+        for (int i = 0; i < h; i++) {
+            const float send = up ? p[i] : p[i + h], mine = up ? p[i + h] : p[i];
+            p[i] = mine + __shfl_xor(send, m);
+        }
+    }
+    float v = p[0];
+#pragma unroll
+    for (; m >= 1; m >>= 1) v += __shfl_xor(v, m);
     return v;
 }
 __device__ __forceinline__ float od_silu(float x) { return x / (1.0f + __expf(-x)); }
diff --git a/osu_dreamer_amd/csrc/rowops.hip b/osu_dreamer_amd/csrc/rowops.hip
--- a/osu_dreamer_amd/csrc/rowops.hip
+++ b/osu_dreamer_amd/csrc/rowops.hip
@@ -426,49 +426,96 @@
     }
 }
 
-template <class T, int NCH>
+constexpr int FP_RUN = 8;
+template <class T, int NCH, int NE>
 __global__ __launch_bounds__(256) void final_proj_kernel(const T* __restrict__ x, int ldx, const float* __restrict__ W,
                                                          const float* __restrict__ bias, float* __restrict__ vout,
                                                          float* __restrict__ inv_rms, int B, int L, int C, int E, float eps) {
+    constexpr int SLOTS = NE + 1 <= 8 ? 8 : 16, LPS = 64 / SLOTS, NK = FP_RUN / LPS;
+    static_assert(FP_RUN % LPS == 0, "whole passes");
     const int lane = threadIdx.x & 63;
-    const long m = (long)blockIdx.x * 4 + (threadIdx.x >> 6);
-    if (m >= (long)B * L) return;
-    const int b = (int)(m / L), l = (int)(m % L);
-    float v[NCH][8];
-    load_row<T, NCH>(x + m * ldx, C, lane, v);
-    const float inv = rsqrtf(row_sumsq<NCH>(v) / (float)C + eps);
-    if (lane == 0 && inv_rms) inv_rms[m] = inv;
-    for (int e = 0; e < E; e++) {
-        float s = 0.f;
+    const long M = (long)B * L;
+    const long m0 = ((long)blockIdx.x * 4 + (threadIdx.x >> 6)) * FP_RUN;
+    if (m0 >= M) return;
+    float wv[NE][NCH][8];
+#pragma unroll
+    for (int e = 0; e < NE; e++)
 #pragma unroll
         for (int i = 0; i < NCH; i++) {
             const int c = (lane + 64 * i) * 8;
-            if (c >= C) continue;
-            float w[8]; od_ld8(W + (size_t)e * C + c, w);
-#pragma unroll
-            for (int k = 0; k < 8; k++) s += w[k] * v[i][k];
-        }
-        s = od_wave_sum(s) * inv;
-        if (lane == 0) vout[((size_t)b * E + e) * L + l] = s + bias[e];
-    }
-}
-
-template <class T, int NCH>
+#pragma unroll
+            for (int k = 0; k < 8; k++) wv[e][i][k] = 0.f;
+            if (e < E && c < C) od_ld8(W + (size_t)e * C + c, wv[e][i]);
+        }
+    float keep[NK];
+#pragma unroll
+    for (int q = 0; q < NK; q++) keep[q] = 0.f;
+    constexpr int PF = 4;
+    od_raw8<T> ring[PF][NCH];
+    auto fetch = [&](long m, od_raw8<T> (&r)[NCH]) {
+#pragma unroll
+        for (int i = 0; i < NCH; i++) {
+            const int c = (lane + 64 * i) * 8;
+            if (m < M && c < C) r[i].ld(x + m * ldx + c);
+            else r[i].zero();
+        }
+    };
+#pragma unroll
+    for (int r = 0; r < PF - 1; r++) fetch(m0 + r, ring[r]);
+#pragma unroll
+    for (int r = 0; r < FP_RUN; r++) {
+        if (m0 + r >= M) break;
+        if (r + PF - 1 < FP_RUN) fetch(m0 + r + PF - 1, ring[(r + PF - 1) % PF]);
+        const od_raw8<T> (&cur)[NCH] = ring[r % PF];
+        float p[SLOTS];
+#pragma unroll
+        for (int q = 0; q < SLOTS; q++) p[q] = 0.f;
+#pragma unroll
+        for (int i = 0; i < NCH; i++) {
+            float v[8];
+            cur[i].get(v);
+#pragma unroll
+            for (int k = 0; k < 8; k++) {
+                p[0] += v[k] * v[k];
+#pragma unroll
+                for (int e = 0; e < NE; e++) p[1 + e] += wv[e][i][k] * v[k];
+            }
+        }
+        const float tot = od_slot_sum<SLOTS>(p, lane);
+        if (lane % LPS == r % LPS) keep[r / LPS] = tot;
+    }
+    const int slot = lane / LPS;
+#pragma unroll
+    for (int q = 0; q < NK; q++) {
+        const long m = m0 + q * LPS + lane % LPS;
+        const float ss = __shfl(keep[q], lane % LPS);
+        const float inv = rsqrtf(ss / (float)C + eps);
+        if (m >= M) continue;
+        if (slot == 0) {
+            if (inv_rms) inv_rms[m] = inv;
+        } else if (slot - 1 < E) {
+            const int b = (int)(m / L), l = (int)(m % L);
+            vout[((size_t)b * E + slot - 1) * L + l] = keep[q] * inv + bias[slot - 1];
+        }
+    }
+}
+
+template <class T, int NCH, int NE>
 __global__ __launch_bounds__(256) void final_proj_bwd_kernel(const T* __restrict__ x, int ldx, const float* __restrict__ inv_rms,
                                                              const float* __restrict__ W, const float* __restrict__ dv,
                                                              T* __restrict__ dx, int lddx, float* __restrict__ dW,
                                                              float* __restrict__ db, int B, int L, int C, int E,
                                                              const OdDetTable* __restrict__ det) {
-    constexpr int MAXE = 8;
-    __shared__ float red[MAXE * NCH * 512];
+    constexpr int MAXE = 8, RW = ROWS_PER_WAVE_BWD, EPR = 64 / RW, NDV = (NE + EPR - 1) / EPR;
+    static_assert(64 % RW == 0 && NE <= MAXE, "a run's dv fits NDV registers");
+    __shared__ float red[NE * NCH * 512];
     __shared__ float redb[4][MAXE];
     const int lane = threadIdx.x & 63, wave = threadIdx.x >> 6;
     const int b = blockIdx.y;
     const int l0 = (blockIdx.x * 4 + wave) * ROWS_PER_WAVE_BWD;
-    float wv[MAXE][NCH][8], dw[MAXE][NCH][8], dbv[MAXE];
-#pragma unroll
-    for (int e = 0; e < MAXE; e++) {
-        dbv[e] = 0.f;
+    float wv[NE][NCH][8], dw[NE][NCH][8];
+#pragma unroll
+    for (int e = 0; e < NE; e++) {
 #pragma unroll
         for (int i = 0; i < NCH; i++) {
             const int c = (lane + 64 * i) * 8;
@@ -477,28 +524,47 @@
             if (e < E && c < C) od_ld8(W + (size_t)e * C + c, wv[e][i]);
         }
     }
+    float dvr[NDV];
+#pragma unroll
+    for (int q = 0; q < NDV; q++) {
+        const int e = q * EPR + lane / RW, l = l0 + lane % RW;
+        dvr[q] = (e < E && l < L) ? dv[((size_t)b * E + e) * L + l] : 0.f;
+    }
+    const float invr = (lane < RW && l0 + lane < L) ? inv_rms[(long)b * L + l0 + lane] : 0.f;
+    od_raw8<T> cur[NCH], nxt[NCH];
+    auto fetch = [&](int l, od_raw8<T> (&r)[NCH]) {
+#pragma unroll
+        for (int i = 0; i < NCH; i++) {
+            const int c = (lane + 64 * i) * 8;
+            if (l < L && c < C) r[i].ld(x + ((long)b * L + l) * ldx + c);
+            else r[i].zero();
+        }
+    };
+    fetch(l0, cur);
     for (int r = 0; r < ROWS_PER_WAVE_BWD; r++) {
         const int l = l0 + r;
         if (l >= L) break;
         const long m = (long)b * L + l;
-        float xv[NCH][8], dn[NCH][8], dve[MAXE];
-        load_row<T, NCH>(x + m * ldx, C, lane, xv);
-        const float inv = inv_rms[m];
-#pragma unroll
-        for (int e = 0; e < MAXE; e++) { dve[e] = e < E ? dv[((size_t)b * E + e) * L + l] : 0.f; dbv[e] += dve[e]; }
+        if (r + 1 < ROWS_PER_WAVE_BWD) fetch(l + 1, nxt);
+        float xv[NCH][8], dn[NCH][8], dve[NE];
+        const float inv = od_readlane(invr, r);
+#pragma unroll
+        for (int e = 0; e < NE; e++) dve[e] = od_readlane(dvr[e / EPR], (e % EPR) * RW + r);
         float dot = 0.f;
 #pragma unroll
-        for (int i = 0; i < NCH; i++)
+        for (int i = 0; i < NCH; i++) {
+            cur[i].get(xv[i]);
 #pragma unroll
             for (int k = 0; k < 8; k++) {
                 const float xh = xv[i][k] * inv;
                 float s = 0.f;
 #pragma unroll
-                for (int e = 0; e < MAXE; e++) { s += dve[e] * wv[e][i][k]; dw[e][i][k] += dve[e] * xh; }
+                for (int e = 0; e < NE; e++) { s += dve[e] * wv[e][i][k]; dw[e][i][k] += dve[e] * xh; }
                 dn[i][k] = s;
                 dot += s * xh;
                 xv[i][k] = xh;
             }
+        }
         dot = od_wave_sum(dot) / (float)C;
 #pragma unroll
         for (int i = 0; i < NCH; i++) {
@@ -509,13 +575,20 @@
             for (int k = 0; k < 8; k++) o[k] = inv * (dn[i][k] - xv[i][k] * dot);
             od_st8(dx + m * lddx + c, o);
         }
-    }
-    if (lane == 0)
-        for (int e = 0; e < MAXE; e++) redb[wave][e] = dbv[e];
+#pragma unroll
+        for (int i = 0; i < NCH; i++) cur[i] = nxt[i];
+    }
+#pragma unroll
+    for (int q = 0; q < NDV; q++) {
+        float v = dvr[q];
+#pragma unroll
+        for (int mk = RW / 2; mk >= 1; mk >>= 1) v += __shfl_xor(v, mk);
+        if (lane % RW == 0) redb[wave][q * EPR + lane / RW] = v;
+    }
     for (int w = 0; w < 4; w++) {
         if (wave == w) {
 #pragma unroll
-            for (int e = 0; e < MAXE; e++)
+            for (int e = 0; e < NE; e++)
 #pragma unroll
                 for (int i = 0; i < NCH; i++)
 #pragma unroll
@@ -951,9 +1024,14 @@
     if (C % 8 || ldx % 8) return OD_ERR_ALIGN;
     if (E > 8 || C > 1024) return OD_ERR_UNSUPPORTED;
     const long M = (long)B * L;
-    dim3 grid((unsigned)((M + 3) / 4));
-    DISPATCH_T_NCH(dtype, nch_for(C),
-        OD_LAUNCH((final_proj_kernel<T_, N_>), grid, dim3(256), 0, (hipStream_t)stream, (const T_*)x, ldx, W, bias, v, inv_rms, B, L, C, E, eps));
+    dim3 grid((unsigned)((M + 4 * FP_RUN - 1) / (4 * FP_RUN)));
+#define FP_GO(T_, N_, NE_) OD_LAUNCH((final_proj_kernel<T_, N_, NE_>), grid, dim3(256), 0, (hipStream_t)stream, (const T_*)x, ldx, W, bias, v, inv_rms, B, L, C, E, eps)
+#define FP_GO_T(T_) do { if (nch_for(C) == 1) { if (E <= 6) FP_GO(T_, 1, 6); else FP_GO(T_, 1, 8); } else { if (E <= 6) FP_GO(T_, 2, 6); else FP_GO(T_, 2, 8); } } while (0)
+    if (dtype == OD_BF16) FP_GO_T(bf16_t);
+    else if (dtype == OD_F32) FP_GO_T(float);
+    else return OD_ERR_ARG;
+#undef FP_GO_T
+#undef FP_GO
     OD_CHECK_LAUNCH();
     return 0;
 }
@@ -964,12 +1042,11 @@
     if (C % 8 || ldx % 8 || lddx % 8) return OD_ERR_ALIGN;
     if (E > 8 || C > 512) return OD_ERR_UNSUPPORTED;
     dim3 grid((L + 4 * ROWS_PER_WAVE_BWD - 1) / (4 * ROWS_PER_WAVE_BWD), B);
-    if (dtype == OD_BF16)
-        OD_LAUNCH((final_proj_bwd_kernel<bf16_t, 1>), grid, dim3(256), 0, (hipStream_t)stream, (const bf16_t*)x, ldx, inv_rms, W, dv,
-                  (bf16_t*)dx, lddx, dW, db, B, L, C, E, od_det_active());
-    else
-        OD_LAUNCH((final_proj_bwd_kernel<float, 1>), grid, dim3(256), 0, (hipStream_t)stream, (const float*)x, ldx, inv_rms, W, dv,
-                  (float*)dx, lddx, dW, db, B, L, C, E, od_det_active());
+#define FPB_GO(T_, NE_) OD_LAUNCH((final_proj_bwd_kernel<T_, 1, NE_>), grid, dim3(256), 0, (hipStream_t)stream, (const T_*)x, ldx, inv_rms, W, dv, \
+                                  (T_*)dx, lddx, dW, db, B, L, C, E, od_det_active())
+    if (dtype == OD_BF16) { if (E <= 6) FPB_GO(bf16_t, 6); else FPB_GO(bf16_t, 8); }
+    else { if (E <= 6) FPB_GO(float, 6); else FPB_GO(float, 8); }
+#undef FPB_GO
     OD_CHECK_LAUNCH();
     return 0;
 }
diff --git a/osu_dreamer_amd/engine.py b/osu_dreamer_amd/engine.py
--- a/osu_dreamer_amd/engine.py
+++ b/osu_dreamer_amd/engine.py
@@ -110,6 +110,7 @@
                 rm[Hp + j] = Hf + j
             self._rowmap = torch.tensor(rm, dtype=torch.int32, device=dev)
         pk = self._packed
+        jobs = []
         for n in self._gemm_weights():
             w = self.P(n + ".weight")
             N, K = w.shape[0], w.shape[1]
@@ -126,11 +127,17 @@
                     pk[n + ".T"] = torch.empty(Kp, Np, dtype=dtype, device=dev)
                 if rmap is not None:
                     pk[n + ".b"] = torch.empty(Np, dtype=torch.float32, device=dev)
+            if not x3:
+                jobs.append((w, pk[n], pk[n + ".T"] if train else None, rmap is not None))
+                if rmap is not None:
+                    jobs.append((self.P(n + ".bias"), pk[n + ".b"].view(Np, 1), None, True))
+                continue
             ops.pack_weight(w, pk[n], row_map=rmap)
             if train:
                 ops.pack_weight(w, pk[n + ".T"], transpose=True, row_map=rmap)
             if rmap is not None:
                 ops.pack_weight(self.P(n + ".bias"), pk[n + ".b"].view(Np, 1), row_map=rmap)
+        ops.pack_weights_multi(jobs, self._rowmap)
 
     def W(self, name: str, T: bool = False) -> torch.Tensor:
         return self._packed[name + (".T" if T else "")]
@@ -195,14 +202,15 @@
         ops.silu(a_pre, a)
         cg, cg_pre = self.buf("cg", (B, Cg), f32), self.buf("cg_pre", (B, Cg), f32)
         ops.linear_small(style, self.P("proj_style.0.weight"), self.P("proj_style.0.bias"), cg, cg_pre, OD_ACT_SILU)
+        mods = []
         for i in range(self.depth):
             p = f"net.layers.{i}."
             for s in ("ssg1", "ssg2"):
-                ops.linear_small(cg, self.P(p + s + ".weight"), self.P(p + s + ".bias"),
-                                 self.buf(f"{s}.{i}", (B, 3 * D), f32))
+                mods.append((self.P(p + s + ".weight"), self.P(p + s + ".bias"), self.buf(f"{s}.{i}", (B, 3 * D), f32)))
             if not self.train:
                 ops.gemm_nt(a, self.W(p + "proj_cl"), self.P(p + "proj_cl.bias"), self.buf(f"cl.{i}", (self.Ma, D)), x3=self.x3)
-        ops.linear_small(cg, self.P("u_mod.weight"), self.P("u_mod.bias"), self.buf("umod", (B, 2 * U), f32))
+        mods.append((self.P("u_mod.weight"), self.P("u_mod.bias"), self.buf("umod", (B, 2 * U), f32)))
+        ops.linear_small_multi(cg, mods)
 
     def pred(self, xt: torch.Tensor, u: torch.Tensor, v: torch.Tensor):
         B, L, M, D, dh, Hp = self.B, self.L, self.M, self.D, self.dh, self.Hp
diff --git a/osu_dreamer_amd/ops.py b/osu_dreamer_amd/ops.py
--- a/osu_dreamer_amd/ops.py
+++ b/osu_dreamer_amd/ops.py
@@ -1,5 +1,6 @@
 from __future__ import annotations
 
+import ctypes
 import os
 from typing import Optional
 
@@ -126,11 +127,48 @@
     _lib.lib().od_pack_weight(code, _p(src), N, K, _p(dst), Np, Kp, int(transpose), _p(row_map), _stream(src))
 
 
+def pack_weights_multi(jobs, row_map=None):
+    n = len(jobs)
+    if n == 0:
+        return
+    src_a, dst_a, dT_a = (ctypes.c_uint64 * n)(), (ctypes.c_uint64 * n)(), (ctypes.c_uint64 * n)()
+    dims = (ctypes.c_int * (6 * n))()
+    for j, (src, dst, dst_T, mapped) in enumerate(jobs):
+        N = src.shape[0]
+        K = src.numel() // N
+        _f32(src)
+        Np, Kp = dst.shape
+        assert dst.is_contiguous() and (not mapped or (row_map is not None and row_map.numel() == Np))
+        if dst_T is not None:
+            assert dst_T.is_contiguous() and tuple(dst_T.shape) == (Kp, Np) and dst_T.dtype == dst.dtype
+        src_a[j], dst_a[j], dT_a[j] = src.data_ptr(), dst.data_ptr(), 0 if dst_T is None else dst_T.data_ptr()
+        dims[6 * j:6 * j + 6] = [N, K, Np, Kp, dt_code(dst.dtype), int(bool(mapped))]
+    if row_map is not None:
+        _i32(row_map)
+    _lib.lib().od_pack_weights_multi(n, src_a, dst_a, dT_a, dims, _p(row_map), _stream(jobs[0][0]))
+
+
 def linear_small(x, W, b, out, pre=None, act=OD_ACT_NONE):
     B, K = x.shape
     N = W.shape[0]
     _f32(x, W, b, out, pre)
     _lib.lib().od_linear_small(_p(x), _p(W), _p(b), _p(out), _p(pre), B, N, K, act, _stream(x))
+
+
+def linear_small_multi(x, jobs):
+    n = len(jobs)
+    if n == 0:
+        return
+    B, K = x.shape
+    W_a, b_a, o_a = (ctypes.c_uint64 * n)(), (ctypes.c_uint64 * n)(), (ctypes.c_uint64 * n)()
+    N_a = (ctypes.c_int * n)()
+    _f32(x)
+    for j, (W, b, out) in enumerate(jobs):
+        _f32(W, b, out)
+        N = W.shape[0]
+        assert W.numel() == N * K and tuple(out.shape) == (B, N)
+        W_a[j], b_a[j], o_a[j], N_a[j] = W.data_ptr(), 0 if b is None else b.data_ptr(), out.data_ptr(), N
+    _lib.lib().od_linear_small_multi(_p(x), n, W_a, b_a, o_a, N_a, B, K, _stream(x))
 
 
 def linear_small_bwd(x, W, pre, dout, dpre, dW, db, dx, accumulate_dx, act=OD_ACT_NONE):
```

Result: no change. 3.255 (median of 6 runs) (+0.5%).
